# lucidrains/vector-quantize-pytorch

Measured on NVIDIA H100. Metric: vectors quantized/sec at dim=256, codebook=1024; indices bit-exact vs ref, higher is better.
Workload: dtype bf16

## Files before the change

### include/vqb200.h

```cpp
#ifndef VQB200_H
#define VQB200_H

#include <stddef.h>
#include <stdint.h>

#ifdef __cplusplus
extern "C" {
#endif

#define VQB_VERSION 100

#define VQB_DTYPE_F32 0
#define VQB_DTYPE_BF16 1

#define VQB_METRIC_EUCLID 0
#define VQB_METRIC_COSINE 1

#define VQB_OK 0
#define VQB_E_INVALID -1
#define VQB_E_UNSUPPORTED -2
#define VQB_E_ALIGN -3
#define VQB_E_NO_DEVICE -4
#define VQB_E_DRIVER -5
#define VQB_E_WORKSPACE -6

typedef struct vqb_flag_entry {
  int32_t row;
  int32_t count;
  int32_t cand0;
  int32_t cand1;
  int32_t cand2;
  int32_t pad[3];
} vqb_flag_entry;

typedef struct vqb_fused_outputs {
  const void* x_eff;
  const float* embed;
  void* q_out;
  int64_t* idx64_out;
  int64_t idx_stride;
  double* loss_sum;
  const void* x_raw;
  void* resid_out;
  void* qsum;
  float* stats_cnt;
  float* stats_sum;
  int dtype;
  void* planes_out;
} vqb_fused_outputs;

int vqb_version(void);
const char* vqb_strerror(int code);

int vqb_padded_codes(int K);

int vqb_codebook_prepare(const float* embed, int K, int D, int metric, void* planes, void* bext, float* bias,
                         float* cnorm2, float* cmax, void* stream);

int vqb_input_prepare(const void* x, int dtype, int64_t N, int D, int metric, void* x_eff, void* a_planes,
                      int n_planes, void* stream);

int vqb_assign(const void* a_planes, int n_a, int64_t N, int D, const void* b_planes, const void* bext,
               const float* cmax, int K, float margin_rel, int n_passes, int32_t* idx, vqb_flag_entry* flagged,
               int32_t* flag_count, float* dbg_best, const vqb_fused_outputs* fused , void* stream);

int vqb_assign_ex(const void* a_planes, int n_a, int64_t N, int D, const void* b_planes, const void* bext,
                  const float* cmax, int K, float margin_rel, int n_passes, int32_t* idx, vqb_flag_entry* flagged,
                  int32_t* flag_count, float* dbg_best, const vqb_fused_outputs* fused, int metric, const float* cnorm2,
                  void* stream);

int vqb_debug_set_profile_buffer(void* device_buffer);
int vqb_debug_active(void);
int vqb_debug_set_mode(int mode);
int vqb_debug_graph_stats(long long* out4);
int vqb_debug_assign_plan(int n_a, int D, int n_passes, int* out6);
int vqb_debug_stats_plan(int64_t N, int K, int sms, int* out3);

int vqb_fix_flagged(const void* x_eff, int dtype, int64_t N, int D, const float* embed, const float* cnorm2, int K,
                    int metric, vqb_flag_entry* flagged, const int32_t* flag_count, int32_t* idx,
                    const vqb_fused_outputs* fused , void* stream);

int vqb_gather(const void* x_eff, int dtype, int64_t N, int D, const float* embed, const int32_t* idx, void* q_out,
               int64_t* idx64_out, int64_t idx_stride, double* loss_sum, const void* x_raw, void* resid_out, void* qsum,
               void* stream);

int vqb_loss_finalize(const double* loss_sum, int64_t numel, int dtype, float weight, float* loss_out, void* stream);

int64_t vqb_stats_offset(int K);
int64_t vqb_stats_floats(int K, int D);
size_t vqb_ema_stats_workspace(int64_t N, int K);
int vqb_ema_stats(const void* x_eff, int dtype, int64_t N, int D, const int32_t* idx, int K, float* stats,
                  void* workspace, size_t workspace_bytes, void* stream);

int vqb_ema_apply(float* cluster_size, float* embed_avg, float* embed, const float* stats, int K, int D, double decay,
                  double eps, int metric, int do_lerp, int do_normalise, void* planes, void* bext, float* bias,
                  float* cnorm2, float* cmax, float* scratch, void* stream);

int vqb_ema_apply_weighted(float* cluster_size, float* embed_avg, float* embed, const float* stats, int K, int D,
                           double decay, double eps, int metric, int do_lerp, int do_normalise, const float* code_weight,
                           void* planes, void* bext, float* bias, float* cnorm2, float* cmax, float* scratch, void* stream);

int vqb_peer_barrier(void* const* peer_flags_host, int rank, int world, uint32_t* epoch_dev, void* stream);
int vqb_ema_apply_peers(float* cluster_size, float* embed_avg, float* embed, const void* const* peer_stats_host, int world,
                        int64_t slice_offset, int K, int D, double decay, double eps, int metric, int do_normalise,
                        const float* code_weight, void* planes, void* bext, float* bias, float* cnorm2, float* cmax,
                        float* scratch, void* stream);

typedef struct vqb_vq_forward_args {
  const void* x;
  int dtype, metric;
  int64_t N;
  int D, K;
  int already_normalised;
  float* cluster_size;
  float* embed_avg;
  float* embed;
  void* planes; void* bext; float* bias; float* cnorm2; float* cmax; float* scratch;
  void* q_out;
  int64_t* idx64_out; int64_t idx_stride;
  float* loss_out; float loss_weight;
  void* resid_out;
  void* qsum;
  int32_t* idx32;
  int update;
  int stats_mode;
  int stats_accumulate;
  int do_normalise;
  double decay, eps;
  float* stats;
  float margin_rel;
  void* workspace; size_t workspace_bytes;
  void* ev_search_begin; void* ev_search_end;
  const void* const* peer_stats; void* const* peer_flags; uint32_t* peer_epoch; int peer_rank, peer_world;
  int64_t peer_slice_offset;
  const void* a_planes_in; void* planes_out;
  const uint8_t* row_mask; const int64_t* n_live;
} vqb_vq_forward_args;
size_t vqb_vq_forward_workspace(int64_t N, int D, int K, int dtype, int metric, int update);
int vqb_vq_forward(const vqb_vq_forward_args* args, void* stream);

int vqb_decode(const float* embeds, int64_t embed_stride, int Q, int K, int D, const int64_t* idx, int64_t N,
               void* out, int dtype, void* stream);

int vqb_rvq_accumulate(const float* embeds, int64_t embed_stride, int Q, int K, int D, const int64_t* idx, int64_t N,
                       void* out, int dtype, void* stream);
int vqb_debug_gather_sum_plan(int nbooks, int K, int D, int esz, int64_t N, int sms, int* out3);

enum { VQB_RVQ_STAGE = 0, VQB_RVQ_EMA = 1, VQB_RVQ_ACCUMULATE = 2, VQB_RVQ_BARRIER = 3, VQB_RVQ_EMA_PEERS = 4,
       VQB_RVQ_SIMVQ_TAIL = 5 };
typedef struct vqb_rvq_op {
  int kind, lane;
  vqb_vq_forward_args stage;
  struct {
    float* cluster_size; float* embed_avg; float* embed; const float* stats; int K, D; double decay, eps;
    int metric, do_lerp, do_normalise; void* planes; void* bext; float* bias; float* cnorm2; float* cmax; float* scratch;
    int n_lerp; int64_t slice_stride;
  } ema;
  struct {
    const float* embeds; int64_t embed_stride; int Q, K, D; const int64_t* idx; int64_t N; void* out; int dtype;
  } acc;
  struct { void* const* flags; uint32_t* epoch; int rank, world; } bar;
  struct {
    float* cluster_size; float* embed_avg; float* embed; const void* const* peer_stats; int64_t slice_offset; int world, K, D;
    double decay, eps; int metric, do_normalise; void* planes; void* bext; float* bias; float* cnorm2; float* cmax; float* scratch;
    int n_lerp; int64_t slice_stride;
  } emap;
  struct {
    const float* r; const float* codes; const int32_t* idx; int64_t N; int D, rotation; float* r_next; float* qsum; int first;
    int64_t* idx64_out; int64_t idx_stride; double* loss_sum; float* loss_out; float input_weight, weight;
  } simvq;
} vqb_rvq_op;
int vqb_rvq_forward(const vqb_rvq_op* ops, int n_ops, void* stream);

int vqb_rsimvq_tail(const float* r, const float* codes, const int32_t* idx, int64_t N, int D, int rotation, float* r_next,
                    float* qsum, int first, int64_t* idx64_out, int64_t idx_stride, double* loss_sum, float* loss_out,
                    float input_weight, float weight, void* stream);
int vqb_rsimvq_backward(const float* x, const float* codes, int Q, int K, const int64_t* idx, int64_t N, int D, int n_active,
                        int rotation, const float* grad_q, const float* grad_loss, float* grad_x, void* stream);

int vqb_rotate(const void* src, const void* tgt, const void* grad_out, int64_t N, int D, int dtype, void* out, void* stream);

int vqb_diveq(const void* x, const void* q, const void* noise, const void* grad_out, int64_t N, int D, int dtype,
              float noise_scale, void* out, float* grad_q, void* stream);

int vqb_fsq_forward(const void* z, int in_dtype, int work_dtype, int64_t N, int G, int D, int Q, int n_active, int sym, int hard,
                    const float* consts, const float* scales, const float* clampv, void* out, void* idx, int idx64,
                    int64_t idx_s_row, int64_t idx_s_g, int64_t idx_s_q, void* stream);
int vqb_fsq_backward(const void* z, int in_dtype, int work_dtype, int64_t N, int G, int D, int Q, int n_active, int sym, int hard,
                     const float* consts, const float* scales, const float* clampv, const void* grad_out, void* grad_z,
                     void* stream);
int vqb_fsq_decode(const void* idx, int idx64, int64_t idx_s_row, int64_t idx_s_g, int64_t idx_s_q, int64_t N, int G, int D,
                   int Q, int work_dtype, int sym, const float* consts, const int32_t* levels_basis, const float* scales, void* out,
                   void* codes, void* stream);

int vqb_lfq_forward(const void* z, int dtype, int64_t N, int G, int D, int Q, int n_active, int residual, int training, int spherical,
                    const float* params, void* out, void* idx, int64_t idx_s_row, int64_t idx_s_g, int64_t idx_s_q, float* ent,
                    const uint8_t* rowmask, double* commit, int commit_blocks, void* stream);
int vqb_lfq_forward_blocks(int64_t N, int G);
int vqb_lfq_entropy(const float* x, int64_t N, int G, int D, int S, const int32_t* rows, int64_t R, int64_t rows_stride,
                    const float* m, float tau, int chunks, double* pse, float* colsum, void* stream);
int vqb_lfq_entropy_tiles(int D);
int vqb_lfq_entropy_backward(const float* x, int64_t N, int G, int D, int S, const int32_t* rows, int64_t R, int64_t rows_stride,
                             const float* m, float tau, const float* cp, const float* V, int ksplit, float* work, float* grad,
                             void* stream);
int vqb_lfq_backward(const void* z, int dtype, int64_t N, int G, int D, int Q, int n_active, int residual, int training, int spherical,
                     const float* params, const void* grad_out, const float* grad_ent, const float* cc, const uint8_t* rowmask,
                     void* grad_z, void* stream);
int vqb_lfq_decode(const void* idx, int idx64, int64_t idx_s_row, int64_t idx_s_g, int64_t idx_s_q, int64_t N, int G, int D, int Q,
                   const float* vals, float* out, float* codes, void* stream);

#ifdef __cplusplus
}
#endif
#endif
```

### vector_quantize_pytorch_b200/_C.py

```python
import ctypes
import os

from . import build as _build

_c = ctypes
_i32, _i64, _f32, _f64, _vp, _sz = _c.c_int, _c.c_int64, _c.c_float, _c.c_double, _c.c_void_p, _c.c_size_t

DTYPE_F32, DTYPE_BF16 = 0, 1
METRIC_EUCLID, METRIC_COSINE = 0, 1

class FusedOutputs(ctypes.Structure):
    _fields_ = [("x_eff", _vp), ("embed", _vp), ("q_out", _vp), ("idx64_out", _vp), ("idx_stride", _i64),
                ("loss_sum", _vp), ("x_raw", _vp), ("resid_out", _vp), ("qsum", _vp), ("stats_cnt", _vp), ("stats_sum", _vp),
                ("dtype", _i32), ("planes_out", _vp)]


class VQForwardArgs(ctypes.Structure):
    _fields_ = [("x", _vp), ("dtype", _i32), ("metric", _i32), ("N", _i64), ("D", _i32), ("K", _i32),
                ("already_normalised", _i32), ("cluster_size", _vp), ("embed_avg", _vp), ("embed", _vp),
                ("planes", _vp), ("bext", _vp), ("bias", _vp), ("cnorm2", _vp), ("cmax", _vp), ("scratch", _vp),
                ("q_out", _vp), ("idx64_out", _vp), ("idx_stride", _i64), ("loss_out", _vp), ("loss_weight", _f32),
                ("resid_out", _vp), ("qsum", _vp), ("idx32", _vp), ("update", _i32), ("stats_mode", _i32), ("stats_accumulate", _i32), ("do_normalise", _i32),
                ("decay", _f64), ("eps", _f64), ("stats", _vp), ("margin_rel", _f32), ("workspace", _vp),
                ("workspace_bytes", _sz), ("ev_search_begin", _vp), ("ev_search_end", _vp),
                ("peer_stats", _vp), ("peer_flags", _vp), ("peer_epoch", _vp), ("peer_rank", _i32), ("peer_world", _i32),
                ("peer_slice_offset", _i64), ("a_planes_in", _vp), ("planes_out", _vp), ("row_mask", _vp), ("n_live", _vp)]


class RvqEmaArgs(ctypes.Structure):
    _fields_ = [("cluster_size", _vp), ("embed_avg", _vp), ("embed", _vp), ("stats", _vp), ("K", _i32), ("D", _i32),
                ("decay", _f64), ("eps", _f64), ("metric", _i32), ("do_lerp", _i32), ("do_normalise", _i32),
                ("planes", _vp), ("bext", _vp), ("bias", _vp), ("cnorm2", _vp), ("cmax", _vp), ("scratch", _vp),
                ("n_lerp", _i32), ("slice_stride", _i64)]


class RvqAccArgs(ctypes.Structure):
    _fields_ = [("embeds", _vp), ("embed_stride", _i64), ("Q", _i32), ("K", _i32), ("D", _i32), ("idx", _vp), ("N", _i64),
                ("out", _vp), ("dtype", _i32)]


class RvqBarArgs(ctypes.Structure):
    _fields_ = [("flags", _vp), ("epoch", _vp), ("rank", _i32), ("world", _i32)]


class RvqEmaPeersArgs(ctypes.Structure):
    _fields_ = [("cluster_size", _vp), ("embed_avg", _vp), ("embed", _vp), ("peer_stats", _vp), ("slice_offset", _i64),
                ("world", _i32), ("K", _i32), ("D", _i32), ("decay", _f64), ("eps", _f64), ("metric", _i32),
                ("do_normalise", _i32), ("planes", _vp), ("bext", _vp), ("bias", _vp), ("cnorm2", _vp), ("cmax", _vp),
                ("scratch", _vp), ("n_lerp", _i32), ("slice_stride", _i64)]


class RvqSimvqArgs(ctypes.Structure):
    _fields_ = [("r", _vp), ("codes", _vp), ("idx", _vp), ("N", _i64), ("D", _i32), ("rotation", _i32), ("r_next", _vp),
                ("qsum", _vp), ("first", _i32), ("idx64_out", _vp), ("idx_stride", _i64), ("loss_sum", _vp), ("loss_out", _vp),
                ("input_weight", _f32), ("weight", _f32)]


class RvqOp(ctypes.Structure):
    _fields_ = [("kind", _i32), ("lane", _i32), ("stage", VQForwardArgs), ("ema", RvqEmaArgs), ("acc", RvqAccArgs),
                ("bar", RvqBarArgs), ("emap", RvqEmaPeersArgs), ("simvq", RvqSimvqArgs)]


RVQ_STAGE, RVQ_EMA, RVQ_ACCUMULATE, RVQ_BARRIER, RVQ_EMA_PEERS, RVQ_SIMVQ_TAIL = 0, 1, 2, 3, 4, 5

SIGNATURES = {
    "vqb_version": (_i32, []),
    "vqb_strerror": (_c.c_char_p, [_i32]),
    "vqb_padded_codes": (_i32, [_i32]),
    "vqb_codebook_prepare": (_i32, [_vp, _i32, _i32, _i32, _vp, _vp, _vp, _vp, _vp, _vp]),
    "vqb_input_prepare": (_i32, [_vp, _i32, _i64, _i32, _i32, _vp, _vp, _i32, _vp]),
    "vqb_assign": (_i32, [_vp, _i32, _i64, _i32, _vp, _vp, _vp, _i32, _f32, _i32, _vp, _vp, _vp, _vp, _vp, _vp]),
    "vqb_assign_ex": (_i32, [_vp, _i32, _i64, _i32, _vp, _vp, _vp, _i32, _f32, _i32, _vp, _vp, _vp, _vp, _vp, _i32, _vp, _vp]),
    "vqb_fix_flagged": (_i32, [_vp, _i32, _i64, _i32, _vp, _vp, _i32, _i32, _vp, _vp, _vp, _vp, _vp]),
    "vqb_gather": (_i32, [_vp, _i32, _i64, _i32, _vp, _vp, _vp, _vp, _i64, _vp, _vp, _vp, _vp, _vp]),
    "vqb_loss_finalize": (_i32, [_vp, _i64, _i32, _f32, _vp, _vp]),
    "vqb_stats_offset": (_i64, [_i32]),
    "vqb_stats_floats": (_i64, [_i32, _i32]),
    "vqb_ema_stats_workspace": (_sz, [_i64, _i32]),
    "vqb_ema_stats": (_i32, [_vp, _i32, _i64, _i32, _vp, _i32, _vp, _vp, _sz, _vp]),
    "vqb_ema_apply": (_i32, [_vp, _vp, _vp, _vp, _i32, _i32, _f64, _f64, _i32, _i32, _i32, _vp, _vp, _vp, _vp, _vp, _vp, _vp]),
    "vqb_rotate": (_i32, [_vp, _vp, _vp, _i64, _i32, _i32, _vp, _vp]),
    "vqb_diveq": (_i32, [_vp, _vp, _vp, _vp, _i64, _i32, _i32, _f32, _vp, _vp, _vp]),
    "vqb_peer_barrier": (_i32, [_vp, _i32, _i32, _vp, _vp]),
    "vqb_ema_apply_peers": (_i32, [_vp, _vp, _vp, _vp, _i32, _i64, _i32, _i32, _f64, _f64, _i32, _i32, _vp, _vp, _vp, _vp, _vp, _vp, _vp, _vp]),
    "vqb_ema_apply_weighted": (_i32, [_vp, _vp, _vp, _vp, _i32, _i32, _f64, _f64, _i32, _i32, _i32, _vp, _vp, _vp, _vp, _vp, _vp, _vp, _vp]),
    "vqb_vq_forward_workspace": (_sz, [_i64, _i32, _i32, _i32, _i32, _i32]),
    "vqb_vq_forward": (_i32, [_vp, _vp]),
    "vqb_debug_set_profile_buffer": (_i32, [_vp]),
    "vqb_debug_set_mode": (_i32, [_i32]),
    "vqb_debug_active": (_i32, []),
    "vqb_debug_graph_stats": (_i32, [_vp]),
    "vqb_debug_assign_plan": (_i32, [_i32, _i32, _i32, _vp]),
    "vqb_debug_stats_plan": (_i32, [_i64, _i32, _i32, _vp]),
    "vqb_decode": (_i32, [_vp, _i64, _i32, _i32, _i32, _vp, _i64, _vp, _i32, _vp]),
    "vqb_rvq_accumulate": (_i32, [_vp, _i64, _i32, _i32, _i32, _vp, _i64, _vp, _i32, _vp]),
    "vqb_debug_gather_sum_plan": (_i32, [_i32, _i32, _i32, _i32, _i64, _i32, _vp]),
    "vqb_rvq_forward": (_i32, [_vp, _i32, _vp]),
    "vqb_rsimvq_tail": (_i32, [_vp, _vp, _vp, _i64, _i32, _i32, _vp, _vp, _i32, _vp, _i64, _vp, _vp, _f32, _f32, _vp]),
    "vqb_rsimvq_backward": (_i32, [_vp, _vp, _i32, _i32, _vp, _i64, _i32, _i32, _i32, _vp, _vp, _vp, _vp]),
    "vqb_fsq_forward": (_i32, [_vp, _i32, _i32, _i64, _i32, _i32, _i32, _i32, _i32, _i32, _vp, _vp, _vp, _vp, _vp, _i32, _i64, _i64,
                               _i64, _vp]),
    "vqb_fsq_backward": (_i32, [_vp, _i32, _i32, _i64, _i32, _i32, _i32, _i32, _i32, _i32, _vp, _vp, _vp, _vp, _vp, _vp]),
    "vqb_fsq_decode": (_i32, [_vp, _i32, _i64, _i64, _i64, _i64, _i32, _i32, _i32, _i32, _i32, _vp, _vp, _vp, _vp, _vp, _vp]),
    "vqb_lfq_forward": (_i32, [_vp, _i32, _i64, _i32, _i32, _i32, _i32, _i32, _i32, _i32, _vp, _vp, _vp, _i64, _i64, _i64, _vp, _vp,
                               _vp, _i32, _vp]),
    "vqb_lfq_forward_blocks": (_i32, [_i64, _i32]),
    "vqb_lfq_entropy": (_i32, [_vp, _i64, _i32, _i32, _i32, _vp, _i64, _i64, _vp, _f32, _i32, _vp, _vp, _vp]),
    "vqb_lfq_entropy_tiles": (_i32, [_i32]),
    "vqb_lfq_entropy_backward": (_i32, [_vp, _i64, _i32, _i32, _i32, _vp, _i64, _i64, _vp, _f32, _vp, _vp, _i32, _vp, _vp, _vp]),
    "vqb_lfq_backward": (_i32, [_vp, _i32, _i64, _i32, _i32, _i32, _i32, _i32, _i32, _i32, _vp, _vp, _vp, _vp, _vp, _vp, _vp]),
    "vqb_lfq_decode": (_i32, [_vp, _i32, _i64, _i64, _i64, _i64, _i32, _i32, _i32, _vp, _vp, _vp, _vp]),
}


def _load():
    path = os.environ.get("VQB200_LIB")
    if not path:
        path = _build.LIB
        if _build.is_stale():
            if _build.find_nvcc() is not None:
                path = _build.build()
            elif not os.path.exists(path):
                raise ImportError("vqb200: libvqb200.so is missing and nvcc is not available to build it; "
                                  "run `python -m vector_quantize_pytorch_b200.build` where nvcc exists")
    lib = ctypes.CDLL(path)
    for name, (res, args) in SIGNATURES.items():
        fn = getattr(lib, name)
        fn.restype = res
        fn.argtypes = args
    return lib, path


lib, LIB_PATH = _load()


class VQBError(RuntimeError):
    pass


def check(rc, what):
    if rc != 0:
        raise VQBError(f"{what}: {lib.vqb_strerror(rc).decode()} (code {rc})")
```

### vector_quantize_pytorch_b200/csrc/code_operands.cuh

```cuda
#pragma once
#include "vqb_common.cuh"

namespace vqb {

constexpr int CODE_ROW_MAX_D = 8 * 128;

template <int NV>
__device__ __forceinline__ void load_code_row(const float* row, int D, int lane, float4 (&c)[NV]) {
#pragma unroll
  for (int j = 0; j < NV; ++j) {
    const int i = j * 128 + lane * 4;
    c[j] = i < D ? *reinterpret_cast<const float4*>(row + i) : make_float4(0.f, 0.f, 0.f, 0.f);
  }
}

template <int NV>
__device__ __forceinline__ void write_code_operands(const float4 (&c)[NV], int k, int Kpad, int D, int metric, uint16_t* planes,
                                                    uint16_t* bext, float* bias, float* cnorm2, float* cmax, int lane) {
  uint16_t* hi = planes + static_cast<int64_t>(k) * D;
  uint16_t* lo = planes + (static_cast<int64_t>(Kpad) + k) * D;
  double n2 = 0.0;
  float r2 = 0.f, l2 = 0.f;
#pragma unroll
  for (int j = 0; j < NV; ++j) {
    const int i = j * 128 + lane * 4;
    if (i >= D) continue;
    const float v[4] = {c[j].x, c[j].y, c[j].z, c[j].w};
    uint16_t h[4], l[4];
#pragma unroll
    for (int e = 0; e < 4; ++e) {
      h[e] = float_to_bf16_bits(v[e]);
      const float dl = v[e] - bf16_bits_to_float(h[e]);
      l[e] = float_to_bf16_bits(dl);
      const float d2 = dl - bf16_bits_to_float(l[e]);
      r2 = fmaf(d2, d2, r2);
      l2 = fmaf(bf16_bits_to_float(l[e]), bf16_bits_to_float(l[e]), l2);
      n2 += static_cast<double>(v[e]) * static_cast<double>(v[e]);
    }
    *reinterpret_cast<uint2*>(hi + i) = make_uint2(h[0] | (uint32_t(h[1]) << 16), h[2] | (uint32_t(h[3]) << 16));
    *reinterpret_cast<uint2*>(lo + i) = make_uint2(l[0] | (uint32_t(l[1]) << 16), l[2] | (uint32_t(l[3]) << 16));
  }
  n2 = warp_sum(n2);
  r2 = warp_sum(r2);
  l2 = warp_sum(l2);
  if (lane == 0) {
    const float n2f = static_cast<float>(n2);
    cnorm2[k] = n2f;
    const float b = (metric == VQB_METRIC_EUCLID) ? 0.5f * n2f : 0.f;
    bias[k] = b;
    const uint16_t b1 = float_to_bf16_bits(b);
    const float q1 = b - bf16_bits_to_float(b1);
    const uint16_t b2 = float_to_bf16_bits(q1);
    const uint16_t b3 = float_to_bf16_bits(q1 - bf16_bits_to_float(b2));
    uint16_t* row = bext + k * 16;
    row[0] = b1 ^ 0x8000; row[1] = b2 ^ 0x8000; row[2] = b3 ^ 0x8000;
#pragma unroll
    for (int j = 3; j < 16; ++j) row[j] = 0;
    atomicMax(reinterpret_cast<unsigned int*>(cmax + CMAX_NORM), __float_as_uint(sqrtf(n2f)));
    atomicMax(reinterpret_cast<unsigned int*>(cmax + CMAX_RES), __float_as_uint(__fsqrt_ru(r2) * 1.0001f));
    atomicMax(reinterpret_cast<unsigned int*>(cmax + CMAX_LO), __float_as_uint(__fsqrt_ru(l2) * 1.0001f));
  }
}

__device__ __forceinline__ void write_padding_operands(int k, int Kpad, int D, uint16_t* planes, uint16_t* bext, float* bias,
                                                       int lane) {
  uint16_t* hi = planes + static_cast<int64_t>(k) * D;
  uint16_t* lo = planes + (static_cast<int64_t>(Kpad) + k) * D;
  for (int i = lane; i < D; i += 32) { hi[i] = 0; lo[i] = 0; }
  if (lane == 0) bias[k] = INFINITY;
  if (lane < 16) bext[k * 16 + lane] = (lane == 0) ? float_to_bf16_bits(-3.0e38f) : 0;
}

}
```

### vector_quantize_pytorch_b200/csrc/ptx.cuh

```cuda
#pragma once
#include <cuda.h>
#include <cuda_runtime.h>
#include <stdint.h>

namespace vqb {

__device__ __forceinline__ uint32_t smem_u32(const void* p) {
  return static_cast<uint32_t>(__cvta_generic_to_shared(p));
}

__device__ __forceinline__ void mbar_init(uint32_t bar, uint32_t count) {
  asm volatile("mbarrier.init.shared::cta.b64 [%0], %1;" ::"r"(bar), "r"(count));
}
__device__ __forceinline__ void fence_barrier_init() {
  asm volatile("fence.mbarrier_init.release.cluster;" ::: "memory");
}
__device__ __forceinline__ void mbar_arrive(uint32_t bar) {
  asm volatile("mbarrier.arrive.shared::cta.b64 _, [%0];" ::"r"(bar) : "memory");
}
__device__ __forceinline__ void mbar_arrive_expect_tx(uint32_t bar, uint32_t bytes) {
  asm volatile("mbarrier.arrive.expect_tx.shared::cta.b64 _, [%0], %1;" ::"r"(bar), "r"(bytes) : "memory");
}
__device__ __forceinline__ bool mbar_try_wait(uint32_t bar, uint32_t parity) {
  uint32_t ok;
  asm volatile(
      "{\n"
      ".reg .pred p;\n"
      "mbarrier.try_wait.parity.shared::cta.b64 p, [%1], %2;\n"
      "selp.u32 %0, 1, 0, p;\n"
      "}\n"
      : "=r"(ok)
      : "r"(bar), "r"(parity)
      : "memory");
  return ok != 0;
}

#ifndef VQB_WAIT_TIMEOUT_CYCLES
#define VQB_WAIT_TIMEOUT_CYCLES (8000000000ll)
#endif
__device__ __forceinline__ void mbar_wait(uint32_t bar, uint32_t parity) {
  if (mbar_try_wait(bar, parity)) return;
  const long long t0 = clock64();
  while (!mbar_try_wait(bar, parity)) {
    if (clock64() - t0 > VQB_WAIT_TIMEOUT_CYCLES) __trap();
  }
}

__device__ __forceinline__ void tma_prefetch_desc(const CUtensorMap* m) {
  asm volatile("prefetch.tensormap [%0];" ::"l"(reinterpret_cast<uint64_t>(m)) : "memory");
}
__device__ __forceinline__ void tma_load_3d(uint32_t dst, const CUtensorMap* m, uint32_t bar, int c0, int c1, int c2) {
  asm volatile(
      "cp.async.bulk.tensor.3d.shared::cluster.global.tile.mbarrier::complete_tx::bytes [%0], [%1, {%3, %4, %5}], [%2];"
      ::"r"(dst), "l"(reinterpret_cast<uint64_t>(m)), "r"(bar), "r"(c0), "r"(c1), "r"(c2)
      : "memory");
}

__device__ __forceinline__ void tma_prefetch_l2_3d(const CUtensorMap* m, int c0, int c1, int c2) {
  asm volatile("cp.async.bulk.prefetch.tensor.3d.L2.global.tile [%0, {%1, %2, %3}];"
               ::"l"(reinterpret_cast<uint64_t>(m)), "r"(c0), "r"(c1), "r"(c2)
               : "memory");
}

__device__ __forceinline__ uint64_t wgmma_desc_sw128(uint32_t saddr) {
  uint64_t d = 0;
  d |= static_cast<uint64_t>((saddr >> 4) & 0x3FFF);
  d |= static_cast<uint64_t>(1) << 16;
  d |= static_cast<uint64_t>(1024 >> 4) << 32;
  d |= static_cast<uint64_t>(1) << 62;
  return d;
}

__device__ __forceinline__ uint64_t wgmma_desc_sw32(uint32_t saddr) {
  uint64_t d = 0;
  d |= static_cast<uint64_t>((saddr >> 4) & 0x3FFF);
  d |= static_cast<uint64_t>(1) << 16;
  d |= static_cast<uint64_t>(256 >> 4) << 32;
  d |= static_cast<uint64_t>(3) << 62;
  return d;
}

__device__ __forceinline__ void fence_proxy_async_shared() { asm volatile("fence.proxy.async.shared::cta;" ::: "memory"); }
__device__ __forceinline__ void wgmma_fence() { asm volatile("wgmma.fence.sync.aligned;" ::: "memory"); }
__device__ __forceinline__ void wgmma_commit() { asm volatile("wgmma.commit_group.sync.aligned;" ::: "memory"); }
template <int N>
__device__ __forceinline__ void wgmma_wait() { asm volatile("wgmma.wait_group.sync.aligned %0;" ::"n"(N) : "memory"); }

template <int R>
__device__ __forceinline__ void fence_regs(float (&d)[R]) {
#pragma unroll
  for (int i = 0; i < R; ++i) asm volatile("" : "+f"(d[i])::"memory");
}

__device__ __forceinline__ void wgmma_m64n128k16_bf16(float (&d)[64], uint64_t adesc, uint64_t bdesc) {
  asm volatile(
      "{\n"
      "wgmma.mma_async.sync.aligned.m64n128k16.f32.bf16.bf16 "
      "{%0, %1, %2, %3, %4, %5, %6, %7, %8, %9, %10, %11, %12, %13, %14, %15, "
      "%16, %17, %18, %19, %20, %21, %22, %23, %24, %25, %26, %27, %28, %29, %30, %31, "
      "%32, %33, %34, %35, %36, %37, %38, %39, %40, %41, %42, %43, %44, %45, %46, %47, "
      "%48, %49, %50, %51, %52, %53, %54, %55, %56, %57, %58, %59, %60, %61, %62, %63}, "
      "%64, %65, 1, 1, 1, 0, 0;\n"
      "}\n"
      : "+f"(d[0]), "+f"(d[1]), "+f"(d[2]), "+f"(d[3]), "+f"(d[4]), "+f"(d[5]), "+f"(d[6]), "+f"(d[7]),
        "+f"(d[8]), "+f"(d[9]), "+f"(d[10]), "+f"(d[11]), "+f"(d[12]), "+f"(d[13]), "+f"(d[14]), "+f"(d[15]),
        "+f"(d[16]), "+f"(d[17]), "+f"(d[18]), "+f"(d[19]), "+f"(d[20]), "+f"(d[21]), "+f"(d[22]), "+f"(d[23]),
        "+f"(d[24]), "+f"(d[25]), "+f"(d[26]), "+f"(d[27]), "+f"(d[28]), "+f"(d[29]), "+f"(d[30]), "+f"(d[31]),
        "+f"(d[32]), "+f"(d[33]), "+f"(d[34]), "+f"(d[35]), "+f"(d[36]), "+f"(d[37]), "+f"(d[38]), "+f"(d[39]),
        "+f"(d[40]), "+f"(d[41]), "+f"(d[42]), "+f"(d[43]), "+f"(d[44]), "+f"(d[45]), "+f"(d[46]), "+f"(d[47]),
        "+f"(d[48]), "+f"(d[49]), "+f"(d[50]), "+f"(d[51]), "+f"(d[52]), "+f"(d[53]), "+f"(d[54]), "+f"(d[55]),
        "+f"(d[56]), "+f"(d[57]), "+f"(d[58]), "+f"(d[59]), "+f"(d[60]), "+f"(d[61]), "+f"(d[62]), "+f"(d[63])
      : "l"(adesc), "l"(bdesc));
}

__device__ __forceinline__ void wgmma_m64n128k16_bf16_rs_set(float (&d)[64], uint32_t a01, uint64_t bdesc) {
  asm volatile(
      "{\n"
      ".reg .pred p;\n"
      "setp.ne.b32 p, %67, 0;\n"
      "wgmma.mma_async.sync.aligned.m64n128k16.f32.bf16.bf16 "
      "{%0, %1, %2, %3, %4, %5, %6, %7, %8, %9, %10, %11, %12, %13, %14, %15, "
      "%16, %17, %18, %19, %20, %21, %22, %23, %24, %25, %26, %27, %28, %29, %30, %31, "
      "%32, %33, %34, %35, %36, %37, %38, %39, %40, %41, %42, %43, %44, %45, %46, %47, "
      "%48, %49, %50, %51, %52, %53, %54, %55, %56, %57, %58, %59, %60, %61, %62, %63}, "
      "{%64, %64, %65, %65}, %66, p, 1, 1, 0;\n"
      "}\n"
      : "=f"(d[0]), "=f"(d[1]), "=f"(d[2]), "=f"(d[3]), "=f"(d[4]), "=f"(d[5]), "=f"(d[6]), "=f"(d[7]),
        "=f"(d[8]), "=f"(d[9]), "=f"(d[10]), "=f"(d[11]), "=f"(d[12]), "=f"(d[13]), "=f"(d[14]), "=f"(d[15]),
        "=f"(d[16]), "=f"(d[17]), "=f"(d[18]), "=f"(d[19]), "=f"(d[20]), "=f"(d[21]), "=f"(d[22]), "=f"(d[23]),
        "=f"(d[24]), "=f"(d[25]), "=f"(d[26]), "=f"(d[27]), "=f"(d[28]), "=f"(d[29]), "=f"(d[30]), "=f"(d[31]),
        "=f"(d[32]), "=f"(d[33]), "=f"(d[34]), "=f"(d[35]), "=f"(d[36]), "=f"(d[37]), "=f"(d[38]), "=f"(d[39]),
        "=f"(d[40]), "=f"(d[41]), "=f"(d[42]), "=f"(d[43]), "=f"(d[44]), "=f"(d[45]), "=f"(d[46]), "=f"(d[47]),
        "=f"(d[48]), "=f"(d[49]), "=f"(d[50]), "=f"(d[51]), "=f"(d[52]), "=f"(d[53]), "=f"(d[54]), "=f"(d[55]),
        "=f"(d[56]), "=f"(d[57]), "=f"(d[58]), "=f"(d[59]), "=f"(d[60]), "=f"(d[61]), "=f"(d[62]), "=f"(d[63])
      : "r"(a01), "r"(0u), "l"(bdesc), "n"(0));
}

__device__ __forceinline__ void wgmma_m64n256k16_bf16(float (&d)[128], uint64_t adesc, uint64_t bdesc) {
  asm volatile(
      "{\n"
      "wgmma.mma_async.sync.aligned.m64n256k16.f32.bf16.bf16 "
      "{%0, %1, %2, %3, %4, %5, %6, %7, %8, %9, %10, %11, %12, %13, %14, %15, "
      "%16, %17, %18, %19, %20, %21, %22, %23, %24, %25, %26, %27, %28, %29, %30, %31, "
      "%32, %33, %34, %35, %36, %37, %38, %39, %40, %41, %42, %43, %44, %45, %46, %47, "
      "%48, %49, %50, %51, %52, %53, %54, %55, %56, %57, %58, %59, %60, %61, %62, %63, "
      "%64, %65, %66, %67, %68, %69, %70, %71, %72, %73, %74, %75, %76, %77, %78, %79, "
      "%80, %81, %82, %83, %84, %85, %86, %87, %88, %89, %90, %91, %92, %93, %94, %95, "
      "%96, %97, %98, %99, %100, %101, %102, %103, %104, %105, %106, %107, %108, %109, %110, %111, "
      "%112, %113, %114, %115, %116, %117, %118, %119, %120, %121, %122, %123, %124, %125, %126, %127}, "
      "%128, %129, 1, 1, 1, 0, 0;\n"
      "}\n"
      :
        "+f"(d[0]), "+f"(d[1]), "+f"(d[2]), "+f"(d[3]), "+f"(d[4]), "+f"(d[5]), "+f"(d[6]), "+f"(d[7]),
        "+f"(d[8]), "+f"(d[9]), "+f"(d[10]), "+f"(d[11]), "+f"(d[12]), "+f"(d[13]), "+f"(d[14]), "+f"(d[15]),
        "+f"(d[16]), "+f"(d[17]), "+f"(d[18]), "+f"(d[19]), "+f"(d[20]), "+f"(d[21]), "+f"(d[22]), "+f"(d[23]),
        "+f"(d[24]), "+f"(d[25]), "+f"(d[26]), "+f"(d[27]), "+f"(d[28]), "+f"(d[29]), "+f"(d[30]), "+f"(d[31]),
        "+f"(d[32]), "+f"(d[33]), "+f"(d[34]), "+f"(d[35]), "+f"(d[36]), "+f"(d[37]), "+f"(d[38]), "+f"(d[39]),
        "+f"(d[40]), "+f"(d[41]), "+f"(d[42]), "+f"(d[43]), "+f"(d[44]), "+f"(d[45]), "+f"(d[46]), "+f"(d[47]),
        "+f"(d[48]), "+f"(d[49]), "+f"(d[50]), "+f"(d[51]), "+f"(d[52]), "+f"(d[53]), "+f"(d[54]), "+f"(d[55]),
        "+f"(d[56]), "+f"(d[57]), "+f"(d[58]), "+f"(d[59]), "+f"(d[60]), "+f"(d[61]), "+f"(d[62]), "+f"(d[63]),
        "+f"(d[64]), "+f"(d[65]), "+f"(d[66]), "+f"(d[67]), "+f"(d[68]), "+f"(d[69]), "+f"(d[70]), "+f"(d[71]),
        "+f"(d[72]), "+f"(d[73]), "+f"(d[74]), "+f"(d[75]), "+f"(d[76]), "+f"(d[77]), "+f"(d[78]), "+f"(d[79]),
        "+f"(d[80]), "+f"(d[81]), "+f"(d[82]), "+f"(d[83]), "+f"(d[84]), "+f"(d[85]), "+f"(d[86]), "+f"(d[87]),
        "+f"(d[88]), "+f"(d[89]), "+f"(d[90]), "+f"(d[91]), "+f"(d[92]), "+f"(d[93]), "+f"(d[94]), "+f"(d[95]),
        "+f"(d[96]), "+f"(d[97]), "+f"(d[98]), "+f"(d[99]), "+f"(d[100]), "+f"(d[101]), "+f"(d[102]), "+f"(d[103]),
        "+f"(d[104]), "+f"(d[105]), "+f"(d[106]), "+f"(d[107]), "+f"(d[108]), "+f"(d[109]), "+f"(d[110]), "+f"(d[111]),
        "+f"(d[112]), "+f"(d[113]), "+f"(d[114]), "+f"(d[115]), "+f"(d[116]), "+f"(d[117]), "+f"(d[118]), "+f"(d[119]),
        "+f"(d[120]), "+f"(d[121]), "+f"(d[122]), "+f"(d[123]), "+f"(d[124]), "+f"(d[125]), "+f"(d[126]), "+f"(d[127])
      : "l"(adesc), "l"(bdesc));
}

__device__ __forceinline__ void wgmma_m64n256k16_bf16_ss_set(float (&d)[128], uint64_t adesc, uint64_t bdesc) {
  asm volatile(
      "{\n"
      ".reg .pred p;\n"
      "setp.ne.b32 p, %130, 0;\n"
      "wgmma.mma_async.sync.aligned.m64n256k16.f32.bf16.bf16 "
      "{%0, %1, %2, %3, %4, %5, %6, %7, %8, %9, %10, %11, %12, %13, %14, %15, "
      "%16, %17, %18, %19, %20, %21, %22, %23, %24, %25, %26, %27, %28, %29, %30, %31, "
      "%32, %33, %34, %35, %36, %37, %38, %39, %40, %41, %42, %43, %44, %45, %46, %47, "
      "%48, %49, %50, %51, %52, %53, %54, %55, %56, %57, %58, %59, %60, %61, %62, %63, "
      "%64, %65, %66, %67, %68, %69, %70, %71, %72, %73, %74, %75, %76, %77, %78, %79, "
      "%80, %81, %82, %83, %84, %85, %86, %87, %88, %89, %90, %91, %92, %93, %94, %95, "
      "%96, %97, %98, %99, %100, %101, %102, %103, %104, %105, %106, %107, %108, %109, %110, %111, "
      "%112, %113, %114, %115, %116, %117, %118, %119, %120, %121, %122, %123, %124, %125, %126, %127}, "
      "%128, %129, p, 1, 1, 0, 0;\n"
      "}\n"
      :
        "=f"(d[0]), "=f"(d[1]), "=f"(d[2]), "=f"(d[3]), "=f"(d[4]), "=f"(d[5]), "=f"(d[6]), "=f"(d[7]),
        "=f"(d[8]), "=f"(d[9]), "=f"(d[10]), "=f"(d[11]), "=f"(d[12]), "=f"(d[13]), "=f"(d[14]), "=f"(d[15]),
        "=f"(d[16]), "=f"(d[17]), "=f"(d[18]), "=f"(d[19]), "=f"(d[20]), "=f"(d[21]), "=f"(d[22]), "=f"(d[23]),
        "=f"(d[24]), "=f"(d[25]), "=f"(d[26]), "=f"(d[27]), "=f"(d[28]), "=f"(d[29]), "=f"(d[30]), "=f"(d[31]),
        "=f"(d[32]), "=f"(d[33]), "=f"(d[34]), "=f"(d[35]), "=f"(d[36]), "=f"(d[37]), "=f"(d[38]), "=f"(d[39]),
        "=f"(d[40]), "=f"(d[41]), "=f"(d[42]), "=f"(d[43]), "=f"(d[44]), "=f"(d[45]), "=f"(d[46]), "=f"(d[47]),
        "=f"(d[48]), "=f"(d[49]), "=f"(d[50]), "=f"(d[51]), "=f"(d[52]), "=f"(d[53]), "=f"(d[54]), "=f"(d[55]),
        "=f"(d[56]), "=f"(d[57]), "=f"(d[58]), "=f"(d[59]), "=f"(d[60]), "=f"(d[61]), "=f"(d[62]), "=f"(d[63]),
        "=f"(d[64]), "=f"(d[65]), "=f"(d[66]), "=f"(d[67]), "=f"(d[68]), "=f"(d[69]), "=f"(d[70]), "=f"(d[71]),
        "=f"(d[72]), "=f"(d[73]), "=f"(d[74]), "=f"(d[75]), "=f"(d[76]), "=f"(d[77]), "=f"(d[78]), "=f"(d[79]),
        "=f"(d[80]), "=f"(d[81]), "=f"(d[82]), "=f"(d[83]), "=f"(d[84]), "=f"(d[85]), "=f"(d[86]), "=f"(d[87]),
        "=f"(d[88]), "=f"(d[89]), "=f"(d[90]), "=f"(d[91]), "=f"(d[92]), "=f"(d[93]), "=f"(d[94]), "=f"(d[95]),
        "=f"(d[96]), "=f"(d[97]), "=f"(d[98]), "=f"(d[99]), "=f"(d[100]), "=f"(d[101]), "=f"(d[102]), "=f"(d[103]),
        "=f"(d[104]), "=f"(d[105]), "=f"(d[106]), "=f"(d[107]), "=f"(d[108]), "=f"(d[109]), "=f"(d[110]), "=f"(d[111]),
        "=f"(d[112]), "=f"(d[113]), "=f"(d[114]), "=f"(d[115]), "=f"(d[116]), "=f"(d[117]), "=f"(d[118]), "=f"(d[119]),
        "=f"(d[120]), "=f"(d[121]), "=f"(d[122]), "=f"(d[123]), "=f"(d[124]), "=f"(d[125]), "=f"(d[126]), "=f"(d[127])
      : "l"(adesc), "l"(bdesc), "n"(0));
}

__device__ __forceinline__ void wgmma_m64n256k16_bf16_rs_set(float (&d)[128], uint32_t a01, uint64_t bdesc) {
  asm volatile(
      "{\n"
      ".reg .pred p;\n"
      "setp.ne.b32 p, %131, 0;\n"
      "wgmma.mma_async.sync.aligned.m64n256k16.f32.bf16.bf16 "
      "{%0, %1, %2, %3, %4, %5, %6, %7, %8, %9, %10, %11, %12, %13, %14, %15, "
      "%16, %17, %18, %19, %20, %21, %22, %23, %24, %25, %26, %27, %28, %29, %30, %31, "
      "%32, %33, %34, %35, %36, %37, %38, %39, %40, %41, %42, %43, %44, %45, %46, %47, "
      "%48, %49, %50, %51, %52, %53, %54, %55, %56, %57, %58, %59, %60, %61, %62, %63, "
      "%64, %65, %66, %67, %68, %69, %70, %71, %72, %73, %74, %75, %76, %77, %78, %79, "
      "%80, %81, %82, %83, %84, %85, %86, %87, %88, %89, %90, %91, %92, %93, %94, %95, "
      "%96, %97, %98, %99, %100, %101, %102, %103, %104, %105, %106, %107, %108, %109, %110, %111, "
      "%112, %113, %114, %115, %116, %117, %118, %119, %120, %121, %122, %123, %124, %125, %126, %127}, "
      "{%128, %128, %129, %129}, %130, p, 1, 1, 0;\n"
      "}\n"
      :
        "=f"(d[0]), "=f"(d[1]), "=f"(d[2]), "=f"(d[3]), "=f"(d[4]), "=f"(d[5]), "=f"(d[6]), "=f"(d[7]),
        "=f"(d[8]), "=f"(d[9]), "=f"(d[10]), "=f"(d[11]), "=f"(d[12]), "=f"(d[13]), "=f"(d[14]), "=f"(d[15]),
        "=f"(d[16]), "=f"(d[17]), "=f"(d[18]), "=f"(d[19]), "=f"(d[20]), "=f"(d[21]), "=f"(d[22]), "=f"(d[23]),
        "=f"(d[24]), "=f"(d[25]), "=f"(d[26]), "=f"(d[27]), "=f"(d[28]), "=f"(d[29]), "=f"(d[30]), "=f"(d[31]),
        "=f"(d[32]), "=f"(d[33]), "=f"(d[34]), "=f"(d[35]), "=f"(d[36]), "=f"(d[37]), "=f"(d[38]), "=f"(d[39]),
        "=f"(d[40]), "=f"(d[41]), "=f"(d[42]), "=f"(d[43]), "=f"(d[44]), "=f"(d[45]), "=f"(d[46]), "=f"(d[47]),
        "=f"(d[48]), "=f"(d[49]), "=f"(d[50]), "=f"(d[51]), "=f"(d[52]), "=f"(d[53]), "=f"(d[54]), "=f"(d[55]),
        "=f"(d[56]), "=f"(d[57]), "=f"(d[58]), "=f"(d[59]), "=f"(d[60]), "=f"(d[61]), "=f"(d[62]), "=f"(d[63]),
        "=f"(d[64]), "=f"(d[65]), "=f"(d[66]), "=f"(d[67]), "=f"(d[68]), "=f"(d[69]), "=f"(d[70]), "=f"(d[71]),
        "=f"(d[72]), "=f"(d[73]), "=f"(d[74]), "=f"(d[75]), "=f"(d[76]), "=f"(d[77]), "=f"(d[78]), "=f"(d[79]),
        "=f"(d[80]), "=f"(d[81]), "=f"(d[82]), "=f"(d[83]), "=f"(d[84]), "=f"(d[85]), "=f"(d[86]), "=f"(d[87]),
        "=f"(d[88]), "=f"(d[89]), "=f"(d[90]), "=f"(d[91]), "=f"(d[92]), "=f"(d[93]), "=f"(d[94]), "=f"(d[95]),
        "=f"(d[96]), "=f"(d[97]), "=f"(d[98]), "=f"(d[99]), "=f"(d[100]), "=f"(d[101]), "=f"(d[102]), "=f"(d[103]),
        "=f"(d[104]), "=f"(d[105]), "=f"(d[106]), "=f"(d[107]), "=f"(d[108]), "=f"(d[109]), "=f"(d[110]), "=f"(d[111]),
        "=f"(d[112]), "=f"(d[113]), "=f"(d[114]), "=f"(d[115]), "=f"(d[116]), "=f"(d[117]), "=f"(d[118]), "=f"(d[119]),
        "=f"(d[120]), "=f"(d[121]), "=f"(d[122]), "=f"(d[123]), "=f"(d[124]), "=f"(d[125]), "=f"(d[126]), "=f"(d[127])
      : "r"(a01), "r"(0u), "l"(bdesc), "n"(0));
}

}
```

### vector_quantize_pytorch_b200/csrc/vq_assign.cu

```cuda
#include <type_traits>
#include "ptx.cuh"
#include "vqb_common.cuh"
#include "gather_row.cuh"
#include "epilogue.cuh"

#ifdef VQB_PROFILE
#define PROF_CLOCK() clock64()
#else
#define PROF_CLOCK() 0ll
#endif

namespace vqb {

constexpr int BM = 128;
constexpr int WM = 64;
constexpr int BN_STAGE = 128;
constexpr int BK = 64;
constexpr int A_SUB_BYTES = BM * BK * 2;
constexpr int B_SUB_BYTES = BN_STAGE * BK * 2;
constexpr int MAX_A_SUB = 8;
constexpr int MAX_STAGES = 8;
constexpr int NUM_CONSUMER_WARPS = 8;
constexpr int NUM_STORE_WARPS = 3;
constexpr int NUM_THREADS = 128 + NUM_CONSUMER_WARPS * 32;
constexpr int SMEM_CTRL_BYTES = 14336;
constexpr int SMEM_LIMIT = 232448;
constexpr int SEED_BYTES = BN_STAGE * 32;

struct AssignParams {
  int64_t N;
  int D, K, Kpad;
  int n_a, n_passes;
  int KB;
  int n_stages;
  int n_seed;
  int stream_a;
  const uint16_t* a_global;
  const uint16_t* bext;
  int num_row_tiles, num_code_steps;
  float margin_rel;
  const float* cmax;
  int32_t* idx;
  int32_t* idx_prov;
  int32_t* hist;
  int hist_shift;
  vqb_flag_entry* flagged;
  int32_t* flag_count;
  float* dbg_best;
  const uint8_t* row_mask;
  long long* prof;
  FusedOut fo;
  int copy_mode;
  int resid_mode;
  int metric;
  const uint16_t* b_hi;
  const float* cnorm2;
  uint32_t tagmask, mul1, mulm1;
};

struct Ctrl {
  uint64_t a_full[MAX_A_SUB], a_empty[MAX_A_SUB];
  uint64_t b_full[MAX_STAGES], b_empty[MAX_STAGES];
  uint64_t g_full[2], g_empty[2];
  int gidx[2][BM];
  MergeSlot merge[BM][3];
  float x2[BM];
};
static_assert(sizeof(Ctrl) <= SMEM_CTRL_BYTES, "control block too large");

template <int GB>
__device__ __forceinline__ float tail_rows(const FusedOut& fo, const int64_t (&rows)[GB], const int (&ks)[GB], int D, int lane) {
  if (fo.dtype == VQB_DTYPE_BF16) return gather_rows<VQB_DTYPE_BF16, GB>(fo, rows, ks, D, lane);
  return gather_rows<VQB_DTYPE_F32, GB>(fo, rows, ks, D, lane);
}

__device__ __forceinline__ float sq_diff16(const uint4& xa, const uint4& ca, bool bf) {
  const uint32_t xw[4] = {xa.x, xa.y, xa.z, xa.w}, cw[4] = {ca.x, ca.y, ca.z, ca.w};
  float s = 0.f;
#pragma unroll
  for (int e = 0; e < 4; ++e) {
    if (bf) {
      const float d0 = __uint_as_float(xw[e] << 16) - __uint_as_float(cw[e] << 16);
      const float d1 = __uint_as_float(xw[e] & 0xFFFF0000u) - __uint_as_float(cw[e] & 0xFFFF0000u);
      s += bf16_round(d0 * d0);
      s += bf16_round(d1 * d1);
    } else {
      const float d = __uint_as_float(xw[e]) - __uint_as_float(cw[e]);
      s += d * d;
    }
  }
  return s;
}

template <int WN>
struct StepLocals {
  float loss_ = 0.f;
  __device__ __forceinline__ float& loss() { return loss_; }
};
template <>
struct StepLocals<256> {
  static __device__ __forceinline__ float& loss() {
    __shared__ float s[NUM_CONSUMER_WARPS * 32];
    return s[threadIdx.x - 128];
  }
  static __device__ __forceinline__ uint32_t* bias_ones() {
    __shared__ __align__(256) uint32_t o[WM * 16 / 2];
    return o;
  }
  __device__ __forceinline__ StepLocals() { loss() = 0.f; }
};
constexpr int WIDE_STATIC_SMEM = NUM_CONSUMER_WARPS * 32 * 4 + WM * 16 * 2;

template <int TAIL, int WN>
__global__ void __launch_bounds__(NUM_THREADS, 1)
vq_assign_kernel(const __grid_constant__ CUtensorMap tmA, const __grid_constant__ CUtensorMap tmB,
                 const __grid_constant__ CUtensorMap tmS, const AssignParams p) {
  static_assert(WN == 128 || WN == 256, "code step width");
  constexpr int SPAN = WN / BN_STAGE;
  constexpr uint32_t STEP_SEED_BYTES = SPAN * SEED_BYTES;
  extern __shared__ __align__(1024) uint8_t smem[];
  Ctrl* ctrl = reinterpret_cast<Ctrl*>(smem);
  const uint32_t smem_base = smem_u32(smem);
  const uint32_t a_base = (smem_base + SMEM_CTRL_BYTES + 1023u) & ~1023u;
  const bool stream_a = WN == 128 && p.stream_a;
  const int n_sub = stream_a ? 0 : p.n_a * p.KB;
  const uint32_t b_base = a_base + n_sub * A_SUB_BYTES;
  const uint32_t a_stage_bytes = stream_a ? A_SUB_BYTES : 0;
  const uint32_t stage_stride = a_stage_bytes + SPAN * B_SUB_BYTES;
  const int n_ring = p.n_stages / SPAN;
  const uint32_t seed_base = b_base + n_ring * stage_stride;

  const int warp = threadIdx.x >> 5;
  const int lane = threadIdx.x & 31;

  if (threadIdx.x == 0) {
    tma_prefetch_desc(&tmA);
    tma_prefetch_desc(&tmB);
    tma_prefetch_desc(&tmS);
    for (int s = 0; s < n_sub; ++s) {
      mbar_init(smem_u32(&ctrl->a_full[s]), 1);
      mbar_init(smem_u32(&ctrl->a_empty[s]), NUM_CONSUMER_WARPS);
    }
    for (int s = 0; s < n_ring; ++s) {
      mbar_init(smem_u32(&ctrl->b_full[s]), 1);
      mbar_init(smem_u32(&ctrl->b_empty[s]), NUM_CONSUMER_WARPS);
    }
    for (int s = 0; s < 2; ++s) {
      mbar_init(smem_u32(&ctrl->g_full[s]), NUM_CONSUMER_WARPS);
      mbar_init(smem_u32(&ctrl->g_empty[s]), NUM_STORE_WARPS);
    }
    fence_barrier_init();
  }
  if constexpr (WN == 256) {
    for (int i = threadIdx.x; i < WM * 16 / 2; i += NUM_THREADS) StepLocals<256>::bias_ones()[i] = 0x3F803F80u;
    fence_proxy_async_shared();
  }
  __syncthreads();

  if (warp == 0) {
    if (lane == 0) {
      long long w_empty = 0, w_aempty = 0;
      const long long pstart = PROF_CLOCK();
      int stage = 0, gstep = 0;
      uint32_t ph = 0;
      for (int t = 0, tile = static_cast<int>(blockIdx.x); tile < p.num_row_tiles; ++t, tile += static_cast<int>(gridDim.x)) {
        const int row0 = tile * BM;
        if (!stream_a && tile + static_cast<int>(gridDim.x) < p.num_row_tiles) {
          for (int ap = 0; ap < p.n_a; ++ap)
            for (int kb = 0; kb < p.KB; ++kb) tma_prefetch_l2_3d(&tmA, kb * BK, row0 + static_cast<int>(gridDim.x) * BM, ap);
        }
        for (int ct = 0; ct < p.num_code_steps; ++ct, ++gstep) {
          for (int kb = 0; kb < p.KB; ++kb) {
            for (int ps = 0; ps < p.n_passes; ++ps) {
              const int bplane = (ps == 1) ? 1 : 0;
              const int aplane = (ps == 2) ? 1 : 0;
              if (!stream_a && ct == 0 && (ps == 0 || ps == 2)) {
                const int sub = aplane * p.KB + kb;
                { const long long c0 = PROF_CLOCK(); mbar_wait(smem_u32(&ctrl->a_empty[sub]), (t & 1) ^ 1); w_aempty += PROF_CLOCK() - c0; }
                mbar_arrive_expect_tx(smem_u32(&ctrl->a_full[sub]), A_SUB_BYTES);
                tma_load_3d(a_base + sub * A_SUB_BYTES, &tmA, smem_u32(&ctrl->a_full[sub]), kb * BK, row0, aplane);
              }
              { const long long c0 = PROF_CLOCK(); mbar_wait(smem_u32(&ctrl->b_empty[stage]), ph ^ 1); w_empty += PROF_CLOCK() - c0; }
              const bool seeds = kb == 0 && ps == 0;
              mbar_arrive_expect_tx(smem_u32(&ctrl->b_full[stage]), stage_stride + (seeds ? STEP_SEED_BYTES : 0));
              if (seeds)
                tma_load_3d(seed_base + (gstep % p.n_seed) * STEP_SEED_BYTES, &tmS, smem_u32(&ctrl->b_full[stage]), 0, ct * WN, 0);
              if (stream_a)
                tma_load_3d(b_base + stage * stage_stride, &tmA, smem_u32(&ctrl->b_full[stage]), kb * BK, row0, aplane);
              tma_load_3d(b_base + stage * stage_stride + a_stage_bytes, &tmB, smem_u32(&ctrl->b_full[stage]), kb * BK,
                          ct * WN, bplane);
              if (++stage == n_ring) { stage = 0; ph ^= 1; }
            }
          }
        }
      }
      if (p.prof) {
        p.prof[blockIdx.x * 16 + 0] = w_empty;
        p.prof[blockIdx.x * 16 + 1] = PROF_CLOCK() - pstart;
        p.prof[blockIdx.x * 16 + 6] = w_aempty;
      }
    }
  } else if (warp <= NUM_STORE_WARPS) {
    const int sw = warp - 1;
    float lsum = 0.f;
    for (int t = 0, tile = static_cast<int>(blockIdx.x); p.fo.enabled && tile < p.num_row_tiles; ++t, tile += static_cast<int>(gridDim.x)) {
      mbar_wait(smem_u32(&ctrl->g_full[t & 1]), (t >> 1) & 1);
      const int* gi = ctrl->gidx[t & 1];
      if (TAIL >= 1) {
        constexpr int CB = 4;
        const bool bf = p.fo.dtype == VQB_DTYPE_BF16;
        const int row_bytes = p.D * (bf ? 2 : 4);
        const uint8_t* src = bf ? reinterpret_cast<const uint8_t*>(p.b_hi) : reinterpret_cast<const uint8_t*>(p.fo.embed);
        const uint8_t* xin = static_cast<const uint8_t*>(p.fo.x_eff);
        uint8_t* dst = static_cast<uint8_t*>(TAIL == 2 ? p.fo.resid_out : p.fo.q_out);
        for (int r0 = sw * CB; r0 < BM; r0 += NUM_STORE_WARPS * CB) {
          int ks[CB];
          bool ex[CB];
#pragma unroll
          for (int b = 0; b < CB; ++b) {
            const int g = gi[r0 + b];
            ex[b] = g < -1;
            ks[b] = ex[b] ? -2 - g : g;
          }
          const int64_t row_base = static_cast<int64_t>(tile) * BM + r0;
          if (p.fo.idx64_out && lane < CB && ks[lane & (CB - 1)] >= 0) {
            int kk = 0;
#pragma unroll
            for (int b = 0; b < CB; ++b) kk = (lane == b) ? ks[b] : kk;
            p.fo.idx64_out[(row_base + lane) * p.fo.idx_stride] = kk;
          }
          if (dst || (ex[0] | ex[1] | ex[2] | ex[3])) {
            for (int off = lane * 16; off < row_bytes; off += 512) {
              uint4 v[CB];
#pragma unroll
              for (int b = 0; b < CB; ++b)
                if (ks[b] >= 0) v[b] = __ldg(reinterpret_cast<const uint4*>(src + static_cast<int64_t>(ks[b]) * row_bytes + off));
              if (TAIL == 1) {
#pragma unroll
                for (int b = 0; b < CB; ++b)
                  if (ex[b]) lsum += sq_diff16(*reinterpret_cast<const uint4*>(xin + (row_base + b) * row_bytes + off), v[b], bf);
              }
              if (TAIL == 2) {
                uint4 x[CB];
#pragma unroll
                for (int b = 0; b < CB; ++b)
                  if (ks[b] >= 0) x[b] = *reinterpret_cast<const uint4*>(xin + (row_base + b) * row_bytes + off);
#pragma unroll
                for (int b = 0; b < CB; ++b) {
                  if (ks[b] < 0) continue;
                  if (ex[b]) lsum += sq_diff16(x[b], v[b], bf);
                  const uint32_t xw[4] = {x[b].x, x[b].y, x[b].z, x[b].w}, cw[4] = {v[b].x, v[b].y, v[b].z, v[b].w};
                  uint32_t rw[4];
                  if (bf) {
#pragma unroll
                    for (int e = 0; e < 4; ++e) {
                      const float d0 = __uint_as_float(xw[e] << 16) - __uint_as_float(cw[e] << 16);
                      const float d1 = __uint_as_float(xw[e] & 0xFFFF0000u) - __uint_as_float(cw[e] & 0xFFFF0000u);
                      asm("cvt.rn.bf16x2.f32 %0, %1, %2;" : "=r"(rw[e]) : "f"(d1), "f"(d0));
                    }
                  } else {
#pragma unroll
                    for (int e = 0; e < 4; ++e) rw[e] = __float_as_uint(__uint_as_float(xw[e]) - __uint_as_float(cw[e]));
                    if (p.fo.planes_out) {
                      const float rf[4] = {__uint_as_float(rw[0]), __uint_as_float(rw[1]), __uint_as_float(rw[2]), __uint_as_float(rw[3])};
                      store_planes4(p.fo.planes_out, p.fo.planes_stride, ((row_base + b) * row_bytes + off) >> 2, rf);
                    }
                  }
                  v[b] = make_uint4(rw[0], rw[1], rw[2], rw[3]);
                }
              }
#pragma unroll
              for (int b = 0; b < CB; ++b)
                if (dst && ks[b] >= 0) *reinterpret_cast<uint4*>(dst + (row_base + b) * row_bytes + off) = v[b];
            }
          }
        }
      } else {
        constexpr int GB = 2;
        for (int r0 = sw * GB; r0 < BM; r0 += NUM_STORE_WARPS * GB) {
          int64_t rows[GB];
          int ks[GB];
          bool any = false;
#pragma unroll
          for (int b = 0; b < GB; ++b) {
            ks[b] = gi[r0 + b];
            rows[b] = ks[b] >= 0 ? static_cast<int64_t>(tile) * BM + r0 + b : -1;
            any |= ks[b] >= 0;
          }
          if (!any) continue;
          lsum += tail_rows<GB>(p.fo, rows, ks, p.D, lane);
        }
      }
      __syncwarp();
      if (lane == 0) mbar_arrive(smem_u32(&ctrl->g_empty[t & 1]));
    }
    if (p.fo.enabled && p.fo.loss_sum) {
      const double w = warp_sum(static_cast<double>(lsum));
      if (lane == 0) atomicAdd(p.fo.loss_sum, w);
    }
  } else {
    const int wg = (warp >> 2) - 1;
    const int q = lane & 3;
    const int rit0 = wg * WM + (warp & 3) * 16 + (lane >> 2);
    const int n_items = p.KB * p.n_passes;
    const uint32_t a_row_off = wg * WM * 128;
    const uint32_t bias_a = q == 0 ? 0x3F803F80u : (q == 1 ? 0x00003F80u : 0u);
    long long w_full = 0, w_afull = 0, w_gap = 0, gap0 = -1;
    const long long cstart = PROF_CLOCK();
    float acc[WN / 2];
    int stage = 0, gstep = 0;
    uint32_t ph = 0;
    StepLocals<WN> locals;
    auto release = [&](int st, int sub) {
      if (lane == 0) {
        mbar_arrive(smem_u32(&ctrl->b_empty[st]));
        if (sub >= 0) mbar_arrive(smem_u32(&ctrl->a_empty[sub]));
      }
    };
    auto row_norms = [&](int tile, float (&xlo)[2]) {
#pragma unroll
      for (int h = 0; h < 2; ++h) {
        const int64_t row = static_cast<int64_t>(tile) * BM + rit0 + 8 * h;
        float a = 0.f, alo = 0.f;
        if (row < p.N) {
          const uint16_t* hp = p.a_global + row * p.D;
          for (int c = q * 8; c < p.D; c += 32) {
            const uint4 u = __ldg(reinterpret_cast<const uint4*>(hp + c));
            uint4 l = make_uint4(0u, 0u, 0u, 0u);
            if (p.n_a == 2) l = __ldg(reinterpret_cast<const uint4*>(hp + p.N * p.D + c));
            const uint32_t w[4] = {u.x, u.y, u.z, u.w};
            const uint32_t wl[4] = {l.x, l.y, l.z, l.w};
#pragma unroll
            for (int e = 0; e < 4; ++e) {
              const float h0 = __uint_as_float(w[e] << 16), h1 = __uint_as_float(w[e] & 0xFFFF0000u);
              const float l0 = __uint_as_float(wl[e] << 16), l1 = __uint_as_float(wl[e] & 0xFFFF0000u);
              a = fmaf(h0 + l0, h0 + l0, a);
              a = fmaf(h1 + l1, h1 + l1, a);
              alo = fmaf(l0, l0, alo);
              alo = fmaf(l1, l1, alo);
            }
          }
        }
        a += __shfl_xor_sync(0xffffffffu, a, 1);
        a += __shfl_xor_sync(0xffffffffu, a, 2);
        alo += __shfl_xor_sync(0xffffffffu, alo, 1);
        alo += __shfl_xor_sync(0xffffffffu, alo, 2);
        if (q == 0) ctrl->x2[rit0 + 8 * h] = a;
        xlo[h] = alo;
      }
    };
    auto init_band = [&](auto (&sc)[2], float (&xlo)[2]) {
      const bool euclid = p.metric != VQB_METRIC_COSINE;
      const float cmax = __ldg(p.cmax + CMAX_NORM);
      const float cres = __ldg(p.cmax + CMAX_RES);
      const float caux = p.n_a == 2 ? 0x1.02p-8f * cmax + __ldg(p.cmax + CMAX_LO) : 0.f;
      __syncwarp();
#pragma unroll
      for (int h = 0; h < 2; ++h) {
        const float x2 = ctrl->x2[rit0 + 8 * h];
        const float xn = sqrtf(x2);
        const float xc = xn * cmax;
        xlo[h] = p.n_a == 2 ? sqrtf(xlo[h]) * 1.0001f : 0.f;
        sc[h].init(2.f * (xn * cres + xlo[h] * caux + p.margin_rel * xc + (euclid ? 0x1p-21f * cmax * cmax : 0.f)) +
                   0x1p-18f * (xc + (euclid ? 0.5f * cmax * cmax : 0.f)) +
                   (euclid ? 0x1p-22f * (x2 + cmax * cmax) + 1e-8f : 1e-30f));
      }
    };
    for (int t = 0, tile = static_cast<int>(blockIdx.x); tile < p.num_row_tiles; ++t, tile += static_cast<int>(gridDim.x)) {
      typename std::conditional<WN == 128, ScanReg, ScanState<16>>::type sc[2];
      ScanQueue<16> sq[2];

      float xlo[2] = {0.f, 0.f};
      for (int ct = 0; ct < p.num_code_steps; ++ct) {
        const bool last_ct = ct == p.num_code_steps - 1;
        if (WN == 256 && ct == 0) {
          row_norms(tile, xlo);
          init_band(sc, xlo);
        }
        if (gap0 >= 0) w_gap += PROF_CLOCK() - gap0;
        { const long long c0 = PROF_CLOCK(); mbar_wait(smem_u32(&ctrl->b_full[stage]), ph); w_full += PROF_CLOCK() - c0; }
        wgmma_fence();
        const uint64_t sd = wgmma_desc_sw32(seed_base + (gstep % p.n_seed) * STEP_SEED_BYTES);
        if constexpr (WN == 128) wgmma_m64n128k16_bf16_rs_set(acc, bias_a, sd);
        else wgmma_m64n256k16_bf16_ss_set(acc, wgmma_desc_sw32(smem_u32(StepLocals<256>::bias_ones())), sd);
        int kb = 0, ps = 0;
        int pend_stage = -1, pend_sub = -1;
        for (int i = 0; i < n_items; ++i) {
          const int aplane = (ps == 2) ? 1 : 0;
          const int sub = aplane * p.KB + kb;
          if (ct == 0 && !stream_a) { const long long c0 = PROF_CLOCK(); mbar_wait(smem_u32(&ctrl->a_full[sub]), t & 1); w_afull += PROF_CLOCK() - c0; }
          if (i > 0) { const long long c0 = PROF_CLOCK(); mbar_wait(smem_u32(&ctrl->b_full[stage]), ph); w_full += PROF_CLOCK() - c0; }
          const uint32_t st_addr = b_base + stage * stage_stride;
          const uint32_t a_addr = (stream_a ? st_addr : a_base + sub * A_SUB_BYTES) + a_row_off;
          const uint64_t ad = wgmma_desc_sw128(a_addr);
          const uint64_t bd = wgmma_desc_sw128(st_addr + a_stage_bytes);
          fence_regs(acc);
          wgmma_fence();
#pragma unroll
          for (int k = 0; k < 8; k += 2) {
            if constexpr (WN == 128) wgmma_m64n128k16_bf16(acc, ad + k, bd + k);
            else wgmma_m64n256k16_bf16(acc, ad + k, bd + k);
          }
          wgmma_commit();
          if (i == n_items - 1) gap0 = PROF_CLOCK();
          wgmma_wait<1>();
          fence_regs(acc);
          if (pend_stage >= 0) release(pend_stage, pend_sub);
          const bool last_use = last_ct && !stream_a && (aplane == 1 ? ps == 2 : ps == 1);
          pend_stage = stage;
          pend_sub = last_use ? sub : -1;
          if (++stage == n_ring) { stage = 0; ph ^= 1; }
          if (++ps == p.n_passes) { ps = 0; ++kb; }
        }
        if (WN == 128 && ct == 0) row_norms(tile, xlo);
        wgmma_wait<0>();
        fence_regs(acc);
        release(pend_stage, pend_sub);
        ++gstep;
        if ((ct + 1) * WN > p.Kpad) {
#pragma unroll
          for (int j = 0; j < WN / 8; ++j)
#pragma unroll
            for (int b = 0; b < 2; ++b)
              if (ct * WN + 8 * j + 2 * q + b >= p.Kpad) { acc[4 * j + b] = -3.0e38f; acc[4 * j + 2 + b] = -3.0e38f; }
        }

        if (WN == 128 && ct == 0) {
          init_band(sc, xlo);
        } else if (ct > 0) {
#pragma unroll
          for (int h = 0; h < 2; ++h) {
            float m = sc[h].t1;
            m = fmaxf(m, __shfl_xor_sync(0xffffffffu, m, 1));
            m = fmaxf(m, __shfl_xor_sync(0xffffffffu, m, 2));
            sc[h].raise(m);
          }
        }
#pragma unroll
        for (int g = 0; g < WN / 64; ++g) {
#pragma unroll
          for (int h = 0; h < 2; ++h) {
            uint32_t r[16];
#pragma unroll
            for (int e = 0; e < 16; ++e) r[e] = __float_as_uint(acc[4 * (8 * g + (e >> 1)) + 2 * h + (e & 1)]);
            if constexpr (WN == 128) sc[h].template scan16<true, false>(sq[h], r, ct * WN + 64 * g + 2 * q, p.mul1);
            else sc[h].template scan16<true>(sq[h], r, ct * WN + 64 * g + 2 * q);
          }
        }
      }

      if (p.fo.enabled) mbar_wait(smem_u32(&ctrl->g_empty[t & 1]), ((t >> 1) & 1) ^ 1);
#pragma unroll
      for (int h = 0; h < 2; ++h) {
        const int rit = rit0 + 8 * h;
        RowState st;
        sc[h].finish(sq[h], st, p.tagmask, p.mul1, p.mulm1);
        MergeSlot* slots = ctrl->merge[rit];
        if (q != 0) publish(&slots[q - 1], st);
        __syncwarp();
        if (q == 0) {
          const RowResult rr = merge_slices(st, slots, 3, 1);
          const int n = rr.n, i0 = rr.i0, i1 = rr.i1;
          const float best = rr.best;
          const int64_t row = static_cast<int64_t>(tile) * BM + rit;
          const bool live = row < p.N && (p.row_mask == nullptr || __ldg(p.row_mask + row) != 0);
          bool exact_loss = false;
          if (TAIL >= 1 && p.fo.loss_sum && live && n < 2) {
            float d2 = ctrl->x2[rit] - 2.f * best;
            if (p.metric == VQB_METRIC_COSINE) d2 += __ldg(p.cnorm2 + i0);
            exact_loss = !(d2 >= 0x1p14f * st.W);
            if (!exact_loss) locals.loss() += d2;
          }
          if (p.fo.enabled) ctrl->gidx[t & 1][rit] = (live && n < 2) ? (exact_loss ? -2 - i0 : i0) : -1;
          if (row < p.N && !live) {
            p.idx[row] = -1;
            if (p.idx_prov) p.idx_prov[row] = -1;
          } else if (row < p.N) {
            p.idx[row] = i0;
            if (p.idx_prov) p.idx_prov[row] = (n < 2) ? i0 : -1;
            if (p.hist && n < 2) atomicAdd(p.hist + static_cast<size_t>(tile >> p.hist_shift) * p.K + i0, 1);
            if (p.dbg_best) p.dbg_best[row] = best;
            if (n >= 2) {
              const bool many = n > 3;
              const int s = many ? static_cast<int>(p.N) - 1 - atomicAdd(p.flag_count + 1, 1) : atomicAdd(p.flag_count, 1);
              vqb_flag_entry e;
              e.row = static_cast<int32_t>(row);
              e.cand0 = many ? 0 : i0;
              e.cand1 = many ? 0 : i1;
              e.cand2 = rr.i2;
              e.count = n;
              e.pad[0] = e.pad[1] = e.pad[2] = 0;
              p.flagged[s] = e;
            }
          }
        }
        __syncwarp();
      }
      if (p.fo.enabled && lane == 0) mbar_arrive(smem_u32(&ctrl->g_full[t & 1]));
    }
    if (TAIL >= 1 && p.fo.loss_sum) {
      const double w = warp_sum(static_cast<double>(locals.loss()));
      if (lane == 0) atomicAdd(p.fo.loss_sum, w);
    }
    if (p.prof && threadIdx.x == 128) {
      p.prof[blockIdx.x * 16 + 2] = w_full;
      p.prof[blockIdx.x * 16 + 3] = PROF_CLOCK() - cstart;
      p.prof[blockIdx.x * 16 + 4] = w_gap;
      p.prof[blockIdx.x * 16 + 5] = w_afull;
    }
  }
}

typedef CUresult (*PFN_encodeTiled)(CUtensorMap*, CUtensorMapDataType, cuuint32_t, void*, const cuuint64_t*,
                                    const cuuint64_t*, const cuuint32_t*, const cuuint32_t*, CUtensorMapInterleave,
                                    CUtensorMapSwizzle, CUtensorMapL2promotion, CUtensorMapFloatOOBfill);

static PFN_encodeTiled get_encode_fn() {
  static PFN_encodeTiled fn = nullptr;
  static bool tried = false;
  if (!tried) {
    tried = true;
    void* f = nullptr;
    cudaDriverEntryPointQueryResult qres;
    if (cudaGetDriverEntryPoint("cuTensorMapEncodeTiled", &f, cudaEnableDefault, &qres) == cudaSuccess &&
        qres == cudaDriverEntryPointSuccess)
      fn = reinterpret_cast<PFN_encodeTiled>(f);
  }
  return fn;
}

static int make_map(CUtensorMap* m, const void* base, int cols, int64_t rows, int planes, int box_cols, int box_rows,
                    CUtensorMapSwizzle swz) {
  PFN_encodeTiled enc = get_encode_fn();
  if (!enc) return VQB_E_DRIVER;
  cuuint64_t dims[3] = {static_cast<cuuint64_t>(cols), static_cast<cuuint64_t>(rows), static_cast<cuuint64_t>(planes)};
  cuuint64_t strides[2] = {static_cast<cuuint64_t>(cols) * 2, static_cast<cuuint64_t>(cols) * 2 * static_cast<cuuint64_t>(rows)};
  cuuint32_t box[3] = {static_cast<cuuint32_t>(box_cols), static_cast<cuuint32_t>(box_rows), 1};
  cuuint32_t estr[3] = {1, 1, 1};
  CUresult r = enc(m, CU_TENSOR_MAP_DATA_TYPE_BFLOAT16, 3, const_cast<void*>(base), dims, strides, box, estr,
                   CU_TENSOR_MAP_INTERLEAVE_NONE, swz, CU_TENSOR_MAP_L2_PROMOTION_L2_256B, CU_TENSOR_MAP_FLOAT_OOB_FILL_NONE);
  return r == CUDA_SUCCESS ? VQB_OK : VQB_E_DRIVER;
}

struct AssignPlan {
  int stream_a, n_stages, n_seed, n_items, KB, smem_bytes;
};

static int assign_plan(int n_a, int D, int n_passes, AssignPlan* pl) {
  if (D <= 0 || (n_a != 1 && n_a != 2)) return VQB_E_INVALID;
  if (n_passes == 0) n_passes = n_a + 1;
  if (n_passes != n_a + 1) return VQB_E_UNSUPPORTED;
  if (D % 8 != 0) return VQB_E_UNSUPPORTED;
  const int KB = (D + BK - 1) / BK;
  const int stream_a = n_a * KB > MAX_A_SUB ? 1 : 0;
  const int a_bytes = stream_a ? 0 : n_a * KB * A_SUB_BYTES;
  const int stage_bytes = B_SUB_BYTES + (stream_a ? A_SUB_BYTES : 0);
  const int fixed = SMEM_CTRL_BYTES + 1024  + a_bytes;
  const int n_items = KB * n_passes;
  int stages = MAX_STAGES;
  auto seed_slots = [&](int st) { return (st + n_items - 1) / n_items; };
  while (stages >= 2 && fixed + stages * stage_bytes + seed_slots(stages) * SEED_BYTES > SMEM_LIMIT) --stages;
  if (stages < 2) return VQB_E_UNSUPPORTED;
  pl->stream_a = stream_a;
  pl->n_stages = stages;
  pl->n_seed = seed_slots(stages);
  pl->n_items = n_items;
  pl->KB = KB;
  pl->smem_bytes = fixed + stages * stage_bytes + pl->n_seed * SEED_BYTES;
  return VQB_OK;
}

static bool wide_step(const AssignPlan& pl, int Kpad, int* n_seed, int* smem_bytes) {
  if (pl.stream_a || pl.n_stages % 2 != 0 || Kpad <= BN_STAGE) return false;
  const int ring = pl.n_stages / 2;
  const int seeds = (ring + pl.n_items - 1) / pl.n_items;
  const int bytes = pl.smem_bytes - pl.n_seed * SEED_BYTES + seeds * 2 * SEED_BYTES;
  if (bytes + WIDE_STATIC_SMEM > SMEM_LIMIT) return false;
  *n_seed = seeds;
  *smem_bytes = bytes;
  return true;
}

}

using namespace vqb;

extern "C" int vqb_debug_assign_plan(int n_a, int D, int n_passes, int* out6) {
  if (!out6) return VQB_E_INVALID;
  AssignPlan pl;
  const int rc = assign_plan(n_a, D, n_passes, &pl);
  if (rc) return rc;
  out6[0] = pl.stream_a; out6[1] = pl.n_stages; out6[2] = pl.n_seed;
  out6[3] = pl.n_items; out6[4] = pl.KB; out6[5] = pl.smem_bytes;
  return VQB_OK;
}

extern "C" int vqb_padded_codes(int K) {
  if (K <= 0) return 0;
  const int BN = code_tile(K);
  return (K + BN - 1) / BN * BN;
}

static long long* g_prof = nullptr;
static int g_dbg_mode = 0;
extern "C" int vqb_debug_set_mode(int mode) { g_dbg_mode = mode; return VQB_OK; }
extern "C" int vqb_debug_active(void) { return (g_prof != nullptr) || (g_dbg_mode != 0); }
extern "C" int vqb_debug_set_profile_buffer(void* buf) { g_prof = static_cast<long long*>(buf); return VQB_OK; }

extern "C" int vqb_assign(const void* a_planes, int n_a, int64_t N, int D, const void* b_planes, const void* bext,
                          const float* cmax, int K, float margin_rel, int n_passes, int32_t* idx,
                          vqb_flag_entry* flagged, int32_t* flag_count, float* dbg_best,
                          const vqb_fused_outputs* fused, void* stream) {
  return vqb_assign_ex(a_planes, n_a, N, D, b_planes, bext, cmax, K, margin_rel, n_passes, idx, flagged, flag_count,
                       dbg_best, fused, VQB_METRIC_EUCLID, nullptr, stream);
}

extern "C" int vqb_assign_ex(const void* a_planes, int n_a, int64_t N, int D, const void* b_planes, const void* bext,
                             const float* cmax, int K, float margin_rel, int n_passes, int32_t* idx,
                             vqb_flag_entry* flagged, int32_t* flag_count, float* dbg_best,
                             const vqb_fused_outputs* fused, int metric, const float* cnorm2, void* stream) {
  return vqb::assign_launch(a_planes, n_a, N, D, b_planes, bext, cmax, K, margin_rel, n_passes, idx, nullptr, nullptr, 0,
                            flagged, flag_count, dbg_best, fused, metric, cnorm2, stream);
}

int vqb::assign_launch(const void* a_planes, int n_a, int64_t N, int D, const void* b_planes, const void* bext,
                       const float* cmax, int K, float margin_rel, int n_passes, int32_t* idx, int32_t* idx_prov,
                       int32_t* hist, int hist_shift, vqb_flag_entry* flagged, int32_t* flag_count, float* dbg_best,
                       const vqb_fused_outputs* fused, int metric, const float* cnorm2, void* stream, const uint8_t* row_mask) {
  if (!a_planes || !b_planes || !bext || !cmax || !idx || !flagged || !flag_count) return VQB_E_INVALID;
  if (N <= 0 || K <= 0) return VQB_E_INVALID;
  AssignPlan plan;
  int rc = assign_plan(n_a, D, n_passes, &plan);
  if (rc) return rc;
  if (n_passes == 0) n_passes = n_a + 1;
  if (N > (static_cast<int64_t>(1) << 31) - BM) return VQB_E_UNSUPPORTED;
  if ((reinterpret_cast<uintptr_t>(a_planes) | reinterpret_cast<uintptr_t>(b_planes) | reinterpret_cast<uintptr_t>(bext)) & 15)
    return VQB_E_ALIGN;
  AssignParams p;
  rc = make_fused(&p.fo, fused, D, N);
  if (rc) return rc;
  rc = check_device();
  if (rc) return rc;

  p.N = N; p.D = D; p.K = K;
  p.Kpad = vqb_padded_codes(K);
  p.n_a = n_a; p.n_passes = n_passes; p.KB = plan.KB;
  p.num_row_tiles = static_cast<int>((N + BM - 1) / BM);
  int smem_bytes = plan.smem_bytes;
  p.n_seed = plan.n_seed;
  const bool wide = wide_step(plan, p.Kpad, &p.n_seed, &smem_bytes);
  const int WN = wide ? 256 : 128;
  p.num_code_steps = (p.Kpad + WN - 1) / WN;
  p.margin_rel = margin_rel;
  p.cmax = cmax; p.idx = idx; p.idx_prov = idx_prov; p.hist = hist; p.hist_shift = hist_shift; p.flagged = flagged; p.flag_count = flag_count; p.dbg_best = dbg_best;
  p.row_mask = row_mask;
  p.prof = g_prof;
  p.tagmask = 0xFFFFFFF0u; p.mul1 = 1u; p.mulm1 = 0xFFFFFFFFu;
  p.metric = metric;
  p.cnorm2 = cnorm2;
  p.b_hi = static_cast<const uint16_t*>(b_planes);
  p.bext = static_cast<const uint16_t*>(bext);
  p.copy_mode = p.fo.enabled && !p.fo.resid_out && !(metric == VQB_METRIC_COSINE && p.fo.loss_sum && !cnorm2);
  p.resid_mode = p.fo.enabled && p.fo.resid_out && !p.fo.q_out &&
                 (!p.fo.x_raw || p.fo.x_raw == p.fo.x_eff) && !(metric == VQB_METRIC_COSINE && p.fo.loss_sum && !cnorm2);
  p.stream_a = plan.stream_a;
  p.a_global = static_cast<const uint16_t*>(a_planes);
  p.n_stages = plan.n_stages;

  CUtensorMap tmA, tmB, tmS;
  rc = make_map(&tmA, a_planes, D, N, n_a, BK, BM, CU_TENSOR_MAP_SWIZZLE_128B);
  if (rc) return rc;
  rc = make_map(&tmB, b_planes, D, p.Kpad, 2, BK, WN, CU_TENSOR_MAP_SWIZZLE_128B);
  if (rc) return rc;
  rc = make_map(&tmS, bext, 16, p.Kpad, 1, 16, WN, CU_TENSOR_MAP_SWIZZLE_32B);
  if (rc) return rc;

  static bool attr_set = false;
  if (!attr_set) {
    void (*const kernels[6])(CUtensorMap, CUtensorMap, CUtensorMap, AssignParams) = {
        vq_assign_kernel<0, 128>, vq_assign_kernel<1, 128>, vq_assign_kernel<2, 128>,
        vq_assign_kernel<0, 256>, vq_assign_kernel<1, 256>, vq_assign_kernel<2, 256>};
    for (int i = 0; i < 6; ++i) {
      const int dyn = i < 3 ? SMEM_LIMIT : SMEM_LIMIT - WIDE_STATIC_SMEM;
      const cudaError_t e = cudaFuncSetAttribute(kernels[i], cudaFuncAttributeMaxDynamicSharedMemorySize, dyn);
      if (e != cudaSuccess) return static_cast<int>(e);
    }
    attr_set = true;
  }
  const int grid = p.num_row_tiles < num_sms() ? p.num_row_tiles : num_sms();
  cudaStream_t s = static_cast<cudaStream_t>(stream);
  if (wide) {
    if (p.copy_mode) vq_assign_kernel<1, 256><<<grid, NUM_THREADS, smem_bytes, s>>>(tmA, tmB, tmS, p);
    else if (p.resid_mode) vq_assign_kernel<2, 256><<<grid, NUM_THREADS, smem_bytes, s>>>(tmA, tmB, tmS, p);
    else vq_assign_kernel<0, 256><<<grid, NUM_THREADS, smem_bytes, s>>>(tmA, tmB, tmS, p);
  } else {
    if (p.copy_mode) vq_assign_kernel<1, 128><<<grid, NUM_THREADS, smem_bytes, s>>>(tmA, tmB, tmS, p);
    else if (p.resid_mode) vq_assign_kernel<2, 128><<<grid, NUM_THREADS, smem_bytes, s>>>(tmA, tmB, tmS, p);
    else vq_assign_kernel<0, 128><<<grid, NUM_THREADS, smem_bytes, s>>>(tmA, tmB, tmS, p);
  }
  return static_cast<int>(cudaGetLastError());
}
```

### vector_quantize_pytorch_b200/csrc/vq_ema.cu

```cuda
#include "vqb_common.cuh"
#include "code_operands.cuh"

namespace vqb {

constexpr int SEG_CHUNK = 512;
constexpr int SEG_THREADS = 256;

struct StatsWs {
  int32_t* counts;
  int32_t* offsets;
  int32_t* cursor;
  int32_t* nwork;
  int32_t* perm;
  int4* work;
  int32_t* ticket;
  int32_t* cta_counts;
};

static inline size_t align_up(size_t v, size_t a) { return (v + a - 1) / a * a; }
static inline int64_t max_work_items(int64_t N, int K) { return K + N / SEG_CHUNK + 1; }

constexpr int SORT_THREADS = 512;
constexpr int SORT_MAX_K = 16384;
constexpr int64_t SORT_MAX_CELLS = 1 << 22;
// ... 35 lines not shown
    ws->perm = reinterpret_cast<int32_t*>(b + o_perm);
    ws->work = reinterpret_cast<int4*>(b + o_work);
    ws->ticket = reinterpret_cast<int32_t*>(b + o_cta);
    ws->cta_counts = reinterpret_cast<int32_t*>(b + o_cta + 256);
  }
  return off;
}

__global__ void hist_kernel(const int32_t* __restrict__ idx, int64_t N, int K, int32_t* counts) {
  extern __shared__ int32_t sh[];
  const bool use_sh = K <= 8192;
  if (use_sh) {
    for (int i = threadIdx.x; i < K; i += blockDim.x) sh[i] = 0;
    __syncthreads();
  }
  for (int64_t r = static_cast<int64_t>(blockIdx.x) * blockDim.x + threadIdx.x; r < N;
       r += static_cast<int64_t>(gridDim.x) * blockDim.x) {
    const int k = idx[r];
    if (k < 0) continue;
    if (use_sh) atomicAdd(&sh[k], 1); else atomicAdd(&counts[k], 1);
  }
  if (use_sh) {
    __syncthreads();
    for (int i = threadIdx.x; i < K; i += blockDim.x)
      if (sh[i]) atomicAdd(&counts[i], sh[i]);
  }
}

__global__ void __launch_bounds__(SORT_THREADS)
hist_cta_kernel(const int32_t* __restrict__ idx, int64_t N, int K, int64_t rows_per_cta, int32_t* __restrict__ cta_counts) {
  extern __shared__ int32_t sh[];
  for (int i = threadIdx.x; i < K; i += SORT_THREADS) sh[i] = 0;
  __syncthreads();
  const int64_t b = blockIdx.x * rows_per_cta;
  const int64_t e = min(N, b + rows_per_cta);
  for (int64_t r = b + threadIdx.x; r < e; r += SORT_THREADS) {
    const int k = idx[r];
    if (k >= 0) atomicAdd(&sh[k], 1);
  }
  __syncthreads();
  int32_t* out = cta_counts + static_cast<size_t>(blockIdx.x) * K;
  for (int i = threadIdx.x; i < K; i += SORT_THREADS) out[i] = sh[i];
}

__device__ void scan_codes_block(const int32_t* counts, int K, int32_t* offsets, int32_t* cursor, int4* work, int32_t* nwork,
                                 float* stats) {
  __shared__ int32_t s_c[32], s_w[32];
  __shared__ int32_t carry_cnt, carry_wk, tot_cnt, tot_wk;
  const int nt = blockDim.x, lane = threadIdx.x & 31, warp = threadIdx.x >> 5, nwarps = nt >> 5;
  if (threadIdx.x == 0) { carry_cnt = 0; carry_wk = 0; }
  __syncthreads();
  for (int base = 0; base < K; base += nt) {
    const int k = base + threadIdx.x;
    const int c = k < K ? __ldcg(counts + k) : 0;
    const int w = (c + SEG_CHUNK - 1) / SEG_CHUNK;
    int ic = c, iw = w;
#pragma unroll
    for (int o = 1; o < 32; o <<= 1) {
      const int a = __shfl_up_sync(0xffffffffu, ic, o), b = __shfl_up_sync(0xffffffffu, iw, o);
      if (lane >= o) { ic += a; iw += b; }
    }
    if (lane == 31) { s_c[warp] = ic; s_w[warp] = iw; }
    __syncthreads();
    if (warp == 0) {
      int a = lane < nwarps ? s_c[lane] : 0, b = lane < nwarps ? s_w[lane] : 0;
      const int a0 = a, b0 = b;
#pragma unroll
      for (int o = 1; o < 32; o <<= 1) {
        const int x = __shfl_up_sync(0xffffffffu, a, o), y = __shfl_up_sync(0xffffffffu, b, o);
        if (lane >= o) { a += x; b += y; }
      }
      s_c[lane] = a - a0;
      s_w[lane] = b - b0;
      if (lane == 31) { tot_cnt = a; tot_wk = b; }
    }
    __syncthreads();
    const int wc = s_c[warp], ww = s_w[warp];
    const int ex_cnt = carry_cnt + wc + ic - c;
    const int ex_wk = carry_wk + ww + iw - w;
    if (k < K) {
      offsets[k] = ex_cnt;
      if (cursor) cursor[k] = ex_cnt;
      if (c) atomicAdd(stats + k, static_cast<float>(c));
      for (int j = 0; j < w; ++j) {
        const int b = ex_cnt + j * SEG_CHUNK;
        const int e = min(ex_cnt + c, b + SEG_CHUNK);
        work[ex_wk + j] = make_int4(k, b, e, 0);
      }
    }
    __syncthreads();
    if (threadIdx.x == 0) { carry_cnt += tot_cnt; carry_wk += tot_wk; }
    __syncthreads();
  }
  if (threadIdx.x == 0) *nwork = carry_wk;
}

constexpr int CS_CODES = 32, CS_PARTS = 32, CS_PER = 8;
__global__ void __launch_bounds__(CS_CODES * CS_PARTS)
colscan_kernel(int32_t* __restrict__ cta_counts, int G, int K, int32_t* __restrict__ counts, int32_t* ticket,
               int32_t* offsets, int4* work, int32_t* nwork, float* stats) {
  __shared__ int32_t part[CS_PARTS][CS_CODES + 1];
  __shared__ int s_last;
  const int lane = threadIdx.x & 31, w = threadIdx.x >> 5;
  const int k = blockIdx.x * CS_CODES + lane;
  const int per = (G + CS_PARTS - 1) / CS_PARTS;
  const int g0 = min(G, w * per), g1 = min(G, g0 + per);
  int v[CS_PER];
  int sum = 0;
#pragma unroll
  for (int j = 0; j < CS_PER; ++j) {
    v[j] = (k < K && g0 + j < g1) ? __ldcg(cta_counts + static_cast<size_t>(g0 + j) * K + k) : 0;
    sum += v[j];
  }
  part[w][lane] = sum;
  __syncthreads();
  int run = 0, total = 0;
#pragma unroll 8
  for (int q = 0; q < CS_PARTS; ++q) { const int x = part[q][lane]; run += (q < w) ? x : 0; total += x; }
  if (k < K) {
#pragma unroll
    for (int j = 0; j < CS_PER; ++j) {
      if (g0 + j < g1) cta_counts[static_cast<size_t>(g0 + j) * K + k] = run;
      run += v[j];
    }
    if (w == 0) counts[k] = total;
  }
  __threadfence();
  __syncthreads();
  if (threadIdx.x == 0) s_last = atomicAdd(ticket, 1) == static_cast<int>(gridDim.x) - 1;
  __syncthreads();
  if (!s_last) return;
  __threadfence();
  if (threadIdx.x == 0) *ticket = 0;
  scan_codes_block(counts, K, offsets, nullptr, work, nwork, stats);
}

__global__ void __launch_bounds__(SORT_THREADS)
scatter_cta_kernel(const int32_t* __restrict__ idx, int64_t N, int K, int64_t rows_per_cta,
                   const int32_t* __restrict__ cta_counts, const int32_t* __restrict__ offsets, int32_t* __restrict__ perm) {
  extern __shared__ int32_t sh[];
  const int32_t* base = cta_counts + static_cast<size_t>(blockIdx.x) * K;
  for (int i = threadIdx.x; i < K; i += SORT_THREADS) sh[i] = offsets[i] + base[i];
  __syncthreads();
  const int64_t b = blockIdx.x * rows_per_cta;
  const int64_t e = min(N, b + rows_per_cta);
  for (int64_t r = b + threadIdx.x; r < e; r += SORT_THREADS) {
    const int k = idx[r];
    if (k < 0) continue;
    const int pos = atomicAdd(&sh[k], 1);
    perm[pos] = static_cast<int32_t>(r);
  }
}

__global__ void scan_kernel(const int32_t* __restrict__ counts, int K, int32_t* offsets, int32_t* cursor, int4* work,
                            int32_t* nwork, float* stats) {
  scan_codes_block(counts, K, offsets, cursor, work, nwork, stats);
}

__global__ void scatter_kernel(const int32_t* __restrict__ idx, int64_t N, int32_t* cursor, int32_t* perm) {
  for (int64_t r = static_cast<int64_t>(blockIdx.x) * blockDim.x + threadIdx.x; r < N;
       r += static_cast<int64_t>(gridDim.x) * blockDim.x) {
    const int k = idx[r];
    if (k < 0) continue;
    const int pos = atomicAdd(&cursor[k], 1);
    perm[pos] = static_cast<int32_t>(r);
  }
}

template <int DT>
__global__ void __launch_bounds__(SEG_THREADS)
segsum_kernel(const void* __restrict__ x, int D, const int32_t* __restrict__ perm, const int4* __restrict__ work,
              const int32_t* __restrict__ nwork, float* embed_sum) {
  if (static_cast<int>(blockIdx.x) >= *nwork) return;
  constexpr int VEC = (DT == VQB_DTYPE_BF16) ? 8 : 4;
  constexpr int UNROLL = 8;
  extern __shared__ __align__(16) uint8_t seg_smem[];
  int32_t* s_perm = reinterpret_cast<int32_t*>(seg_smem);
  float* red = reinterpret_cast<float*>(seg_smem + SEG_CHUNK * sizeof(int32_t));
  const int4 wk = work[blockIdx.x];
  const int nrows = wk.z - wk.y;
  for (int i = threadIdx.x; i < nrows; i += SEG_THREADS) s_perm[i] = perm[wk.y + i];
  __syncthreads();
  const int TX = D / VEC;
  const int NY = SEG_THREADS / TX;
  const int tx = threadIdx.x % TX, ty = threadIdx.x / TX;
  float acc[VEC];
#pragma unroll
  for (int e = 0; e < VEC; ++e) acc[e] = 0.f;
  if (ty < NY) {
    const uint8_t* xb = reinterpret_cast<const uint8_t*>(x) + static_cast<size_t>(tx) * 16;
    const size_t row_bytes = static_cast<size_t>(D) * (DT == VQB_DTYPE_BF16 ? 2 : 4);
    auto accumulate = [&](const uint4& u) {
      const uint32_t w[4] = {u.x, u.y, u.z, u.w};
      if (DT == VQB_DTYPE_BF16) {
#pragma unroll
        for (int e = 0; e < 4; ++e) { acc[(2 * e) % VEC] += __uint_as_float(w[e] << 16); acc[(2 * e + 1) % VEC] += __uint_as_float(w[e] & 0xFFFF0000u); }
      } else {
#pragma unroll
        for (int e = 0; e < 4; ++e) acc[e % VEC] += __uint_as_float(w[e]);
      }
    };
    int r = ty;
    for (; r + (UNROLL - 1) * NY < nrows; r += UNROLL * NY) {
      uint4 u[UNROLL];
#pragma unroll
      for (int q = 0; q < UNROLL; ++q) u[q] = __ldg(reinterpret_cast<const uint4*>(xb + static_cast<size_t>(s_perm[r + q * NY]) * row_bytes));
#pragma unroll
      for (int q = 0; q < UNROLL; ++q) accumulate(u[q]);
    }
    for (; r < nrows; r += NY) accumulate(__ldg(reinterpret_cast<const uint4*>(xb + static_cast<size_t>(s_perm[r]) * row_bytes)));
    float* dst = red + ty * D + tx * VEC;
#pragma unroll
    for (int e = 0; e < VEC; ++e) dst[e] = acc[e];
  }
  __syncthreads();
  for (int i = threadIdx.x; i < D; i += blockDim.x) {
    float s = 0.f;
    for (int y = 0; y < NY; ++y) s += red[y * D + i];
    float* out = embed_sum + static_cast<int64_t>(wk.x) * D + i;
    atomicAdd(out, s);
  }
}

template <int DT>
__global__ void stats_add_flagged_kernel(const void* __restrict__ x, int64_t N, int D, const vqb_flag_entry* __restrict__ flagged,
                                         const int32_t* __restrict__ flag_count, const int32_t* __restrict__ idx,
                                         float* stats, int64_t soff) {
  using E = Elem<DT>;
  const int lane = threadIdx.x & 31;
  const int warps = (gridDim.x * blockDim.x) >> 5;
  int64_t cnt = flag_count[0], cnt_back = flag_count[1];
  if (cnt > N) cnt = N;
  if (cnt_back > N - cnt) cnt_back = N - cnt;
  for (int64_t j = (blockIdx.x * blockDim.x + threadIdx.x) >> 5; j < cnt + cnt_back; j += warps) {
    const int64_t e = j < cnt ? j : N - 1 - (j - cnt);
    const int row = flagged[e].row;
    const int k = idx[row];
    if (lane == 0) atomicAdd(stats + k, 1.f);
    float* dst = stats + soff + static_cast<int64_t>(k) * D;
    for (int i = lane * 4; i < D; i += 128) {
      const int64_t o = static_cast<int64_t>(row) * D + i;
      asm volatile("red.global.add.v4.f32 [%0], {%1, %2, %3, %4};" ::"l"(dst + i), "f"(E::load(x, o)), "f"(E::load(x, o + 1)),
                   "f"(E::load(x, o + 2)), "f"(E::load(x, o + 3)) : "memory");
    }
  }
}

__device__ __forceinline__ float lerp_f32(float a, float b, float w) {
  return (fabsf(w) < 0.5f) ? a + w * (b - a) : b - (b - a) * (1.f - w);
}

struct LocalStats {
  const float* p;
  __device__ __forceinline__ float load(int64_t i) const { return p[i]; }
  __device__ __forceinline__ float4 load4(int64_t i) const { return *reinterpret_cast<const float4*>(p + i); }
};
struct PeerStats {
  EmaStats s;
  __device__ __forceinline__ float load(int64_t i) const {
    float v[MAX_PEERS];
#pragma unroll
    for (int r = 0; r < MAX_PEERS; ++r)
      if (r < s.world) v[r] = s.p[r][i];
    float n = 0.f;
#pragma unroll
    for (int r = 0; r < MAX_PEERS; ++r)
      if (r < s.world) n += v[r];
    return n;
  }
  __device__ __forceinline__ float4 load4(int64_t i) const {
    float4 v[MAX_PEERS];
#pragma unroll
    for (int r = 0; r < MAX_PEERS; ++r)
      if (r < s.world) v[r] = *reinterpret_cast<const float4*>(s.p[r] + i);
    float4 n = make_float4(0.f, 0.f, 0.f, 0.f);
#pragma unroll
    for (int r = 0; r < MAX_PEERS; ++r)
      if (r < s.world) { n.x += v[r].x; n.y += v[r].y; n.z += v[r].z; n.w += v[r].w; }
    return n;
  }
};

template <class Src>
__global__ void ema_sizes_kernel(float* cluster_size, const Src src, int K, float w, const float* __restrict__ code_weight,
                                 int n_lerp, int64_t slice_stride, float* scratch, float* cmax) {
  __shared__ double part[32];
  double s = 0.0;
  for (int k = threadIdx.x; k < K; k += blockDim.x) {
    float c = cluster_size[k];
    if (n_lerp) {
      const float wk = code_weight ? __fmul_rn(w, code_weight[k]) : w;
      for (int j = 0; j < n_lerp; ++j) c = lerp_f32(c, src.load(j * slice_stride + k), wk);
      cluster_size[k] = c;
    }
    s += c;
  }
  s = warp_sum(s);
  if ((threadIdx.x & 31) == 0) part[threadIdx.x >> 5] = s;
  __syncthreads();
  if (threadIdx.x == 0) {
    double t = 0.0;
    for (int i = 0; i < (blockDim.x >> 5); ++i) t += part[i];
    scratch[0] = static_cast<float>(t);
    if (cmax) { cmax[CMAX_NORM] = 0.f; cmax[CMAX_RES] = 0.f; cmax[CMAX_LO] = 0.f; }
  }
}

template <int NV, class Src>
__global__ void ema_rows_kernel(const float* __restrict__ cluster_size, float* embed_avg, float* embed, const Src src,
                                int64_t soff, int K, int Kpad, int D, float w, const float* __restrict__ code_weight, float eps,
                                float keps, int metric, int n_lerp, int64_t slice_stride, int do_normalise,
                                const float* __restrict__ scratch, uint16_t* planes, uint16_t* bext, float* bias, float* cnorm2,
                                float* cmax) {
  const int lane = threadIdx.x & 31;
  const int k = blockIdx.x * (blockDim.x >> 5) + (threadIdx.x >> 5);
  if (k >= Kpad) return;
  if (k >= K) {
    if (do_normalise) write_padding_operands(k, Kpad, D, planes, bext, bias, lane);
    return;
  }
  float* avg = embed_avg + static_cast<int64_t>(k) * D;
  float* emb = embed + static_cast<int64_t>(k) * D;
  float4 a[NV];
  load_code_row<NV>(avg, D, lane, a);
  if (code_weight) w = __fmul_rn(w, code_weight[k]);
  const int64_t roff = soff + static_cast<int64_t>(k) * D;
  for (int q = 0; q < n_lerp; ++q) {
    float4 b[NV];
#pragma unroll
    for (int j = 0; j < NV; ++j) {
      const int i = j * 128 + lane * 4;
      if (i < D) b[j] = src.load4(q * slice_stride + roff + i);
    }
#pragma unroll
    for (int j = 0; j < NV; ++j) {
      const int i = j * 128 + lane * 4;
      if (i >= D) continue;
      a[j].x = lerp_f32(a[j].x, b[j].x, w); a[j].y = lerp_f32(a[j].y, b[j].y, w);
      a[j].z = lerp_f32(a[j].z, b[j].z, w); a[j].w = lerp_f32(a[j].w, b[j].w, w);
    }
  }
  if (n_lerp) {
#pragma unroll
    for (int j = 0; j < NV; ++j) {
      const int i = j * 128 + lane * 4;
      if (i < D) *reinterpret_cast<float4*>(avg + i) = a[j];
    }
  }
  if (!do_normalise) return;
  const float total = scratch[0];
  const float denom = __fmul_rn(__fdiv_rn(__fadd_rn(cluster_size[k], eps), __fadd_rn(total, keps)), total);
  double n2 = 0.0;
#pragma unroll
  for (int j = 0; j < NV; ++j) {
    const int i = j * 128 + lane * 4;
    if (i >= D) continue;
    a[j] = make_float4(__fdiv_rn(a[j].x, denom), __fdiv_rn(a[j].y, denom), __fdiv_rn(a[j].z, denom), __fdiv_rn(a[j].w, denom));
    if (metric == VQB_METRIC_COSINE)
      n2 += static_cast<double>(a[j].x) * a[j].x + static_cast<double>(a[j].y) * a[j].y + static_cast<double>(a[j].z) * a[j].z +
            static_cast<double>(a[j].w) * a[j].w;
  }
  if (metric == VQB_METRIC_COSINE) {
    const float nrm = fmaxf(static_cast<float>(sqrt(warp_sum(n2))), 1e-6f);
#pragma unroll
    for (int j = 0; j < NV; ++j)
      a[j] = make_float4(__fdiv_rn(a[j].x, nrm), __fdiv_rn(a[j].y, nrm), __fdiv_rn(a[j].z, nrm), __fdiv_rn(a[j].w, nrm));
  }
#pragma unroll
  for (int j = 0; j < NV; ++j) {
    const int i = j * 128 + lane * 4;
    if (i < D) *reinterpret_cast<float4*>(emb + i) = a[j];
  }
  write_code_operands<NV>(a, k, Kpad, D, metric, planes, bext, bias, cnorm2, cmax, lane);
}

template <class Src>
static void ema_launch(int part, const Src& src, float* cluster_size, float* embed_avg, float* embed, int K, int D, float w,
                       const float* code_weight, float eps, float keps, int metric, int n_lerp, int64_t slice_stride,
                       int do_normalise, uint16_t* planes, uint16_t* bext, float* bias, float* cnorm2, float* cmax,
                       float* scratch, cudaStream_t s) {
  if (part & 1)
    ema_sizes_kernel<Src><<<1, 1024, 0, s>>>(cluster_size, src, K, w, code_weight, n_lerp, slice_stride, scratch,
                                             do_normalise ? cmax : nullptr);
  if (part & 2) {
    const int Kpad = vqb_padded_codes(K);
    const int wpb = 8;
    const int64_t soff = vqb_stats_offset(K);
    auto rows = D <= 4 * 128 ? ema_rows_kernel<4, Src> : ema_rows_kernel<8, Src>;
    rows<<<(Kpad + wpb - 1) / wpb, wpb * 32, 0, s>>>(cluster_size, embed_avg, embed, src, soff, K, Kpad, D, w, code_weight, eps, keps,
                                                    metric, n_lerp, slice_stride, do_normalise, scratch, planes, bext, bias, cnorm2,
                                                    cmax);
  }
}

}

using namespace vqb;

extern "C" int64_t vqb_stats_offset(int K) { return K <= 0 ? 0 : (static_cast<int64_t>(K) + 3) / 4 * 4; }
extern "C" int64_t vqb_stats_floats(int K, int D) { return (K <= 0 || D <= 0) ? 0 : vqb_stats_offset(K) + static_cast<int64_t>(K) * D; }

int vqb::stats_add_flagged(const void* x_eff, int dtype, int64_t N, int D, const vqb_flag_entry* flagged,
                           const int32_t* flag_count, const int32_t* idx, int K, float* stats, void* stream) {
  if (!x_eff || !flagged || !flag_count || !idx || !stats) return VQB_E_INVALID;
  cudaStream_t s = static_cast<cudaStream_t>(stream);
  const int g = num_sms() * 8;
  const int64_t soff = vqb_stats_offset(K);
  if (dtype == VQB_DTYPE_F32) stats_add_flagged_kernel<VQB_DTYPE_F32><<<g, 256, 0, s>>>(x_eff, N, D, flagged, flag_count, idx, stats, soff);
  else stats_add_flagged_kernel<VQB_DTYPE_BF16><<<g, 256, 0, s>>>(x_eff, N, D, flagged, flag_count, idx, stats, soff);
  return static_cast<int>(cudaGetLastError());
}

extern "C" size_t vqb_ema_stats_workspace(int64_t N, int K) {
  if (N <= 0 || K <= 0) return 0;
  return carve(nullptr, nullptr, N, K);
}

extern "C" int vqb_debug_stats_plan(int64_t N, int K, int sms, int* out3) {
  if (!out3 || N <= 0 || K <= 0 || sms <= 0) return VQB_E_INVALID;
  if (N >= (static_cast<int64_t>(1) << 31)) return VQB_E_UNSUPPORTED;
  int shift = 31;
  out3[0] = sort_ctas(N, K, sms, &shift);
  out3[1] = shift;
  out3[2] = static_cast<int>(sort_ctas_bound(N, K));
  return VQB_OK;
}

static int stats_check(const void* x_eff, int dtype, int64_t N, int D, int K, const float* stats, const void* workspace,
                       size_t workspace_bytes, StatsWs* ws) {
  if (!stats || !workspace || N <= 0 || D <= 0 || K <= 0) return VQB_E_INVALID;
  if (dtype != VQB_DTYPE_F32 && dtype != VQB_DTYPE_BF16) return VQB_E_INVALID;
  if (D % 8 != 0 || D > 4 * SEG_THREADS) return VQB_E_UNSUPPORTED;
  if (N >= (static_cast<int64_t>(1) << 31)) return VQB_E_UNSUPPORTED;
  if ((reinterpret_cast<uintptr_t>(x_eff) | reinterpret_cast<uintptr_t>(workspace) | reinterpret_cast<uintptr_t>(stats)) & 15)
    return VQB_E_ALIGN;
  if (carve(ws, const_cast<void*>(workspace), N, K) > workspace_bytes) return VQB_E_WORKSPACE;
  return VQB_OK;
}

int vqb::stats_begin(float* stats, int dtype, int64_t N, int D, int K, void* workspace, size_t workspace_bytes, int prehist,
                     size_t zero_before, int32_t** hist, int* hist_shift, void* stats_stream, void* stream) {
  StatsWs ws;
  int rc = stats_check(stats, dtype, N, D, K, stats, workspace, workspace_bytes, &ws);
  if (rc) return rc;
  cudaStream_t s = static_cast<cudaStream_t>(stream);
  cudaError_t e = cudaMemsetAsync(stats, 0, sizeof(float) * static_cast<size_t>(vqb_stats_floats(K, D)),
                                  static_cast<cudaStream_t>(stats_stream ? stats_stream : stream));
  if (e != cudaSuccess) return static_cast<int>(e);
  int shift = 31;
  const int G = sort_ctas(N, K, num_sms(), &shift);
  e = cudaMemsetAsync(reinterpret_cast<uint8_t*>(ws.ticket) - zero_before, 0,
                      zero_before + 256 + ((G > 0 && prehist) ? sizeof(int32_t) * static_cast<size_t>(G) * K : 0), s);
  if (e != cudaSuccess) return static_cast<int>(e);
  if (G == 0) {
    e = cudaMemsetAsync(ws.counts, 0, sizeof(int32_t) * K, s);
    if (e != cudaSuccess) return static_cast<int>(e);
  }
  if (hist) *hist = G > 0 ? ws.cta_counts : ws.counts;
  if (hist_shift) *hist_shift = shift;
  return VQB_OK;
}

int vqb::stats_scan(const int32_t* idx, int dtype, int64_t N, int D, int K, float* stats, void* workspace,
                    size_t workspace_bytes, int prehist, void* stream) {
  StatsWs ws;
  int rc = stats_check(stats, dtype, N, D, K, stats, workspace, workspace_bytes, &ws);
  if (rc) return rc;
  if (!idx) return VQB_E_INVALID;
  cudaStream_t s = static_cast<cudaStream_t>(stream);
  int shift = 31;
  const int G = sort_ctas(N, K, num_sms(), &shift);
  if (G > 0) {
    static bool attr_set = false;
    if (!attr_set) {
      cudaFuncSetAttribute(hist_cta_kernel, cudaFuncAttributeMaxDynamicSharedMemorySize, SORT_MAX_K * 4);
      cudaFuncSetAttribute(scatter_cta_kernel, cudaFuncAttributeMaxDynamicSharedMemorySize, SORT_MAX_K * 4);
      attr_set = true;
    }
    const int64_t rows_per_cta = static_cast<int64_t>(128) << shift;
    if (!prehist) hist_cta_kernel<<<G, SORT_THREADS, static_cast<size_t>(K) * sizeof(int32_t), s>>>(idx, N, K, rows_per_cta, ws.cta_counts);
    colscan_kernel<<<(K + CS_CODES - 1) / CS_CODES, CS_CODES * CS_PARTS, 0, s>>>(ws.cta_counts, G, K, ws.counts, ws.ticket,
                                                                              ws.offsets, ws.work, ws.nwork, stats);
  } else {
    if (!prehist) {
      int g = static_cast<int>((N + 1023) / 1024);
      const int cap = num_sms() * 4;
      if (g > cap) g = cap;
      hist_kernel<<<g, 256, K <= 8192 ? K * sizeof(int32_t) : 0, s>>>(idx, N, K, ws.counts);
    }
    scan_kernel<<<1, 1024, 0, s>>>(ws.counts, K, ws.offsets, ws.cursor, ws.work, ws.nwork, stats);
  }
  return static_cast<int>(cudaGetLastError());
}

int vqb::stats_sum(const void* x_eff, int dtype, int64_t N, int D, const int32_t* idx, int K, float* stats, void* workspace,
                   size_t workspace_bytes, void* stream) {
  StatsWs ws;
  int rc = stats_check(x_eff, dtype, N, D, K, stats, workspace, workspace_bytes, &ws);
  if (rc) return rc;
  if (!x_eff || !idx) return VQB_E_INVALID;
  cudaStream_t s = static_cast<cudaStream_t>(stream);
  int shift = 31;
  const int G = sort_ctas(N, K, num_sms(), &shift);
  if (G > 0) {
    scatter_cta_kernel<<<G, SORT_THREADS, static_cast<size_t>(K) * sizeof(int32_t), s>>>(idx, N, K, static_cast<int64_t>(128) << shift,
                                                                                        ws.cta_counts, ws.offsets, ws.perm);
  } else {
    int g = static_cast<int>((N + 1023) / 1024);
    const int cap = num_sms() * 4;
    if (g > cap) g = cap;
    scatter_kernel<<<g, 256, 0, s>>>(idx, N, ws.cursor, ws.perm);
  }
  const int64_t soff = vqb_stats_offset(K);
  const int items = static_cast<int>(max_work_items(N, K));
  const int TX = D / (dtype == VQB_DTYPE_BF16 ? 8 : 4);
  const size_t red_bytes = SEG_CHUNK * sizeof(int32_t) + static_cast<size_t>(SEG_THREADS / TX) * D * sizeof(float);
  if (dtype == VQB_DTYPE_F32)
    segsum_kernel<VQB_DTYPE_F32><<<items, SEG_THREADS, red_bytes, s>>>(x_eff, D, ws.perm, ws.work, ws.nwork, stats + soff);
  else
    segsum_kernel<VQB_DTYPE_BF16><<<items, SEG_THREADS, red_bytes, s>>>(x_eff, D, ws.perm, ws.work, ws.nwork, stats + soff);
  return static_cast<int>(cudaGetLastError());
}

extern "C" int vqb_ema_stats(const void* x_eff, int dtype, int64_t N, int D, const int32_t* idx, int K, float* stats,
                             void* workspace, size_t workspace_bytes, void* stream) {
  if (!x_eff || !idx) return VQB_E_INVALID;
  int rc = stats_begin(stats, dtype, N, D, K, workspace, workspace_bytes, 0, 0, nullptr, nullptr, nullptr, stream);
  if (rc) return rc;
  rc = stats_scan(idx, dtype, N, D, K, stats, workspace, workspace_bytes, 0, stream);
  if (rc) return rc;
  return stats_sum(x_eff, dtype, N, D, idx, K, stats, workspace, workspace_bytes, stream);
}

extern "C" int vqb_ema_apply(float* cluster_size, float* embed_avg, float* embed, const float* stats, int K, int D,
                             double decay, double eps, int metric, int do_lerp, int do_normalise, void* planes,
                             void* bext, float* bias, float* cnorm2, float* cmax, float* scratch, void* stream) {
  return vqb_ema_apply_weighted(cluster_size, embed_avg, embed, stats, K, D, decay, eps, metric, do_lerp, do_normalise,
                                nullptr, planes, bext, bias, cnorm2, cmax, scratch, stream);
}

extern "C" int vqb_ema_apply_weighted(float* cluster_size, float* embed_avg, float* embed, const float* stats, int K, int D,
                                      double decay, double eps, int metric, int do_lerp, int do_normalise,
                                      const float* code_weight, void* planes, void* bext, float* bias, float* cnorm2,
                                      float* cmax, float* scratch, void* stream) {
  return ema_apply_part(3, local_stats(stats), cluster_size, embed_avg, embed, K, D, decay, eps, metric, do_lerp ? 1 : 0,
                        do_normalise, code_weight, planes, bext, bias, cnorm2, cmax, scratch, stream);
}

extern "C" int vqb_ema_apply_peers(float* cluster_size, float* embed_avg, float* embed, const void* const* peer_stats_host,
                                   int world, int64_t slice_offset, int K, int D, double decay, double eps, int metric,
                                   int do_normalise, const float* code_weight, void* planes, void* bext, float* bias,
                                   float* cnorm2, float* cmax, float* scratch, void* stream) {
  EmaStats src;
  const int rc = peer_stats(&src, peer_stats_host, world, slice_offset);
  if (rc) return rc;
  return ema_apply_part(3, src, cluster_size, embed_avg, embed, K, D, decay, eps, metric, 1, do_normalise, code_weight, planes,
                        bext, bias, cnorm2, cmax, scratch, stream);
}

int vqb::ema_apply_part(int part, const EmaStats& src, float* cluster_size, float* embed_avg, float* embed, int K, int D,
                        double decay, double eps, int metric, int n_lerp, int do_normalise, const float* code_weight,
                        void* planes, void* bext, float* bias, float* cnorm2, float* cmax, float* scratch, void* stream,
                        int64_t slice_stride) {
  if (!cluster_size || !embed_avg || !embed || !scratch || K <= 0 || D <= 0 || n_lerp < 0) return VQB_E_INVALID;
  if (n_lerp && (!src.p[0] || (slice_stride & 3))) return VQB_E_INVALID;
  if (!n_lerp && src.world) return VQB_E_INVALID;
  if (do_normalise && (!planes || !bext || !bias || !cnorm2 || !cmax)) return VQB_E_INVALID;
  if (D % 8 != 0 || D > CODE_ROW_MAX_D) return VQB_E_UNSUPPORTED;
  if ((reinterpret_cast<uintptr_t>(embed_avg) | reinterpret_cast<uintptr_t>(embed) | reinterpret_cast<uintptr_t>(planes)) & 15)
    return VQB_E_ALIGN;
  const int64_t soff = vqb_stats_offset(K);
  for (int r = 0; n_lerp && r < (src.world ? src.world : 1); ++r)
    if ((reinterpret_cast<uintptr_t>(src.p[r]) | reinterpret_cast<uintptr_t>(src.p[r] + soff)) & 15) return VQB_E_ALIGN;
  const float w = static_cast<float>(1.0 - decay);
  const float epsf = static_cast<float>(eps);
  const float keps = static_cast<float>(static_cast<double>(K) * eps);
  uint16_t* pl = static_cast<uint16_t*>(planes);
  uint16_t* be = static_cast<uint16_t*>(bext);
  cudaStream_t s = static_cast<cudaStream_t>(stream);
  if (src.world)
    ema_launch(part, PeerStats{src}, cluster_size, embed_avg, embed, K, D, w, code_weight, epsf, keps, metric, n_lerp, slice_stride,
               do_normalise, pl, be, bias, cnorm2, cmax, scratch, s);
  else
    ema_launch(part, LocalStats{src.p[0]}, cluster_size, embed_avg, embed, K, D, w, code_weight, epsf, keps, metric, n_lerp,
               slice_stride, do_normalise, pl, be, bias, cnorm2, cmax, scratch, s);
  return static_cast<int>(cudaGetLastError());
}
```

### vector_quantize_pytorch_b200/csrc/vq_forward.cu

```cuda
#include "vqb_common.cuh"
#include <stdio.h>
#include <stdlib.h>
#include <string.h>
#include <mutex>

using namespace vqb;

static_assert(sizeof(vqb_vq_forward_args) == 328, "vqb_vq_forward_args layout changed");
static_assert(sizeof(vqb_fused_outputs) == 104, "vqb_fused_outputs layout changed");
static_assert(sizeof(vqb_rvq_op) == 808, "vqb_rvq_op layout changed");

extern "C" int vqb_debug_active(void);

namespace {
inline size_t up256(size_t v) { return (v + 255) / 256 * 256; }

struct FwdWs {
  size_t x_eff, a_planes, flagged, counters, stats_ws, idx_prov, total;
};

FwdWs carve_fwd(int64_t N, int D, int K, int dtype, int metric, int update) {
  FwdWs w;
  size_t off = 0;
  const size_t esz = dtype == VQB_DTYPE_BF16 ? 2 : 4;
// ... 202 lines not shown
    cudaGraphDestroy(graph);
    if (++g_graph_failures > 4) g_graph_disabled = true;
    return fn(ctx, stream);
  };
  Variant* use = nullptr;
  if (pend || !donor) {
    use = pend ? pend : spare;
    if (!use) return fail();
    cudaGraphExec_t exec = nullptr;
    if (cudaGraphInstantiate(&exec, graph, 0) != cudaSuccess || !exec) return fail();
    if (use == &se->var[se->n_var]) ++se->n_var;
    use->exec = exec;
    ++g_n_instantiate;
  } else {
    if (spare) {
      if (spare == &se->var[se->n_var]) ++se->n_var;
      memcpy(spare->pkey, pk, kKeyBytes);
      spare->exec = nullptr;
      spare->last_use = g_tick;
    }
    cudaGraphExecUpdateResultInfo info;
    if (cudaGraphExecUpdate(donor->exec, graph, &info) != cudaSuccess) {
      cudaGetLastError();
      cudaGraphExecDestroy(donor->exec);
      donor->exec = nullptr;
      if (cudaGraphInstantiate(&donor->exec, graph, 0) != cudaSuccess || !donor->exec) {
        donor->exec = nullptr;
        memset(donor->pkey, 0xFF, kKeyBytes);
        return fail();
      }
    }
    use = donor;
    ++g_n_update;
  }
  cudaGraphDestroy(graph);
  memcpy(use->pkey, pk, kKeyBytes);
  use->last_use = g_tick;
  return static_cast<int>(cudaGraphLaunch(use->exec, s));
}

bool graphs_usable(cudaStream_t s) {
  cudaStreamCaptureStatus cap = cudaStreamCaptureStatusNone;
  return graph_mode() && !g_graph_disabled && !vqb_debug_active() && cudaStreamIsCapturing(s, &cap) == cudaSuccess &&
         cap == cudaStreamCaptureStatusNone;
}

int enqueue_one(const void* ctx, void* stream) { return vq_forward_enqueue(static_cast<const vqb_vq_forward_args*>(ctx), stream); }

struct RvqCtx { const vqb_rvq_op* ops; int n; };

struct LaneStreams {
  cudaStream_t stream[kLanes] = {nullptr, nullptr, nullptr, nullptr};
  cudaEvent_t begin = nullptr, done[kLanes] = {nullptr, nullptr, nullptr, nullptr};
  bool ok = false;
};
LaneStreams* lane_streams() {
  static LaneStreams ls;
  static bool tried = false;
  if (!tried) {
    tried = true;
    ls.ok = cudaEventCreateWithFlags(&ls.begin, cudaEventDisableTiming) == cudaSuccess;
    for (int l = 1; l < kLanes && ls.ok; ++l)
      ls.ok = cudaStreamCreateWithFlags(&ls.stream[l], cudaStreamNonBlocking) == cudaSuccess &&
              cudaEventCreateWithFlags(&ls.done[l], cudaEventDisableTiming) == cudaSuccess;
    if (!ls.ok) cudaGetLastError();
  }
  return ls.ok ? &ls : nullptr;
}

int rvq_enqueue(const void* ctx, void* stream) {
  const RvqCtx* c = static_cast<const RvqCtx*>(ctx);
  cudaStream_t s = static_cast<cudaStream_t>(stream);
  bool used[kLanes] = {false, false, false, false};
  for (int i = 0; i < c->n; ++i) {
    if (c->ops[i].lane < 0 || c->ops[i].lane >= kLanes) return VQB_E_INVALID;
    used[c->ops[i].lane] = true;
  }
  LaneStreams* ls = (used[1] || used[2] || used[3]) ? lane_streams() : nullptr;
  cudaStream_t lane_s[kLanes] = {s, s, s, s};
  if (ls) {
    if (cudaEventRecord(ls->begin, s) != cudaSuccess) return static_cast<int>(cudaGetLastError());
    for (int l = 1; l < kLanes; ++l)
      if (used[l]) {
        if (cudaStreamWaitEvent(ls->stream[l], ls->begin, 0) != cudaSuccess) return static_cast<int>(cudaGetLastError());
        lane_s[l] = ls->stream[l];
      }
  }
  int rc = VQB_OK;
  for (int i = 0; i < c->n && rc == VQB_OK; ++i) {
    const vqb_rvq_op& op = c->ops[i];
    cudaStream_t os = lane_s[op.lane];
    if (op.kind == VQB_RVQ_STAGE) {
      rc = vq_forward_enqueue(&op.stage, os, ls ? op.lane : 0);
    } else if (op.kind == VQB_RVQ_EMA) {
      rc = ema_apply_part(3, local_stats(op.ema.stats), op.ema.cluster_size, op.ema.embed_avg, op.ema.embed, op.ema.K, op.ema.D,
                          op.ema.decay, op.ema.eps, op.ema.metric, op.ema.do_lerp ? (op.ema.n_lerp > 1 ? op.ema.n_lerp : 1) : 0,
                          op.ema.do_normalise, nullptr, op.ema.planes, op.ema.bext, op.ema.bias, op.ema.cnorm2, op.ema.cmax,
                          op.ema.scratch, os, op.ema.slice_stride);
    } else if (op.kind == VQB_RVQ_ACCUMULATE) {
      rc = vqb_rvq_accumulate(op.acc.embeds, op.acc.embed_stride, op.acc.Q, op.acc.K, op.acc.D, op.acc.idx, op.acc.N,
                              op.acc.out, op.acc.dtype, os);
    } else if (op.kind == VQB_RVQ_BARRIER) {
      rc = vqb_peer_barrier(op.bar.flags, op.bar.rank, op.bar.world, op.bar.epoch, os);
    } else if (op.kind == VQB_RVQ_EMA_PEERS) {
      EmaStats src;
      rc = peer_stats(&src, op.emap.peer_stats, op.emap.world, op.emap.slice_offset);
      if (rc == VQB_OK)
        rc = ema_apply_part(3, src, op.emap.cluster_size, op.emap.embed_avg, op.emap.embed, op.emap.K, op.emap.D, op.emap.decay,
                            op.emap.eps, op.emap.metric, op.emap.n_lerp > 1 ? op.emap.n_lerp : 1, op.emap.do_normalise, nullptr,
                            op.emap.planes, op.emap.bext, op.emap.bias, op.emap.cnorm2, op.emap.cmax, op.emap.scratch, os,
                            op.emap.slice_stride);
    } else if (op.kind == VQB_RVQ_SIMVQ_TAIL) {
      const auto& t = op.simvq;
      rc = vqb_rsimvq_tail(t.r, t.codes, t.idx, t.N, t.D, t.rotation, t.r_next, t.qsum, t.first, t.idx64_out, t.idx_stride,
                           t.loss_sum, t.loss_out, t.input_weight, t.weight, os);
    } else {
      rc = VQB_E_INVALID;
    }
  }
  if (ls) {
    for (int l = 1; l < kLanes; ++l)
      if (used[l]) {
        if (cudaEventRecord(ls->done[l], ls->stream[l]) != cudaSuccess || cudaStreamWaitEvent(s, ls->done[l], 0) != cudaSuccess)
          if (rc == VQB_OK) rc = static_cast<int>(cudaGetLastError());
      }
  }
  return rc;
}

uint64_t hash_words(const uint64_t* w, int n, uint64_t seed) {
  uint64_t h = seed ^ 0x9E3779B97F4A7C15ull;
  for (int i = 0; i < n; ++i) {
    h ^= w[i] + 0x9E3779B97F4A7C15ull + (h << 6) + (h >> 2);
    h *= 0xFF51AFD7ED558CCDull;
    h ^= h >> 33;
  }
  return h;
}
}

extern "C" int vqb_vq_forward(const vqb_vq_forward_args* a, void* stream) {
  if (!a) return VQB_E_INVALID;
  if (a->update && a->stats_accumulate) return VQB_E_UNSUPPORTED;
  if (a->qsum) return VQB_E_UNSUPPORTED;
  std::lock_guard<std::mutex> lock(g_cache_mutex);
  if (a->ev_search_begin || a->ev_search_end || !graphs_usable(static_cast<cudaStream_t>(stream)))
    return vq_forward_enqueue(a, stream);
  uint64_t sk[kKeyWords], pk[kKeyWords];
  make_keys(a, stream, sk, pk);
  return run_cached(sk, pk, enqueue_one, a, stream);
}

extern "C" int vqb_rvq_forward(const vqb_rvq_op* ops, int n_ops, void* stream) {
  if (!ops || n_ops <= 0 || n_ops > kKeyWords - 2) return VQB_E_INVALID;
  std::lock_guard<std::mutex> lock(g_cache_mutex);
  RvqCtx ctx{ops, n_ops};
  bool events = false;
  for (int i = 0; i < n_ops; ++i) {
    if (ops[i].kind != VQB_RVQ_STAGE) continue;
    if (ops[i].stage.update && ops[i].stage.stats_accumulate) return VQB_E_UNSUPPORTED;
    if (ops[i].stage.qsum) return VQB_E_UNSUPPORTED;
    events |= ops[i].stage.ev_search_begin || ops[i].stage.ev_search_end;
  }
  if (events || !graphs_usable(static_cast<cudaStream_t>(stream))) return rvq_enqueue(&ctx, stream);
  uint64_t sk[kKeyWords], pk[kKeyWords];
  memset(sk, 0, sizeof(sk));
  memset(pk, 0, sizeof(pk));
  for (int i = 0; i < n_ops; ++i) {
    const vqb_rvq_op& op = ops[i];
    uint64_t s1[kKeyWords], p1[kKeyWords];
    memset(s1, 0, sizeof(s1));
    memset(p1, 0, sizeof(p1));
    if (op.kind == VQB_RVQ_STAGE) {
      make_keys(&op.stage, nullptr, s1, p1);
    } else if (op.kind == VQB_RVQ_EMA) {
      const void* ptrs[] = {op.ema.cluster_size, op.ema.embed_avg, op.ema.embed, op.ema.stats, op.ema.planes, op.ema.bext,
                            op.ema.bias, op.ema.cnorm2, op.ema.cmax, op.ema.scratch};
      for (int j = 0; j < 10; ++j) p1[j] = reinterpret_cast<uint64_t>(ptrs[j]);
      s1[0] = op.ema.K; s1[1] = op.ema.D; s1[2] = op.ema.metric; s1[3] = op.ema.do_lerp; s1[4] = op.ema.do_normalise;
      memcpy(&s1[5], &op.ema.decay, 8); memcpy(&s1[6], &op.ema.eps, 8);
      s1[7] = static_cast<uint64_t>(op.ema.n_lerp); s1[8] = static_cast<uint64_t>(op.ema.slice_stride);
    } else if (op.kind == VQB_RVQ_BARRIER) {
      if (!op.bar.flags || op.bar.world < 1 || op.bar.world > 16) return VQB_E_INVALID;
      for (int r = 0; r < op.bar.world; ++r) p1[r] = reinterpret_cast<uint64_t>(op.bar.flags[r]);
      p1[16] = reinterpret_cast<uint64_t>(op.bar.epoch);
      s1[0] = op.bar.rank; s1[1] = op.bar.world;
    } else if (op.kind == VQB_RVQ_EMA_PEERS) {
      if (!op.emap.peer_stats || op.emap.world < 1 || op.emap.world > 16) return VQB_E_INVALID;
      const void* ptrs[] = {op.emap.cluster_size, op.emap.embed_avg, op.emap.embed, op.emap.planes, op.emap.bext,
                            op.emap.bias, op.emap.cnorm2, op.emap.cmax, op.emap.scratch};
      for (int j = 0; j < 9; ++j) p1[j] = reinterpret_cast<uint64_t>(ptrs[j]);
      for (int r = 0; r < op.emap.world; ++r) p1[16 + r] = reinterpret_cast<uint64_t>(op.emap.peer_stats[r]);
      s1[0] = op.emap.K; s1[1] = op.emap.D; s1[2] = op.emap.metric; s1[3] = op.emap.do_normalise; s1[4] = op.emap.world;
      s1[5] = static_cast<uint64_t>(op.emap.slice_offset);
      memcpy(&s1[6], &op.emap.decay, 8); memcpy(&s1[7], &op.emap.eps, 8);
      s1[8] = static_cast<uint64_t>(op.emap.n_lerp); s1[9] = static_cast<uint64_t>(op.emap.slice_stride);
    } else if (op.kind == VQB_RVQ_ACCUMULATE) {
      p1[0] = reinterpret_cast<uint64_t>(op.acc.embeds); p1[1] = reinterpret_cast<uint64_t>(op.acc.idx);
      p1[2] = reinterpret_cast<uint64_t>(op.acc.out);
      s1[0] = op.acc.embed_stride; s1[1] = op.acc.Q; s1[2] = op.acc.K; s1[3] = op.acc.D; s1[4] = op.acc.N; s1[5] = op.acc.dtype;
    } else if (op.kind == VQB_RVQ_SIMVQ_TAIL) {
      const auto& t = op.simvq;
      const void* ptrs[] = {t.r, t.codes, t.idx, t.r_next, t.qsum, t.idx64_out, t.loss_sum, t.loss_out};
      for (int j = 0; j < 8; ++j) p1[j] = reinterpret_cast<uint64_t>(ptrs[j]);
      s1[0] = static_cast<uint64_t>(t.N); s1[1] = t.D; s1[2] = t.rotation; s1[3] = t.first; s1[4] = static_cast<uint64_t>(t.idx_stride);
      s1[5] = t.loss_out != nullptr;
      uint32_t wb[2];
      memcpy(&wb[0], &t.input_weight, 4); memcpy(&wb[1], &t.weight, 4);
      s1[6] = wb[0]; s1[7] = wb[1];
    } else {
      return VQB_E_INVALID;
    }
    sk[i] = hash_words(s1, kKeyWords, (static_cast<uint64_t>(op.kind) << 8) | static_cast<uint64_t>(op.lane));
    pk[i] = hash_words(p1, kKeyWords, 1);
  }
  sk[kKeyWords - 2] = static_cast<uint64_t>(n_ops) | (1ull << 40);
  sk[kKeyWords - 1] = reinterpret_cast<uint64_t>(stream);
  return run_cached(sk, pk, rvq_enqueue, &ctx, stream);
}

extern "C" int vqb_debug_graph_stats(long long* out4) {
  if (!out4) return VQB_E_INVALID;
  out4[0] = g_n_replay; out4[1] = g_n_update; out4[2] = g_n_instantiate; out4[3] = g_n_direct;
  return VQB_OK;
}

static int vq_forward_enqueue(const vqb_vq_forward_args* a, void* stream, int lane) {
  if (!a || !a->x || !a->embed || !a->planes || !a->bext || !a->cnorm2 || !a->cmax || !a->idx32 || !a->workspace)
    return VQB_E_INVALID;
  if (a->N <= 0 || a->D <= 0 || a->K <= 0) return VQB_E_INVALID;
  if (a->dtype != VQB_DTYPE_F32 && a->dtype != VQB_DTYPE_BF16) return VQB_E_INVALID;
  if (a->update && (!a->stats)) return VQB_E_INVALID;
  if (a->update >= 2 && (!a->cluster_size || !a->embed_avg || !a->bias || !a->scratch)) return VQB_E_INVALID;
  if (a->update == 3 && (!a->peer_stats || !a->peer_flags || !a->peer_epoch || a->peer_world < 1 || a->peer_world > 16))
    return VQB_E_INVALID;
  if (a->update < 0 || a->update > 3) return VQB_E_INVALID;
  const FwdWs w = carve_fwd(a->N, a->D, a->K, a->dtype, a->metric, a->update);
  if (w.total > a->workspace_bytes) return VQB_E_WORKSPACE;
  if (reinterpret_cast<uintptr_t>(a->workspace) & 255) return VQB_E_ALIGN;
  uint8_t* ws = static_cast<uint8_t*>(a->workspace);
  cudaStream_t s = static_cast<cudaStream_t>(stream);
  const bool cosine = a->metric == VQB_METRIC_COSINE;
  const bool l2 = cosine && !a->already_normalised;

  const void* x_eff = a->x;
  const void* a_planes = a->x;
  int n_a = 1;
  int rc = VQB_OK;
  if (a->dtype == VQB_DTYPE_BF16) {
    if (l2) {
      rc = vqb_input_prepare(a->x, a->dtype, a->N, a->D, 1, ws + w.x_eff, nullptr, 0, stream);
      if (rc) return rc;
      x_eff = ws + w.x_eff;
      a_planes = x_eff;
    }
  } else if (a->a_planes_in && !l2) {
    if (reinterpret_cast<uintptr_t>(a->a_planes_in) & 15) return VQB_E_ALIGN;
    a_planes = a->a_planes_in;
    n_a = 2;
  } else {
    rc = vqb_input_prepare(a->x, a->dtype, a->N, a->D, l2 ? 1 : 0, l2 ? ws + w.x_eff : nullptr, ws + w.a_planes, 2, stream);
    if (rc) return rc;
    if (l2) x_eff = ws + w.x_eff;
    a_planes = ws + w.a_planes;
    n_a = 2;
  }
  int32_t* flag_count = reinterpret_cast<int32_t*>(ws + w.counters);
  double* loss_sum = reinterpret_cast<double*>(ws + w.counters + 8);
  cudaError_t e = cudaSuccess;
  bool counters_zeroed = false;

  vqb_fused_outputs f = {};
  f.x_eff = x_eff; f.embed = a->embed; f.q_out = a->q_out; f.idx64_out = a->idx64_out; f.idx_stride = a->idx_stride;
  f.loss_sum = a->loss_out ? loss_sum : nullptr;
  f.x_raw = (x_eff != a->x) ? a->x : nullptr;
  f.resid_out = a->resid_out; f.dtype = a->dtype;
  f.planes_out = (a->dtype == VQB_DTYPE_F32 && a->resid_out && !l2) ? a->planes_out : nullptr;
  if (a->planes_out && (a->dtype != VQB_DTYPE_F32 || !a->resid_out || l2)) return VQB_E_UNSUPPORTED;
  const bool want_tail = a->q_out || a->idx64_out || a->loss_out;
  if (a->row_mask && (a->resid_out || a->planes_out)) return VQB_E_UNSUPPORTED;
  if (a->n_live && !a->row_mask) return VQB_E_INVALID;
  vqb_flag_entry* flagged = reinterpret_cast<vqb_flag_entry*>(ws + w.flagged);
  SideStream* side = a->update ? side_stream(lane) : nullptr;
  int32_t* idx_prov = side ? reinterpret_cast<int32_t*>(ws + w.idx_prov) : nullptr;
  const size_t stats_ws_bytes = a->update ? vqb_ema_stats_workspace(a->N, a->K) : 0;
  int32_t* hist = nullptr;
  int hist_shift = 0;
  if (side) {
    if (cudaEventRecord(side->fork0, s) != cudaSuccess || cudaStreamWaitEvent(side->stream, side->fork0, 0) != cudaSuccess)
      return static_cast<int>(cudaGetLastError());
    static_assert(sizeof(vqb_flag_entry) == 32, "flag entry layout");
    rc = stats_begin(a->stats, a->dtype, a->N, a->D, a->K, ws + w.stats_ws, stats_ws_bytes, 1, w.stats_ws - w.counters, &hist,
                     &hist_shift, side->stream, stream);
    if (rc) return rc;
    counters_zeroed = true;
  }
  if (!counters_zeroed) {
    e = cudaMemsetAsync(ws + w.counters, 0, 16, s);
    if (e != cudaSuccess) return static_cast<int>(e);
  }
  if (a->ev_search_begin) cudaEventRecord(static_cast<cudaEvent_t>(a->ev_search_begin), s);
  rc = assign_launch(a_planes, n_a, a->N, a->D, a->planes, a->bext, a->cmax, a->K, a->margin_rel, 0, a->idx32, idx_prov,
                     hist, hist_shift, flagged, flag_count, nullptr, want_tail ? &f : nullptr, a->metric, a->cnorm2, stream,
                     a->row_mask);
  if (rc) return rc;
  if (a->ev_search_end) cudaEventRecord(static_cast<cudaEvent_t>(a->ev_search_end), s);
  if (side) {
    if (cudaEventRecord(side->fork, s) != cudaSuccess || cudaStreamWaitEvent(side->stream, side->fork, 0) != cudaSuccess)
      return static_cast<int>(cudaGetLastError());
    rc = stats_scan(idx_prov, a->dtype, a->N, a->D, a->K, a->stats, ws + w.stats_ws, stats_ws_bytes, 1, side->stream);
    const cudaError_t ce = cudaEventRecord(side->counts, side->stream);
    if (!rc) rc = stats_sum(x_eff, a->dtype, a->N, a->D, idx_prov, a->K, a->stats, ws + w.stats_ws, stats_ws_bytes, side->stream);
    const cudaError_t je = cudaEventRecord(side->join, side->stream);
    if (rc) return rc;
    if (ce != cudaSuccess || je != cudaSuccess) return static_cast<int>(cudaGetLastError());
  }
  rc = vqb_fix_flagged(x_eff, a->dtype, a->N, a->D, a->embed, a->cnorm2, a->K, a->metric, flagged, flag_count, a->idx32,
                       want_tail ? &f : nullptr, stream);
  if (rc) return rc;
  if (a->loss_out) {
    rc = loss_finalize_launch(loss_sum, a->N * a->D, a->row_mask ? a->n_live : nullptr, a->D, a->dtype, a->loss_weight, a->loss_out,
                              stream);
    if (rc) return rc;
  }
  EmaStats src = local_stats(a->stats);
  if (a->update == 3) {
    rc = peer_stats(&src, a->peer_stats, a->peer_world, a->peer_slice_offset);
    if (rc) return rc;
  }
  auto ema = [&](int part) {
    return ema_apply_part(part, src, a->cluster_size, a->embed_avg, a->embed, a->K, a->D, a->decay, a->eps, a->metric, 1,
                          a->do_normalise, nullptr, a->planes, a->bext, a->bias, a->cnorm2, a->cmax, a->scratch, stream);
  };
  if (side) {
    if (cudaStreamWaitEvent(s, side->counts, 0) != cudaSuccess) return static_cast<int>(cudaGetLastError());
    rc = stats_add_flagged(x_eff, a->dtype, a->N, a->D, flagged, flag_count, a->idx32, a->K, a->stats, stream);
    if (rc) return rc;
    if (a->update >= 2) {
      if (a->update == 3) {
        rc = vqb_peer_barrier(a->peer_flags, a->peer_rank, a->peer_world, a->peer_epoch, stream);
        if (rc) return rc;
      }
      rc = ema(1);
      if (rc) return rc;
    }
    if (cudaStreamWaitEvent(s, side->join, 0) != cudaSuccess) return static_cast<int>(cudaGetLastError());
  } else if (a->update) {
    rc = vqb_ema_stats(x_eff, a->dtype, a->N, a->D, a->idx32, a->K, a->stats, ws + w.stats_ws, stats_ws_bytes, stream);
    if (rc) return rc;
  }
  if (a->update < 2) return VQB_OK;
  if (a->update == 3) {
    rc = vqb_peer_barrier(a->peer_flags, a->peer_rank, a->peer_world, a->peer_epoch, stream);
    if (rc) return rc;
  }
  return ema(side ? 2 : 3);
}
```

### vector_quantize_pytorch_b200/csrc/vqb_common.cuh

```cuda
#pragma once
#include <cuda_runtime.h>
#include <cuda_bf16.h>
#include <stdint.h>
#include <stdio.h>
#include <math.h>

#include "../../include/vqb200.h"

namespace vqb {

enum CmaxSlot { CMAX_NORM = 0 , CMAX_RES = 1 , CMAX_LO = 2 , CMAX_SLOTS = 3 };

__host__ __device__ inline int code_tile(int K) { return K >= 256 ? 256 : ((K + 15) / 16) * 16; }

inline int device_props(int* sms, int* major) {
  static int cached_dev = -1, c_sms = 0, c_major = 0;
  int dev = 0;
  if (cudaGetDevice(&dev) != cudaSuccess) return VQB_E_NO_DEVICE;
  if (dev != cached_dev) {
    if (cudaDeviceGetAttribute(&c_sms, cudaDevAttrMultiProcessorCount, dev) != cudaSuccess) return VQB_E_NO_DEVICE;
    if (cudaDeviceGetAttribute(&c_major, cudaDevAttrComputeCapabilityMajor, dev) != cudaSuccess) return VQB_E_NO_DEVICE;
    cached_dev = dev;
  }
  *sms = c_sms;
  *major = c_major;
  return VQB_OK;
}
inline int check_device() {
  int sms, major;
  int rc = device_props(&sms, &major);
  if (rc) return rc;
  return major == 9 ? VQB_OK : VQB_E_NO_DEVICE;
}
inline int num_sms() {
  int sms = 1, major;
  device_props(&sms, &major);
  return sms;
}

__device__ __forceinline__ float bf16_bits_to_float(uint16_t b) { return __uint_as_float(static_cast<uint32_t>(b) << 16); }
__device__ __forceinline__ uint16_t float_to_bf16_bits(float f) {
  return __bfloat16_as_ushort(__float2bfloat16_rn(f));
}
__device__ __forceinline__ float bf16_round(float f) { return bf16_bits_to_float(float_to_bf16_bits(f)); }

template <int DT> struct Elem;
template <> struct Elem<VQB_DTYPE_F32> {
  using T = float;
  static __device__ __forceinline__ float load(const void* p, int64_t i) { return reinterpret_cast<const float*>(p)[i]; }
  static __device__ __forceinline__ void store(void* p, int64_t i, float v) { reinterpret_cast<float*>(p)[i] = v; }
  static __device__ __forceinline__ float round(float v) { return v; }
};
template <> struct Elem<VQB_DTYPE_BF16> {
  using T = uint16_t;
  static __device__ __forceinline__ float load(const void* p, int64_t i) { return bf16_bits_to_float(reinterpret_cast<const uint16_t*>(p)[i]); }
  static __device__ __forceinline__ void store(void* p, int64_t i, float v) { reinterpret_cast<uint16_t*>(p)[i] = float_to_bf16_bits(v); }
  static __device__ __forceinline__ float round(float v) { return bf16_round(v); }
};

__device__ __forceinline__ double warp_sum(double v) {
#pragma unroll
  for (int o = 16; o > 0; o >>= 1) v += __shfl_xor_sync(0xffffffffu, v, o);
  return v;
}
__device__ __forceinline__ float warp_sum(float v) {
#pragma unroll
  for (int o = 16; o > 0; o >>= 1) v += __shfl_xor_sync(0xffffffffu, v, o);
  return v;
}


int assign_launch(const void* a_planes, int n_a, int64_t N, int D, const void* b_planes, const void* bext,
                  const float* cmax, int K, float margin_rel, int n_passes, int32_t* idx, int32_t* idx_prov,
                  int32_t* hist, int hist_shift, vqb_flag_entry* flagged, int32_t* flag_count, float* dbg_best,
                  const vqb_fused_outputs* fused, int metric, const float* cnorm2, void* stream,
                  const uint8_t* row_mask = nullptr );
int loss_finalize_launch(const double* loss_sum, int64_t numel, const int64_t* n_live, int D, int dtype, float weight,
                         float* loss_out, void* stream);
int stats_add_flagged(const void* x_eff, int dtype, int64_t N, int D, const vqb_flag_entry* flagged,
                      const int32_t* flag_count, const int32_t* idx, int K, float* stats, void* stream);
int stats_begin(float* stats, int dtype, int64_t N, int D, int K, void* workspace, size_t workspace_bytes, int prehist,
                size_t zero_before, int32_t** hist, int* hist_shift, void* stats_stream, void* stream);
int stats_scan(const int32_t* idx, int dtype, int64_t N, int D, int K, float* stats, void* workspace, size_t workspace_bytes,
               int prehist, void* stream);
int stats_sum(const void* x_eff, int dtype, int64_t N, int D, const int32_t* idx, int K, float* stats, void* workspace,
              size_t workspace_bytes, void* stream);
constexpr int MAX_PEERS = 16;
struct EmaStats {
  const float* p[MAX_PEERS];
  int world;
};
inline EmaStats local_stats(const float* stats) {
  EmaStats s = {};
  s.p[0] = stats;
  return s;
}
int peer_stats(EmaStats* src, const void* const* peer_stats_host, int world, int64_t slice_offset);
int ema_apply_part(int part, const EmaStats& src, float* cluster_size, float* embed_avg, float* embed, int K, int D,
                   double decay, double eps, int metric, int n_lerp, int do_normalise, const float* code_weight,
                   void* planes, void* bext, float* bias, float* cnorm2, float* cmax, float* scratch, void* stream,
                   int64_t slice_stride = 0);


}
```

### vector_quantize_pytorch_b200/ops.py

```python
from __future__ import annotations

import ctypes
from dataclasses import dataclass

import torch

from . import _C
from ._C import lib, check

DEFAULT_MARGIN = 2.0 ** -18

_DT = {torch.float32: _C.DTYPE_F32, torch.bfloat16: _C.DTYPE_BF16}

PROFILE_EVENTS = None
LAUNCHES = 0


def _count(n):
    global LAUNCHES
    LAUNCHES += n


def _dtype_code(t: torch.Tensor) -> int:
    try:
        return _DT[t.dtype]
    except KeyError:
        raise TypeError(f"vqb200 supports float32 and bfloat16 inputs, got {t.dtype}") from None


def _require_cuda(*ts):
    for t in ts:
        if t is not None and not t.is_cuda:
            raise RuntimeError("vqb200 has no CPU path: tensors must live on a CUDA (H100, sm_90) device")


def _p(t):
    return None if t is None else t.data_ptr()


def _stream():
    return torch.cuda.current_stream().cuda_stream


def padded_codes(K: int) -> int:
    return lib.vqb_padded_codes(K)


@dataclass
class CodebookOperands:
    planes: torch.Tensor
    bext: torch.Tensor
    bias: torch.Tensor
    cnorm2: torch.Tensor
    cmax: torch.Tensor
    scratch: torch.Tensor
    K: int
    D: int
    cosine: bool

    @staticmethod
    def allocate(K: int, D: int, cosine: bool, device) -> "CodebookOperands":
        Kpad = padded_codes(K)
        return CodebookOperands(
            planes=torch.empty((2, Kpad, D), dtype=torch.float16, device=device),
            bext=torch.empty((Kpad, 16), dtype=torch.bfloat16, device=device),
            bias=torch.empty((Kpad,), dtype=torch.float32, device=device),
            cnorm2=torch.empty((K,), dtype=torch.float32, device=device),
            cmax=torch.zeros((3,), dtype=torch.float32, device=device),
            scratch=torch.zeros((2,), dtype=torch.float32, device=device),
            K=K, D=D, cosine=cosine)


def prepare_codebook(embed: torch.Tensor, cosine: bool, out: CodebookOperands | None = None) -> CodebookOperands:
    _require_cuda(embed)
    assert embed.dtype == torch.float32 and embed.dim() == 2 and embed.is_contiguous()
    K, D = embed.shape
    ops = out if out is not None else CodebookOperands.allocate(K, D, cosine, embed.device)
    with torch.cuda.device(embed.device):
        check(lib.vqb_codebook_prepare(_p(embed), K, D, int(cosine), _p(ops.planes), _p(ops.bext), _p(ops.bias), _p(ops.cnorm2),
                                       _p(ops.cmax), _stream()), "vqb_codebook_prepare")
    _count(1)
    return ops


@dataclass
class SearchResult:
    idx: torch.Tensor
    x_eff: torch.Tensor
    flag_count: torch.Tensor
    flagged: torch.Tensor
    best: torch.Tensor | None = None
    rescan_count: torch.Tensor | None = None


def search(x: torch.Tensor, ops: CodebookOperands, embed: torch.Tensor, *, margin: float | None = None, n_passes: int = 0,
           debug_best: bool = False, fix: bool = True, normalise: bool = True, fused: dict | None = None) -> SearchResult:
    _require_cuda(x, embed)
    assert x.dim() == 2 and x.is_contiguous()
    N, D = x.shape
    assert D == ops.D
    dt = _dtype_code(x)
    cosine = ops.cosine
    l2 = cosine and normalise
    dev = x.device
    margin = DEFAULT_MARGIN if margin is None else margin
    with torch.cuda.device(dev):
        st = _stream()
        if x.dtype == torch.bfloat16:
            if l2:
                x_eff = torch.empty_like(x)
                check(lib.vqb_input_prepare(_p(x), dt, N, D, 1, _p(x_eff), None, 0, st), "vqb_input_prepare")
                _count(1)
            else:
                x_eff = x
            a_planes, n_a = x_eff, 1
        else:
            a_planes = torch.empty((2, N, D), dtype=torch.bfloat16, device=dev)
            x_eff = torch.empty_like(x) if l2 else x
            check(lib.vqb_input_prepare(_p(x), dt, N, D, int(l2), _p(x_eff) if l2 else None, _p(a_planes), 2, st),
                  "vqb_input_prepare")
            _count(1)
            n_a = 2
        idx = torch.empty((N,), dtype=torch.int32, device=dev)
        flagged = torch.empty((N, 8), dtype=torch.int32, device=dev)
        count = torch.zeros((2,), dtype=torch.int32, device=dev)
        best = torch.empty((N,), dtype=torch.float32, device=dev) if debug_best else None
        fo = None
        if fused is not None:
            fo = _C.FusedOutputs(x_eff=_p(x_eff), embed=_p(embed), q_out=_p(fused.get("q_out")),
                                 idx64_out=_p(fused.get("idx64_out")), idx_stride=int(fused.get("idx_stride", 1)),
                                 loss_sum=_p(fused.get("loss_sum")), x_raw=_p(x) if x_eff is not x else None,
                                 resid_out=_p(fused.get("resid_out")), stats_cnt=None, stats_sum=None, dtype=dt,
                                 planes_out=_p(fused.get("planes_out")),
                                 qsum=_p(fused.get("qsum")))
        fo_ref = ctypes.byref(fo) if fo is not None else None
        prof = PROFILE_EVENTS
        if prof is not None:
            ev0, ev1 = torch.cuda.Event(enable_timing=True), torch.cuda.Event(enable_timing=True)
            ev0.record()
        check(lib.vqb_assign_ex(_p(a_planes), n_a, N, D, _p(ops.planes), _p(ops.bext), _p(ops.cmax), ops.K, float(margin),
                                int(n_passes), _p(idx), _p(flagged), _p(count), _p(best), fo_ref, int(cosine),
                                _p(ops.cnorm2), st), "vqb_assign")
        if prof is not None:
            ev1.record()
            prof.append((ev0, ev1))
        _count(1 + 3 * int(fix))
        if fix:
            check(lib.vqb_fix_flagged(_p(x_eff), dt, N, D, _p(embed), _p(ops.cnorm2), ops.K, int(cosine), _p(flagged),
                                      _p(count), _p(idx), fo_ref, st), "vqb_fix_flagged")
    return SearchResult(idx, x_eff, count[:1], flagged, best, count[1:])


class Scratch:

    def __init__(self):
        self.idx = None
        self.ws = None

    def __deepcopy__(self, memo):
        return Scratch()

    def __reduce__(self):
        return (Scratch, ())

    @staticmethod
    def _fit(buf, nbytes, device):
        if buf is None or buf.numel() < nbytes or buf.device != device:
            buf = torch.empty((max(nbytes, 256),), dtype=torch.uint8, device=device)
        return buf

    def take(self, idx_bytes: int, ws_bytes: int, device) -> tuple[torch.Tensor, torch.Tensor]:
        self.idx = self._fit(self.idx, idx_bytes, device)
        self.ws = self._fit(self.ws, ws_bytes, device)
        return self.idx, self.ws


def vq_forward_args(x: torch.Tensor, ops: CodebookOperands, state: tuple, *, update: int, do_normalise: bool, decay: float,
                    eps: float, q_out=None, idx64_out=None, idx_stride: int = 1, loss_out=None, loss_weight: float = 1.0,
                    resid_out=None, stats=None, margin: float | None = None, already_normalised: bool = False,
                    scratch: Scratch | None = None, peer=None, peer_ptrs=None, peer_slice_offset: int = 0,
                    a_planes_in=None, planes_out=None, row_mask=None, n_live=None):
    if row_mask is not None:
        assert row_mask.dtype == torch.uint8 and row_mask.is_contiguous() and row_mask.numel() == x.shape[0] and row_mask.is_cuda
        assert n_live is None or (n_live.dtype == torch.int64 and n_live.numel() == 1 and n_live.is_cuda)
    _require_cuda(x, state[2])
    assert x.dim() == 2 and x.is_contiguous()
    N, D = x.shape
    K = ops.K
    dt = _dtype_code(x)
    dev = x.device
    cs, ea, emb = state
    nbytes = lib.vqb_vq_forward_workspace(N, D, K, dt, int(ops.cosine), int(update))
    idx_buf, ws = (scratch or Scratch()).take(4 * N, nbytes, dev)
    idx32 = idx_buf[:4 * N].view(torch.int32)
    if update and stats is None:
        stats = torch.empty((stats_floats(K, D),), dtype=torch.float32, device=dev)
    a = _C.VQForwardArgs(
        x=_p(x), dtype=dt, metric=int(ops.cosine), N=N, D=D, K=K, already_normalised=int(already_normalised),
        cluster_size=_p(cs), embed_avg=_p(ea), embed=_p(emb), planes=_p(ops.planes), bext=_p(ops.bext), bias=_p(ops.bias),
        cnorm2=_p(ops.cnorm2), cmax=_p(ops.cmax), scratch=_p(ops.scratch), q_out=_p(q_out), idx64_out=_p(idx64_out),
        idx_stride=int(idx_stride), loss_out=_p(loss_out), loss_weight=float(loss_weight), resid_out=_p(resid_out),
        idx32=_p(idx32), update=int(update), stats_mode=1, do_normalise=int(do_normalise), decay=float(decay),
        eps=float(eps), stats=_p(stats), margin_rel=float(DEFAULT_MARGIN if margin is None else margin),
        workspace=_p(ws), workspace_bytes=nbytes, ev_search_begin=None, ev_search_end=None,
        a_planes_in=_p(a_planes_in), planes_out=_p(planes_out), row_mask=_p(row_mask), n_live=_p(n_live))
    if update == 3:
        a.peer_stats = ctypes.cast(peer_ptrs, ctypes.c_void_p)
        a.peer_flags = ctypes.cast(peer.flag_ptrs, ctypes.c_void_p)
        a.peer_epoch = peer.epoch.data_ptr()
        a.peer_rank, a.peer_world, a.peer_slice_offset = peer.rank, peer.world, int(peer_slice_offset)
    n_launch = (4 + (1 if dt == _C.DTYPE_F32 or ops.cosine else 0) + (1 if loss_out is not None else 0) + (5 if update else 0)
                + (2 if update == 2 else 0) + (3 if update == 3 else 0))
    return a, idx32, stats, n_launch


def vq_forward(x: torch.Tensor, ops: CodebookOperands, state: tuple, **kw) -> tuple[torch.Tensor, torch.Tensor | None]:
    a, idx32, stats, n_launch = vq_forward_args(x, ops, state, **kw)
    with torch.cuda.device(x.device):
        prof = PROFILE_EVENTS
        if prof is not None:
            ev0, ev1 = torch.cuda.Event(enable_timing=True), torch.cuda.Event(enable_timing=True)
            ev0.record(); ev1.record()
            a.ev_search_begin, a.ev_search_end = ev0.cuda_event, ev1.cuda_event
            prof.append((ev0, ev1))
        check(lib.vqb_vq_forward(ctypes.byref(a), _stream()), "vqb_vq_forward")
    _count(n_launch)
    return idx32, stats


class RvqProgram:
    MAX_OPS = 62

    def __init__(self, device):
        self.device = device
        self.ops = []
        self.keep = []
        self.scratch = {}
        self.scratch_bufs = []
        self.launches = 0

    def stage(self, lane, x, cb_ops, state, **kw):
        scratch = self.scratch.setdefault(lane, Scratch())
        a, idx32, stats, n = vq_forward_args(x, cb_ops, state, scratch=scratch, **kw)
        op = _C.RvqOp(kind=_C.RVQ_STAGE, lane=lane)
        op.stage = a
        self.ops.append(op)
        self.keep.append((x, cb_ops, state, kw, idx32, stats))
        self.scratch_bufs += [scratch.idx, scratch.ws]
        self.launches += n
        return idx32, stats

    def ema(self, lane, cluster_size, embed_avg, embed, stats, cb_ops, *, decay, eps, do_lerp, do_normalise, n_lerp=1, slice_stride=0):
        K, D = embed.shape
        op = _C.RvqOp(kind=_C.RVQ_EMA, lane=lane)
        op.ema = _C.RvqEmaArgs(cluster_size=_p(cluster_size), embed_avg=_p(embed_avg), embed=_p(embed), stats=_p(stats), K=K, D=D,
                               decay=float(decay), eps=float(eps), metric=int(cb_ops.cosine), do_lerp=int(do_lerp),
                               do_normalise=int(do_normalise), planes=_p(cb_ops.planes), bext=_p(cb_ops.bext), bias=_p(cb_ops.bias),
                               cnorm2=_p(cb_ops.cnorm2), cmax=_p(cb_ops.cmax), scratch=_p(cb_ops.scratch),
                               n_lerp=int(n_lerp), slice_stride=int(slice_stride))
        self.ops.append(op)
        self.keep.append((cluster_size, embed_avg, embed, stats, cb_ops))
        self.launches += 2

    def barrier(self, lane, peer):
        op = _C.RvqOp(kind=_C.RVQ_BARRIER, lane=lane)
        op.bar = _C.RvqBarArgs(flags=ctypes.cast(peer.flag_ptrs, ctypes.c_void_p), epoch=peer.epoch.data_ptr(), rank=peer.rank,
                               world=peer.world)
        self.ops.append(op)
        self.keep.append(peer)
        self.launches += 1

    def ema_peers(self, lane, cluster_size, embed_avg, embed, peer, peer_ptrs, slice_offset, cb_ops, *, decay, eps, do_normalise,
                  n_lerp=1, slice_stride=0):
        K, D = embed.shape
        op = _C.RvqOp(kind=_C.RVQ_EMA_PEERS, lane=lane)
        op.emap = _C.RvqEmaPeersArgs(cluster_size=_p(cluster_size), embed_avg=_p(embed_avg), embed=_p(embed),
                                     peer_stats=ctypes.cast(peer_ptrs, ctypes.c_void_p), slice_offset=int(slice_offset),
                                     world=peer.world, K=K, D=D, decay=float(decay), eps=float(eps), metric=int(cb_ops.cosine),
                                     do_normalise=int(do_normalise), planes=_p(cb_ops.planes), bext=_p(cb_ops.bext),
                                     bias=_p(cb_ops.bias), cnorm2=_p(cb_ops.cnorm2), cmax=_p(cb_ops.cmax), scratch=_p(cb_ops.scratch),
                                     n_lerp=int(n_lerp), slice_stride=int(slice_stride))
        self.ops.append(op)
        self.keep.append((cluster_size, embed_avg, embed, peer, peer_ptrs, cb_ops))
        self.launches += 2

    def accumulate(self, lane, embeds, indices, out):
        N, Q = indices.shape
        if embeds.dim() == 2:
            K, D = embeds.shape
            stride = 0
        else:
            _, K, D = embeds.shape
            stride = K * D
        op = _C.RvqOp(kind=_C.RVQ_ACCUMULATE, lane=lane)
        op.acc = _C.RvqAccArgs(embeds=_p(embeds), embed_stride=stride, Q=Q, K=K, D=D, idx=_p(indices), N=N, out=_p(out),
                               dtype=_DT[out.dtype])
        self.ops.append(op)
        self.keep.append((embeds, indices, out))
        self.launches += 1

    def simvq_tail(self, lane, r, codes, idx32, *, rotation, r_next, qsum, first, idx64_out, idx_stride, loss_sum, loss_out,
                   input_weight, weight):
        N, D = r.shape
        op = _C.RvqOp(kind=_C.RVQ_SIMVQ_TAIL, lane=lane)
        op.simvq = _C.RvqSimvqArgs(r=_p(r), codes=_p(codes), idx=_p(idx32), N=N, D=D, rotation=int(rotation), r_next=_p(r_next),
                                   qsum=_p(qsum), first=int(first), idx64_out=_p(idx64_out), idx_stride=int(idx_stride),
                                   loss_sum=_p(loss_sum), loss_out=_p(loss_out), input_weight=float(input_weight),
                                   weight=float(weight))
        self.ops.append(op)
        self.keep.append((r, codes, idx32, r_next, qsum, idx64_out, loss_sum, loss_out))
        self.launches += 3 if loss_out is not None else 1

    def freeze(self):
        n = len(self.ops)
        assert 0 < n <= self.MAX_OPS
        self.arr = (_C.RvqOp * n)(*self.ops)
        self.n = n
        self.ops = None
        self.keep = None
        return self

    def run(self):
        if getattr(self, "arr", None) is None:
            self.freeze()
        with torch.cuda.device(self.device):
            check(lib.vqb_rvq_forward(ctypes.cast(self.arr, ctypes.c_void_p), self.n, _stream()), "vqb_rvq_forward")
        _count(self.launches)


def gather(x_eff: torch.Tensor, embed: torch.Tensor, idx: torch.Tensor, *, q_out: torch.Tensor | None = None,
           idx64_out: torch.Tensor | None = None, idx_stride: int = 1, loss_sum: torch.Tensor | None = None,
           x_raw: torch.Tensor | None = None, resid_out: torch.Tensor | None = None) -> None:
    _require_cuda(x_eff, embed, idx)
    N, D = x_eff.shape
    with torch.cuda.device(x_eff.device):
        check(lib.vqb_gather(_p(x_eff), _dtype_code(x_eff), N, D, _p(embed), _p(idx), _p(q_out), _p(idx64_out),
                             int(idx_stride), _p(loss_sum), _p(x_raw), _p(resid_out), None, _stream()), "vqb_gather")
    _count(1)


def loss_finalize(loss_sum: torch.Tensor, numel: int, dtype: torch.dtype, weight: float, out: torch.Tensor) -> None:
    with torch.cuda.device(loss_sum.device):
        check(lib.vqb_loss_finalize(_p(loss_sum), int(numel), _DT[dtype], float(weight), _p(out), _stream()),
              "vqb_loss_finalize")
    _count(1)


def stats_floats(K: int, D: int) -> int:
    return lib.vqb_stats_floats(K, D)


def stats_offset(K: int) -> int:
    return lib.vqb_stats_offset(K)


def ema_stats(x_eff: torch.Tensor, idx: torch.Tensor, K: int, out: torch.Tensor | None = None) -> torch.Tensor:
    _require_cuda(x_eff, idx)
    N, D = x_eff.shape
    dev = x_eff.device
    stats = out if out is not None else torch.empty((stats_floats(K, D),), dtype=torch.float32, device=dev)
    ws_bytes = lib.vqb_ema_stats_workspace(N, K)
    ws = torch.empty((ws_bytes,), dtype=torch.uint8, device=dev)
    with torch.cuda.device(dev):
        check(lib.vqb_ema_stats(_p(x_eff), _dtype_code(x_eff), N, D, _p(idx), K, _p(stats), _p(ws), ws_bytes, _stream()),
              "vqb_ema_stats")
    _count(4)
    return stats


def ema_apply(cluster_size: torch.Tensor, embed_avg: torch.Tensor, embed: torch.Tensor, stats: torch.Tensor | None,
              ops: CodebookOperands, *, decay: float, eps: float, do_lerp: bool, do_normalise: bool,
# ... 263 lines not shown
```

Baseline: 397.0 million.

## Add single-pass fp16 codebook plane to replace multi-pass bf16 split search

```diff
diff --git a/include/vqb200.h b/include/vqb200.h
--- a/include/vqb200.h
+++ b/include/vqb200.h
@@ -74,6 +74,10 @@
 int vqb_debug_set_mode(int mode);
 int vqb_debug_graph_stats(long long* out4);
 int vqb_debug_assign_plan(int n_a, int D, int n_passes, int* out6);
+int vqb_debug_assign_plan_f16(int D, int* out6);
+int vqb_debug_assign_f16(const void* x, int64_t N, int D, const void* b_planes, const void* bext, const float* cmax, int K,
+                         float margin_rel, int32_t* idx, vqb_flag_entry* flagged, int32_t* flag_count, float* dbg_best,
+                         int metric, void* stream);
 int vqb_debug_stats_plan(int64_t N, int K, int sms, int* out3);
 
 int vqb_fix_flagged(const void* x_eff, int dtype, int64_t N, int D, const float* embed, const float* cnorm2, int K,
diff --git a/vector_quantize_pytorch_b200/_C.py b/vector_quantize_pytorch_b200/_C.py
--- a/vector_quantize_pytorch_b200/_C.py
+++ b/vector_quantize_pytorch_b200/_C.py
@@ -91,6 +91,8 @@
     "vqb_debug_active": (_i32, []),
     "vqb_debug_graph_stats": (_i32, [_vp]),
     "vqb_debug_assign_plan": (_i32, [_i32, _i32, _i32, _vp]),
+    "vqb_debug_assign_plan_f16": (_i32, [_i32, _vp]),
+    "vqb_debug_assign_f16": (_i32, [_vp, _i64, _i32, _vp, _vp, _vp, _i32, _f32, _vp, _vp, _vp, _vp, _i32, _vp]),
     "vqb_debug_stats_plan": (_i32, [_i64, _i32, _i32, _vp]),
     "vqb_decode": (_i32, [_vp, _i64, _i32, _i32, _i32, _vp, _i64, _vp, _i32, _vp]),
     "vqb_rvq_accumulate": (_i32, [_vp, _i64, _i32, _i32, _i32, _vp, _i64, _vp, _i32, _vp]),
diff --git a/vector_quantize_pytorch_b200/csrc/code_operands.cuh b/vector_quantize_pytorch_b200/csrc/code_operands.cuh
--- a/vector_quantize_pytorch_b200/csrc/code_operands.cuh
+++ b/vector_quantize_pytorch_b200/csrc/code_operands.cuh
@@ -19,14 +19,24 @@
                                                     uint16_t* bext, float* bias, float* cnorm2, float* cmax, int lane) {
   uint16_t* hi = planes + static_cast<int64_t>(k) * D;
   uint16_t* lo = planes + (static_cast<int64_t>(Kpad) + k) * D;
+  uint16_t* h16 = planes + (2 * static_cast<int64_t>(Kpad) + k) * D;
   double n2 = 0.0;
-  float r2 = 0.f, l2 = 0.f;
+  float r2 = 0.f, l2 = 0.f, f2 = 0.f;
 #pragma unroll
   for (int j = 0; j < NV; ++j) {
     const int i = j * 128 + lane * 4;
     if (i >= D) continue;
     const float v[4] = {c[j].x, c[j].y, c[j].z, c[j].w};
     uint16_t h[4], l[4];
+    uint32_t w16[2];
+#pragma unroll
+    for (int e = 0; e < 2; ++e) {
+      asm("cvt.rn.satfinite.f16x2.f32 %0, %1, %2;" : "=r"(w16[e]) : "f"(v[2 * e + 1]), "f"(v[2 * e]));
+      const float d0 = v[2 * e] - __half2float(__ushort_as_half(static_cast<uint16_t>(w16[e] & 0xFFFFu)));
+      const float d1 = v[2 * e + 1] - __half2float(__ushort_as_half(static_cast<uint16_t>(w16[e] >> 16)));
+      f2 = fmaf(d0, d0, f2);
+      f2 = fmaf(d1, d1, f2);
+    }
 #pragma unroll
     for (int e = 0; e < 4; ++e) {
       h[e] = float_to_bf16_bits(v[e]);
@@ -39,10 +49,12 @@
     }
     *reinterpret_cast<uint2*>(hi + i) = make_uint2(h[0] | (uint32_t(h[1]) << 16), h[2] | (uint32_t(h[3]) << 16));
     *reinterpret_cast<uint2*>(lo + i) = make_uint2(l[0] | (uint32_t(l[1]) << 16), l[2] | (uint32_t(l[3]) << 16));
+    *reinterpret_cast<uint2*>(h16 + i) = make_uint2(w16[0], w16[1]);
   }
   n2 = warp_sum(n2);
   r2 = warp_sum(r2);
   l2 = warp_sum(l2);
+  f2 = warp_sum(f2);
   if (lane == 0) {
     const float n2f = static_cast<float>(n2);
     cnorm2[k] = n2f;
@@ -59,6 +71,7 @@
     atomicMax(reinterpret_cast<unsigned int*>(cmax + CMAX_NORM), __float_as_uint(sqrtf(n2f)));
     atomicMax(reinterpret_cast<unsigned int*>(cmax + CMAX_RES), __float_as_uint(__fsqrt_ru(r2) * 1.0001f));
     atomicMax(reinterpret_cast<unsigned int*>(cmax + CMAX_LO), __float_as_uint(__fsqrt_ru(l2) * 1.0001f));
+    atomicMax(reinterpret_cast<unsigned int*>(cmax + CMAX_F16), __float_as_uint(__fsqrt_ru(f2) * 1.0001f));
   }
 }
 
@@ -66,7 +79,8 @@
                                                        int lane) {
   uint16_t* hi = planes + static_cast<int64_t>(k) * D;
   uint16_t* lo = planes + (static_cast<int64_t>(Kpad) + k) * D;
-  for (int i = lane; i < D; i += 32) { hi[i] = 0; lo[i] = 0; }
+  uint16_t* h16 = planes + (2 * static_cast<int64_t>(Kpad) + k) * D;
+  for (int i = lane; i < D; i += 32) { hi[i] = 0; lo[i] = 0; h16[i] = 0; }
   if (lane == 0) bias[k] = INFINITY;
   if (lane < 16) bext[k * 16 + lane] = (lane == 0) ? float_to_bf16_bits(-3.0e38f) : 0;
 }
diff --git a/vector_quantize_pytorch_b200/csrc/ptx.cuh b/vector_quantize_pytorch_b200/csrc/ptx.cuh
--- a/vector_quantize_pytorch_b200/csrc/ptx.cuh
+++ b/vector_quantize_pytorch_b200/csrc/ptx.cuh
@@ -81,6 +81,8 @@
 }
 
 __device__ __forceinline__ void fence_proxy_async_shared() { asm volatile("fence.proxy.async.shared::cta;" ::: "memory"); }
+template <int ID, int N>
+__device__ __forceinline__ void named_barrier_sync() { asm volatile("bar.sync %0, %1;" ::"n"(ID), "n"(N) : "memory"); }
 __device__ __forceinline__ void wgmma_fence() { asm volatile("wgmma.fence.sync.aligned;" ::: "memory"); }
 __device__ __forceinline__ void wgmma_commit() { asm volatile("wgmma.commit_group.sync.aligned;" ::: "memory"); }
 template <int N>
@@ -92,25 +94,48 @@
   for (int i = 0; i < R; ++i) asm volatile("" : "+f"(d[i])::"memory");
 }
 
-__device__ __forceinline__ void wgmma_m64n128k16_bf16(float (&d)[64], uint64_t adesc, uint64_t bdesc) {
-  asm volatile(
-      "{\n"
-      "wgmma.mma_async.sync.aligned.m64n128k16.f32.bf16.bf16 "
-      "{%0, %1, %2, %3, %4, %5, %6, %7, %8, %9, %10, %11, %12, %13, %14, %15, "
-      "%16, %17, %18, %19, %20, %21, %22, %23, %24, %25, %26, %27, %28, %29, %30, %31, "
-      "%32, %33, %34, %35, %36, %37, %38, %39, %40, %41, %42, %43, %44, %45, %46, %47, "
-      "%48, %49, %50, %51, %52, %53, %54, %55, %56, %57, %58, %59, %60, %61, %62, %63}, "
-      "%64, %65, 1, 1, 1, 0, 0;\n"
-      "}\n"
-      : "+f"(d[0]), "+f"(d[1]), "+f"(d[2]), "+f"(d[3]), "+f"(d[4]), "+f"(d[5]), "+f"(d[6]), "+f"(d[7]),
-        "+f"(d[8]), "+f"(d[9]), "+f"(d[10]), "+f"(d[11]), "+f"(d[12]), "+f"(d[13]), "+f"(d[14]), "+f"(d[15]),
-        "+f"(d[16]), "+f"(d[17]), "+f"(d[18]), "+f"(d[19]), "+f"(d[20]), "+f"(d[21]), "+f"(d[22]), "+f"(d[23]),
-        "+f"(d[24]), "+f"(d[25]), "+f"(d[26]), "+f"(d[27]), "+f"(d[28]), "+f"(d[29]), "+f"(d[30]), "+f"(d[31]),
-        "+f"(d[32]), "+f"(d[33]), "+f"(d[34]), "+f"(d[35]), "+f"(d[36]), "+f"(d[37]), "+f"(d[38]), "+f"(d[39]),
-        "+f"(d[40]), "+f"(d[41]), "+f"(d[42]), "+f"(d[43]), "+f"(d[44]), "+f"(d[45]), "+f"(d[46]), "+f"(d[47]),
-        "+f"(d[48]), "+f"(d[49]), "+f"(d[50]), "+f"(d[51]), "+f"(d[52]), "+f"(d[53]), "+f"(d[54]), "+f"(d[55]),
-        "+f"(d[56]), "+f"(d[57]), "+f"(d[58]), "+f"(d[59]), "+f"(d[60]), "+f"(d[61]), "+f"(d[62]), "+f"(d[63])
-      : "l"(adesc), "l"(bdesc));
+#define VQB_ACC_REGS_64 \
+  "%0, %1, %2, %3, %4, %5, %6, %7, %8, %9, %10, %11, %12, %13, %14, %15, " \
+  "%16, %17, %18, %19, %20, %21, %22, %23, %24, %25, %26, %27, %28, %29, %30, %31, " \
+  "%32, %33, %34, %35, %36, %37, %38, %39, %40, %41, %42, %43, %44, %45, %46, %47, " \
+  "%48, %49, %50, %51, %52, %53, %54, %55, %56, %57, %58, %59, %60, %61, %62, %63"
+#define VQB_ACC_REGS_128 \
+  "%0, %1, %2, %3, %4, %5, %6, %7, %8, %9, %10, %11, %12, %13, %14, %15, " \
+  "%16, %17, %18, %19, %20, %21, %22, %23, %24, %25, %26, %27, %28, %29, %30, %31, " \
+  "%32, %33, %34, %35, %36, %37, %38, %39, %40, %41, %42, %43, %44, %45, %46, %47, " \
+  "%48, %49, %50, %51, %52, %53, %54, %55, %56, %57, %58, %59, %60, %61, %62, %63, " \
+  "%64, %65, %66, %67, %68, %69, %70, %71, %72, %73, %74, %75, %76, %77, %78, %79, " \
+  "%80, %81, %82, %83, %84, %85, %86, %87, %88, %89, %90, %91, %92, %93, %94, %95, " \
+  "%96, %97, %98, %99, %100, %101, %102, %103, %104, %105, %106, %107, %108, %109, %110, %111, " \
+  "%112, %113, %114, %115, %116, %117, %118, %119, %120, %121, %122, %123, %124, %125, %126, %127"
+#define VQB_ACC_RW_64(d) \
+  "+f"(d[0]), "+f"(d[1]), "+f"(d[2]), "+f"(d[3]), "+f"(d[4]), "+f"(d[5]), "+f"(d[6]), "+f"(d[7]),\
+  "+f"(d[8]), "+f"(d[9]), "+f"(d[10]), "+f"(d[11]), "+f"(d[12]), "+f"(d[13]), "+f"(d[14]), "+f"(d[15]),\
+  "+f"(d[16]), "+f"(d[17]), "+f"(d[18]), "+f"(d[19]), "+f"(d[20]), "+f"(d[21]), "+f"(d[22]), "+f"(d[23]),\
+  "+f"(d[24]), "+f"(d[25]), "+f"(d[26]), "+f"(d[27]), "+f"(d[28]), "+f"(d[29]), "+f"(d[30]), "+f"(d[31]),\
+  "+f"(d[32]), "+f"(d[33]), "+f"(d[34]), "+f"(d[35]), "+f"(d[36]), "+f"(d[37]), "+f"(d[38]), "+f"(d[39]),\
+  "+f"(d[40]), "+f"(d[41]), "+f"(d[42]), "+f"(d[43]), "+f"(d[44]), "+f"(d[45]), "+f"(d[46]), "+f"(d[47]),\
+  "+f"(d[48]), "+f"(d[49]), "+f"(d[50]), "+f"(d[51]), "+f"(d[52]), "+f"(d[53]), "+f"(d[54]), "+f"(d[55]),\
+  "+f"(d[56]), "+f"(d[57]), "+f"(d[58]), "+f"(d[59]), "+f"(d[60]), "+f"(d[61]), "+f"(d[62]), "+f"(d[63])
+#define VQB_ACC_RW_128(d) \
+  VQB_ACC_RW_64(d), \
+  "+f"(d[64]), "+f"(d[65]), "+f"(d[66]), "+f"(d[67]), "+f"(d[68]), "+f"(d[69]), "+f"(d[70]), "+f"(d[71]),\
+  "+f"(d[72]), "+f"(d[73]), "+f"(d[74]), "+f"(d[75]), "+f"(d[76]), "+f"(d[77]), "+f"(d[78]), "+f"(d[79]),\
+  "+f"(d[80]), "+f"(d[81]), "+f"(d[82]), "+f"(d[83]), "+f"(d[84]), "+f"(d[85]), "+f"(d[86]), "+f"(d[87]),\
+  "+f"(d[88]), "+f"(d[89]), "+f"(d[90]), "+f"(d[91]), "+f"(d[92]), "+f"(d[93]), "+f"(d[94]), "+f"(d[95]),\
+  "+f"(d[96]), "+f"(d[97]), "+f"(d[98]), "+f"(d[99]), "+f"(d[100]), "+f"(d[101]), "+f"(d[102]), "+f"(d[103]),\
+  "+f"(d[104]), "+f"(d[105]), "+f"(d[106]), "+f"(d[107]), "+f"(d[108]), "+f"(d[109]), "+f"(d[110]), "+f"(d[111]),\
+  "+f"(d[112]), "+f"(d[113]), "+f"(d[114]), "+f"(d[115]), "+f"(d[116]), "+f"(d[117]), "+f"(d[118]), "+f"(d[119]),\
+  "+f"(d[120]), "+f"(d[121]), "+f"(d[122]), "+f"(d[123]), "+f"(d[124]), "+f"(d[125]), "+f"(d[126]), "+f"(d[127])
+
+template <bool F16>
+__device__ __forceinline__ void wgmma_m64n128k16(float (&d)[64], uint64_t adesc, uint64_t bdesc) {
+  if constexpr (F16)
+    asm volatile("wgmma.mma_async.sync.aligned.m64n128k16.f32.f16.f16 {" VQB_ACC_REGS_64 "}, %64, %65, 1, 1, 1, 0, 0;\n"
+                 : VQB_ACC_RW_64(d) : "l"(adesc), "l"(bdesc));
+  else
+    asm volatile("wgmma.mma_async.sync.aligned.m64n128k16.f32.bf16.bf16 {" VQB_ACC_REGS_64 "}, %64, %65, 1, 1, 1, 0, 0;\n"
+                 : VQB_ACC_RW_64(d) : "l"(adesc), "l"(bdesc));
 }
 
 __device__ __forceinline__ void wgmma_m64n128k16_bf16_rs_set(float (&d)[64], uint32_t a01, uint64_t bdesc) {
@@ -136,38 +161,14 @@
       : "r"(a01), "r"(0u), "l"(bdesc), "n"(0));
 }
 
-__device__ __forceinline__ void wgmma_m64n256k16_bf16(float (&d)[128], uint64_t adesc, uint64_t bdesc) {
-  asm volatile(
-      "{\n"
-      "wgmma.mma_async.sync.aligned.m64n256k16.f32.bf16.bf16 "
-      "{%0, %1, %2, %3, %4, %5, %6, %7, %8, %9, %10, %11, %12, %13, %14, %15, "
-      "%16, %17, %18, %19, %20, %21, %22, %23, %24, %25, %26, %27, %28, %29, %30, %31, "
-      "%32, %33, %34, %35, %36, %37, %38, %39, %40, %41, %42, %43, %44, %45, %46, %47, "
-      "%48, %49, %50, %51, %52, %53, %54, %55, %56, %57, %58, %59, %60, %61, %62, %63, "
-      "%64, %65, %66, %67, %68, %69, %70, %71, %72, %73, %74, %75, %76, %77, %78, %79, "
-      "%80, %81, %82, %83, %84, %85, %86, %87, %88, %89, %90, %91, %92, %93, %94, %95, "
-      "%96, %97, %98, %99, %100, %101, %102, %103, %104, %105, %106, %107, %108, %109, %110, %111, "
-      "%112, %113, %114, %115, %116, %117, %118, %119, %120, %121, %122, %123, %124, %125, %126, %127}, "
-      "%128, %129, 1, 1, 1, 0, 0;\n"
-      "}\n"
-      :
-        "+f"(d[0]), "+f"(d[1]), "+f"(d[2]), "+f"(d[3]), "+f"(d[4]), "+f"(d[5]), "+f"(d[6]), "+f"(d[7]),
-        "+f"(d[8]), "+f"(d[9]), "+f"(d[10]), "+f"(d[11]), "+f"(d[12]), "+f"(d[13]), "+f"(d[14]), "+f"(d[15]),
-        "+f"(d[16]), "+f"(d[17]), "+f"(d[18]), "+f"(d[19]), "+f"(d[20]), "+f"(d[21]), "+f"(d[22]), "+f"(d[23]),
-        "+f"(d[24]), "+f"(d[25]), "+f"(d[26]), "+f"(d[27]), "+f"(d[28]), "+f"(d[29]), "+f"(d[30]), "+f"(d[31]),
-        "+f"(d[32]), "+f"(d[33]), "+f"(d[34]), "+f"(d[35]), "+f"(d[36]), "+f"(d[37]), "+f"(d[38]), "+f"(d[39]),
-        "+f"(d[40]), "+f"(d[41]), "+f"(d[42]), "+f"(d[43]), "+f"(d[44]), "+f"(d[45]), "+f"(d[46]), "+f"(d[47]),
-        "+f"(d[48]), "+f"(d[49]), "+f"(d[50]), "+f"(d[51]), "+f"(d[52]), "+f"(d[53]), "+f"(d[54]), "+f"(d[55]),
-        "+f"(d[56]), "+f"(d[57]), "+f"(d[58]), "+f"(d[59]), "+f"(d[60]), "+f"(d[61]), "+f"(d[62]), "+f"(d[63]),
-        "+f"(d[64]), "+f"(d[65]), "+f"(d[66]), "+f"(d[67]), "+f"(d[68]), "+f"(d[69]), "+f"(d[70]), "+f"(d[71]),
-        "+f"(d[72]), "+f"(d[73]), "+f"(d[74]), "+f"(d[75]), "+f"(d[76]), "+f"(d[77]), "+f"(d[78]), "+f"(d[79]),
-        "+f"(d[80]), "+f"(d[81]), "+f"(d[82]), "+f"(d[83]), "+f"(d[84]), "+f"(d[85]), "+f"(d[86]), "+f"(d[87]),
-        "+f"(d[88]), "+f"(d[89]), "+f"(d[90]), "+f"(d[91]), "+f"(d[92]), "+f"(d[93]), "+f"(d[94]), "+f"(d[95]),
-        "+f"(d[96]), "+f"(d[97]), "+f"(d[98]), "+f"(d[99]), "+f"(d[100]), "+f"(d[101]), "+f"(d[102]), "+f"(d[103]),
-        "+f"(d[104]), "+f"(d[105]), "+f"(d[106]), "+f"(d[107]), "+f"(d[108]), "+f"(d[109]), "+f"(d[110]), "+f"(d[111]),
-        "+f"(d[112]), "+f"(d[113]), "+f"(d[114]), "+f"(d[115]), "+f"(d[116]), "+f"(d[117]), "+f"(d[118]), "+f"(d[119]),
-        "+f"(d[120]), "+f"(d[121]), "+f"(d[122]), "+f"(d[123]), "+f"(d[124]), "+f"(d[125]), "+f"(d[126]), "+f"(d[127])
-      : "l"(adesc), "l"(bdesc));
+template <bool F16>
+__device__ __forceinline__ void wgmma_m64n256k16(float (&d)[128], uint64_t adesc, uint64_t bdesc) {
+  if constexpr (F16)
+    asm volatile("wgmma.mma_async.sync.aligned.m64n256k16.f32.f16.f16 {" VQB_ACC_REGS_128 "}, %128, %129, 1, 1, 1, 0, 0;\n"
+                 : VQB_ACC_RW_128(d) : "l"(adesc), "l"(bdesc));
+  else
+    asm volatile("wgmma.mma_async.sync.aligned.m64n256k16.f32.bf16.bf16 {" VQB_ACC_REGS_128 "}, %128, %129, 1, 1, 1, 0, 0;\n"
+                 : VQB_ACC_RW_128(d) : "l"(adesc), "l"(bdesc));
 }
 
 __device__ __forceinline__ void wgmma_m64n256k16_bf16_ss_set(float (&d)[128], uint64_t adesc, uint64_t bdesc) {
diff --git a/vector_quantize_pytorch_b200/csrc/vq_assign.cu b/vector_quantize_pytorch_b200/csrc/vq_assign.cu
--- a/vector_quantize_pytorch_b200/csrc/vq_assign.cu
+++ b/vector_quantize_pytorch_b200/csrc/vq_assign.cu
@@ -111,7 +111,7 @@
 };
 constexpr int WIDE_STATIC_SMEM = NUM_CONSUMER_WARPS * 32 * 4 + WM * 16 * 2;
 
-template <int TAIL, int WN>
+template <int TAIL, int WN, bool F16>
 __global__ void __launch_bounds__(NUM_THREADS, 1)
 vq_assign_kernel(const __grid_constant__ CUtensorMap tmA, const __grid_constant__ CUtensorMap tmB,
                  const __grid_constant__ CUtensorMap tmS, const AssignParams p) {
@@ -170,11 +170,18 @@
             for (int kb = 0; kb < p.KB; ++kb) tma_prefetch_l2_3d(&tmA, kb * BK, row0 + static_cast<int>(gridDim.x) * BM, ap);
         }
         for (int ct = 0; ct < p.num_code_steps; ++ct, ++gstep) {
+          if (F16 && ct == 0) {
+            for (int kb = 0; kb < p.KB; ++kb) {
+              { const long long c0 = PROF_CLOCK(); mbar_wait(smem_u32(&ctrl->a_empty[kb]), (t & 1) ^ 1); w_aempty += PROF_CLOCK() - c0; }
+              mbar_arrive_expect_tx(smem_u32(&ctrl->a_full[kb]), A_SUB_BYTES);
+              tma_load_3d(a_base + kb * A_SUB_BYTES, &tmA, smem_u32(&ctrl->a_full[kb]), kb * BK, row0, 0);
+            }
+          }
           for (int kb = 0; kb < p.KB; ++kb) {
             for (int ps = 0; ps < p.n_passes; ++ps) {
-              const int bplane = (ps == 1) ? 1 : 0;
+              const int bplane = F16 ? 2 : ((ps == 1) ? 1 : 0);
               const int aplane = (ps == 2) ? 1 : 0;
-              if (!stream_a && ct == 0 && (ps == 0 || ps == 2)) {
+              if (!F16 && !stream_a && ct == 0 && (ps == 0 || ps == 2)) {
                 const int sub = aplane * p.KB + kb;
                 { const long long c0 = PROF_CLOCK(); mbar_wait(smem_u32(&ctrl->a_empty[sub]), (t & 1) ^ 1); w_aempty += PROF_CLOCK() - c0; }
                 mbar_arrive_expect_tx(smem_u32(&ctrl->a_full[sub]), A_SUB_BYTES);
@@ -236,9 +243,13 @@
               for (int b = 0; b < CB; ++b)
                 if (ks[b] >= 0) v[b] = __ldg(reinterpret_cast<const uint4*>(src + static_cast<int64_t>(ks[b]) * row_bytes + off));
               if (TAIL == 1) {
+                uint4 xv[CB];
 #pragma unroll
                 for (int b = 0; b < CB; ++b)
-                  if (ex[b]) lsum += sq_diff16(*reinterpret_cast<const uint4*>(xin + (row_base + b) * row_bytes + off), v[b], bf);
+                  if (ex[b]) xv[b] = *reinterpret_cast<const uint4*>(xin + (row_base + b) * row_bytes + off);
+#pragma unroll
+                for (int b = 0; b < CB; ++b)
+                  if (ex[b]) lsum += sq_diff16(xv[b], v[b], bf);
               }
               if (TAIL == 2) {
                 uint4 x[CB];
@@ -346,21 +357,54 @@
         alo += __shfl_xor_sync(0xffffffffu, alo, 1);
         alo += __shfl_xor_sync(0xffffffffu, alo, 2);
         if (q == 0) ctrl->x2[rit0 + 8 * h] = a;
-        xlo[h] = alo;
-      }
+        if (!F16) xlo[h] = alo;
+      }
+    };
+    auto to_f16 = [&](int t, float (&xlo)[2]) {
+      for (int sub = 0; sub < p.KB; ++sub) mbar_wait(smem_u32(&ctrl->a_full[sub]), t & 1);
+      xlo[0] = xlo[1] = 0.f;
+#pragma unroll 1
+      for (int i = 0; i < 2 * p.KB; ++i) {
+#pragma unroll
+        for (int h = 0; h < 2; ++h) {
+          const uint32_t chunk = a_base + (i >> 1) * A_SUB_BYTES + (rit0 + 8 * h) * 128 + (q + 4 * (i & 1)) * 16;
+          uint32_t w[4];
+          asm volatile("ld.shared.v4.b32 {%0, %1, %2, %3}, [%4];" : "=r"(w[0]), "=r"(w[1]), "=r"(w[2]), "=r"(w[3]) : "r"(chunk) : "memory");
+          uint32_t o[4];
+#pragma unroll
+          for (int e = 0; e < 4; ++e) {
+            const float x0 = __uint_as_float(w[e] << 16), x1 = __uint_as_float(w[e] & 0xFFFF0000u);
+            asm("cvt.rn.satfinite.f16x2.f32 %0, %1, %2;" : "=r"(o[e]) : "f"(x1), "f"(x0));
+            const float d0 = x0 - __half2float(__ushort_as_half(static_cast<uint16_t>(o[e] & 0xFFFFu)));
+            const float d1 = x1 - __half2float(__ushort_as_half(static_cast<uint16_t>(o[e] >> 16)));
+            xlo[h] = fmaf(d0, d0, xlo[h]);
+            xlo[h] = fmaf(d1, d1, xlo[h]);
+          }
+          asm volatile("st.shared.v4.b32 [%0], {%1, %2, %3, %4};" ::"r"(chunk), "r"(o[0]), "r"(o[1]), "r"(o[2]), "r"(o[3]) : "memory");
+        }
+      }
+#pragma unroll
+      for (int h = 0; h < 2; ++h) {
+        xlo[h] += __shfl_xor_sync(0xffffffffu, xlo[h], 1);
+        xlo[h] += __shfl_xor_sync(0xffffffffu, xlo[h], 2);
+      }
+      fence_proxy_async_shared();
+      if (a_row_off == 0) named_barrier_sync<1, 128>();
+      else named_barrier_sync<2, 128>();
     };
     auto init_band = [&](auto (&sc)[2], float (&xlo)[2]) {
       const bool euclid = p.metric != VQB_METRIC_COSINE;
       const float cmax = __ldg(p.cmax + CMAX_NORM);
-      const float cres = __ldg(p.cmax + CMAX_RES);
-      const float caux = p.n_a == 2 ? 0x1.02p-8f * cmax + __ldg(p.cmax + CMAX_LO) : 0.f;
+      const float cres = __ldg(p.cmax + (F16 ? CMAX_F16 : CMAX_RES));
+      const float caux = F16 ? cmax + cres : (p.n_a == 2 ? 0x1.02p-8f * cmax + __ldg(p.cmax + CMAX_LO) : 0.f);
       __syncwarp();
 #pragma unroll
       for (int h = 0; h < 2; ++h) {
         const float x2 = ctrl->x2[rit0 + 8 * h];
         const float xn = sqrtf(x2);
         const float xc = xn * cmax;
-        xlo[h] = p.n_a == 2 ? sqrtf(xlo[h]) * 1.0001f : 0.f;
+        if (F16) xlo[h] = fminf(sqrtf(xlo[h]) * 1.0001f, 3.4e38f);
+        else xlo[h] = p.n_a == 2 ? sqrtf(xlo[h]) * 1.0001f : 0.f;
         sc[h].init(2.f * (xn * cres + xlo[h] * caux + p.margin_rel * xc + (euclid ? 0x1p-21f * cmax * cmax : 0.f)) +
                    0x1p-18f * (xc + (euclid ? 0.5f * cmax * cmax : 0.f)) +
                    (euclid ? 0x1p-22f * (x2 + cmax * cmax) + 1e-8f : 1e-30f));
@@ -373,7 +417,9 @@
       float xlo[2] = {0.f, 0.f};
       for (int ct = 0; ct < p.num_code_steps; ++ct) {
         const bool last_ct = ct == p.num_code_steps - 1;
+        if (WN == 128 && F16 && ct == 0) to_f16(t, xlo);
         if (WN == 256 && ct == 0) {
+          if (F16) to_f16(t, xlo);
           row_norms(tile, xlo);
           init_band(sc, xlo);
         }
@@ -388,7 +434,7 @@
         for (int i = 0; i < n_items; ++i) {
           const int aplane = (ps == 2) ? 1 : 0;
           const int sub = aplane * p.KB + kb;
-          if (ct == 0 && !stream_a) { const long long c0 = PROF_CLOCK(); mbar_wait(smem_u32(&ctrl->a_full[sub]), t & 1); w_afull += PROF_CLOCK() - c0; }
+          if (!F16 && ct == 0 && !stream_a) { const long long c0 = PROF_CLOCK(); mbar_wait(smem_u32(&ctrl->a_full[sub]), t & 1); w_afull += PROF_CLOCK() - c0; }
           if (i > 0) { const long long c0 = PROF_CLOCK(); mbar_wait(smem_u32(&ctrl->b_full[stage]), ph); w_full += PROF_CLOCK() - c0; }
           const uint32_t st_addr = b_base + stage * stage_stride;
           const uint32_t a_addr = (stream_a ? st_addr : a_base + sub * A_SUB_BYTES) + a_row_off;
@@ -398,15 +444,15 @@
           wgmma_fence();
 #pragma unroll
           for (int k = 0; k < 8; k += 2) {
-            if constexpr (WN == 128) wgmma_m64n128k16_bf16(acc, ad + k, bd + k);
-            else wgmma_m64n256k16_bf16(acc, ad + k, bd + k);
+            if constexpr (WN == 128) wgmma_m64n128k16<F16>(acc, ad + k, bd + k);
+            else wgmma_m64n256k16<F16>(acc, ad + k, bd + k);
           }
           wgmma_commit();
           if (i == n_items - 1) gap0 = PROF_CLOCK();
           wgmma_wait<1>();
           fence_regs(acc);
           if (pend_stage >= 0) release(pend_stage, pend_sub);
-          const bool last_use = last_ct && !stream_a && (aplane == 1 ? ps == 2 : ps == 1);
+          const bool last_use = last_ct && !stream_a && (aplane == 1 ? ps == 2 : ps == (F16 ? 0 : 1));
           pend_stage = stage;
           pend_sub = last_use ? sub : -1;
           if (++stage == n_ring) { stage = 0; ph ^= 1; }
@@ -546,13 +592,18 @@
   int stream_a, n_stages, n_seed, n_items, KB, smem_bytes;
 };
 
-static int assign_plan(int n_a, int D, int n_passes, AssignPlan* pl) {
+static int assign_plan(int n_a, int D, int n_passes, AssignPlan* pl, bool f16 = false) {
   if (D <= 0 || (n_a != 1 && n_a != 2)) return VQB_E_INVALID;
+  if (f16) {
+    if (n_a != 1) return VQB_E_UNSUPPORTED;
+    n_passes = 1;
+  }
   if (n_passes == 0) n_passes = n_a + 1;
-  if (n_passes != n_a + 1) return VQB_E_UNSUPPORTED;
+  if (!f16 && n_passes != n_a + 1) return VQB_E_UNSUPPORTED;
   if (D % 8 != 0) return VQB_E_UNSUPPORTED;
   const int KB = (D + BK - 1) / BK;
   const int stream_a = n_a * KB > MAX_A_SUB ? 1 : 0;
+  if (f16 && stream_a) return VQB_E_UNSUPPORTED;
   const int a_bytes = stream_a ? 0 : n_a * KB * A_SUB_BYTES;
   const int stage_bytes = B_SUB_BYTES + (stream_a ? A_SUB_BYTES : 0);
   const int fixed = SMEM_CTRL_BYTES + 1024  + a_bytes;
@@ -595,6 +646,16 @@
   return VQB_OK;
 }
 
+extern "C" int vqb_debug_assign_plan_f16(int D, int* out6) {
+  if (!out6) return VQB_E_INVALID;
+  AssignPlan pl;
+  const int rc = assign_plan(1, D, 1, &pl, true);
+  if (rc) return rc;
+  out6[0] = pl.stream_a; out6[1] = pl.n_stages; out6[2] = pl.n_seed;
+  out6[3] = pl.n_items; out6[4] = pl.KB; out6[5] = pl.smem_bytes;
+  return VQB_OK;
+}
+
 extern "C" int vqb_padded_codes(int K) {
   if (K <= 0) return 0;
   const int BN = code_tile(K);
@@ -623,15 +684,42 @@
                             flagged, flag_count, dbg_best, fused, metric, cnorm2, stream);
 }
 
+template <bool F16>
+static void launch_kernel(bool wide, int tail, int grid, int smem_bytes, cudaStream_t s, const CUtensorMap& tmA,
+                          const CUtensorMap& tmB, const CUtensorMap& tmS, const AssignParams& p) {
+  if (wide) {
+    if (tail == 1) vq_assign_kernel<1, 256, F16><<<grid, NUM_THREADS, smem_bytes, s>>>(tmA, tmB, tmS, p);
+    else if (tail == 2) vq_assign_kernel<2, 256, F16><<<grid, NUM_THREADS, smem_bytes, s>>>(tmA, tmB, tmS, p);
+    else vq_assign_kernel<0, 256, F16><<<grid, NUM_THREADS, smem_bytes, s>>>(tmA, tmB, tmS, p);
+  } else {
+    if (tail == 1) vq_assign_kernel<1, 128, F16><<<grid, NUM_THREADS, smem_bytes, s>>>(tmA, tmB, tmS, p);
+    else if (tail == 2) vq_assign_kernel<2, 128, F16><<<grid, NUM_THREADS, smem_bytes, s>>>(tmA, tmB, tmS, p);
+    else vq_assign_kernel<0, 128, F16><<<grid, NUM_THREADS, smem_bytes, s>>>(tmA, tmB, tmS, p);
+  }
+}
+
+extern "C" int vqb_debug_assign_f16(const void* x, int64_t N, int D, const void* b_planes, const void* bext, const float* cmax,
+                                    int K, float margin_rel, int32_t* idx, vqb_flag_entry* flagged, int32_t* flag_count,
+                                    float* dbg_best, int metric, void* stream) {
+  int out6[6];
+  const int rc = vqb_debug_assign_plan_f16(D, out6);
+  if (rc) return rc;
+  return vqb::assign_launch(x, 1, N, D, b_planes, bext, cmax, K, margin_rel, 0, idx, nullptr, nullptr, 0, flagged, flag_count,
+                            dbg_best, nullptr, metric, nullptr, stream, nullptr, true);
+}
+
 int vqb::assign_launch(const void* a_planes, int n_a, int64_t N, int D, const void* b_planes, const void* bext,
                        const float* cmax, int K, float margin_rel, int n_passes, int32_t* idx, int32_t* idx_prov,
                        int32_t* hist, int hist_shift, vqb_flag_entry* flagged, int32_t* flag_count, float* dbg_best,
-                       const vqb_fused_outputs* fused, int metric, const float* cnorm2, void* stream, const uint8_t* row_mask) {
+                       const vqb_fused_outputs* fused, int metric, const float* cnorm2, void* stream, const uint8_t* row_mask,
+                       bool f16) {
   if (!a_planes || !b_planes || !bext || !cmax || !idx || !flagged || !flag_count) return VQB_E_INVALID;
   if (N <= 0 || K <= 0) return VQB_E_INVALID;
   AssignPlan plan;
-  int rc = assign_plan(n_a, D, n_passes, &plan);
-  if (rc) return rc;
+  f16 = f16 && assign_plan(n_a, D, n_passes, &plan, true) == VQB_OK;
+  int rc = assign_plan(n_a, D, n_passes, &plan, f16);
+  if (rc) return rc;
+  if (f16) n_passes = 1;
   if (n_passes == 0) n_passes = n_a + 1;
   if (N > (static_cast<int64_t>(1) << 31) - BM) return VQB_E_UNSUPPORTED;
   if ((reinterpret_cast<uintptr_t>(a_planes) | reinterpret_cast<uintptr_t>(b_planes) | reinterpret_cast<uintptr_t>(bext)) & 15)
@@ -670,18 +758,20 @@
   CUtensorMap tmA, tmB, tmS;
   rc = make_map(&tmA, a_planes, D, N, n_a, BK, BM, CU_TENSOR_MAP_SWIZZLE_128B);
   if (rc) return rc;
-  rc = make_map(&tmB, b_planes, D, p.Kpad, 2, BK, WN, CU_TENSOR_MAP_SWIZZLE_128B);
+  rc = make_map(&tmB, b_planes, D, p.Kpad, f16 ? 3 : 2, BK, WN, CU_TENSOR_MAP_SWIZZLE_128B);
   if (rc) return rc;
   rc = make_map(&tmS, bext, 16, p.Kpad, 1, 16, WN, CU_TENSOR_MAP_SWIZZLE_32B);
   if (rc) return rc;
 
   static bool attr_set = false;
   if (!attr_set) {
-    void (*const kernels[6])(CUtensorMap, CUtensorMap, CUtensorMap, AssignParams) = {
-        vq_assign_kernel<0, 128>, vq_assign_kernel<1, 128>, vq_assign_kernel<2, 128>,
-        vq_assign_kernel<0, 256>, vq_assign_kernel<1, 256>, vq_assign_kernel<2, 256>};
-    for (int i = 0; i < 6; ++i) {
-      const int dyn = i < 3 ? SMEM_LIMIT : SMEM_LIMIT - WIDE_STATIC_SMEM;
+    void (*const kernels[12])(CUtensorMap, CUtensorMap, CUtensorMap, AssignParams) = {
+        vq_assign_kernel<0, 128, false>, vq_assign_kernel<1, 128, false>, vq_assign_kernel<2, 128, false>,
+        vq_assign_kernel<0, 128, true>, vq_assign_kernel<1, 128, true>, vq_assign_kernel<2, 128, true>,
+        vq_assign_kernel<0, 256, false>, vq_assign_kernel<1, 256, false>, vq_assign_kernel<2, 256, false>,
+        vq_assign_kernel<0, 256, true>, vq_assign_kernel<1, 256, true>, vq_assign_kernel<2, 256, true>};
+    for (int i = 0; i < 12; ++i) {
+      const int dyn = i < 6 ? SMEM_LIMIT : SMEM_LIMIT - WIDE_STATIC_SMEM;
       const cudaError_t e = cudaFuncSetAttribute(kernels[i], cudaFuncAttributeMaxDynamicSharedMemorySize, dyn);
       if (e != cudaSuccess) return static_cast<int>(e);
     }
@@ -689,14 +779,8 @@
   }
   const int grid = p.num_row_tiles < num_sms() ? p.num_row_tiles : num_sms();
   cudaStream_t s = static_cast<cudaStream_t>(stream);
-  if (wide) {
-    if (p.copy_mode) vq_assign_kernel<1, 256><<<grid, NUM_THREADS, smem_bytes, s>>>(tmA, tmB, tmS, p);
-    else if (p.resid_mode) vq_assign_kernel<2, 256><<<grid, NUM_THREADS, smem_bytes, s>>>(tmA, tmB, tmS, p);
-    else vq_assign_kernel<0, 256><<<grid, NUM_THREADS, smem_bytes, s>>>(tmA, tmB, tmS, p);
-  } else {
-    if (p.copy_mode) vq_assign_kernel<1, 128><<<grid, NUM_THREADS, smem_bytes, s>>>(tmA, tmB, tmS, p);
-    else if (p.resid_mode) vq_assign_kernel<2, 128><<<grid, NUM_THREADS, smem_bytes, s>>>(tmA, tmB, tmS, p);
-    else vq_assign_kernel<0, 128><<<grid, NUM_THREADS, smem_bytes, s>>>(tmA, tmB, tmS, p);
-  }
+  const int tail = p.copy_mode ? 1 : (p.resid_mode ? 2 : 0);
+  if (f16) launch_kernel<true>(wide, tail, grid, smem_bytes, s, tmA, tmB, tmS, p);
+  else launch_kernel<false>(wide, tail, grid, smem_bytes, s, tmA, tmB, tmS, p);
   return static_cast<int>(cudaGetLastError());
 }
diff --git a/vector_quantize_pytorch_b200/csrc/vq_ema.cu b/vector_quantize_pytorch_b200/csrc/vq_ema.cu
--- a/vector_quantize_pytorch_b200/csrc/vq_ema.cu
+++ b/vector_quantize_pytorch_b200/csrc/vq_ema.cu
@@ -361,7 +361,7 @@
     double t = 0.0;
     for (int i = 0; i < (blockDim.x >> 5); ++i) t += part[i];
     scratch[0] = static_cast<float>(t);
-    if (cmax) { cmax[CMAX_NORM] = 0.f; cmax[CMAX_RES] = 0.f; cmax[CMAX_LO] = 0.f; }
+    if (cmax) { cmax[CMAX_NORM] = 0.f; cmax[CMAX_RES] = 0.f; cmax[CMAX_LO] = 0.f; cmax[CMAX_F16] = 0.f; }
   }
 }
 
diff --git a/vector_quantize_pytorch_b200/csrc/vq_forward.cu b/vector_quantize_pytorch_b200/csrc/vq_forward.cu
--- a/vector_quantize_pytorch_b200/csrc/vq_forward.cu
+++ b/vector_quantize_pytorch_b200/csrc/vq_forward.cu
@@ -528,7 +528,7 @@
   if (a->ev_search_begin) cudaEventRecord(static_cast<cudaEvent_t>(a->ev_search_begin), s);
   rc = assign_launch(a_planes, n_a, a->N, a->D, a->planes, a->bext, a->cmax, a->K, a->margin_rel, 0, a->idx32, idx_prov,
                      hist, hist_shift, flagged, flag_count, nullptr, want_tail ? &f : nullptr, a->metric, a->cnorm2, stream,
-                     a->row_mask);
+                     a->row_mask, n_a == 1);
   if (rc) return rc;
   if (a->ev_search_end) cudaEventRecord(static_cast<cudaEvent_t>(a->ev_search_end), s);
   if (side) {
diff --git a/vector_quantize_pytorch_b200/csrc/vqb_common.cuh b/vector_quantize_pytorch_b200/csrc/vqb_common.cuh
--- a/vector_quantize_pytorch_b200/csrc/vqb_common.cuh
+++ b/vector_quantize_pytorch_b200/csrc/vqb_common.cuh
@@ -1,6 +1,7 @@
 #pragma once
 #include <cuda_runtime.h>
 #include <cuda_bf16.h>
+#include <cuda_fp16.h>
 #include <stdint.h>
 #include <stdio.h>
 #include <math.h>
@@ -9,7 +10,10 @@
 
 namespace vqb {
 
-enum CmaxSlot { CMAX_NORM = 0 , CMAX_RES = 1 , CMAX_LO = 2 , CMAX_SLOTS = 3 };
+enum CmaxSlot {
+  CMAX_NORM = 0 , CMAX_RES = 1 , CMAX_LO = 2 ,
+  CMAX_F16 = 3 , CMAX_SLOTS = 4
+};
 
 __host__ __device__ inline int code_tile(int K) { return K >= 256 ? 256 : ((K + 15) / 16) * 16; }
 
@@ -74,7 +78,8 @@
                   const float* cmax, int K, float margin_rel, int n_passes, int32_t* idx, int32_t* idx_prov,
                   int32_t* hist, int hist_shift, vqb_flag_entry* flagged, int32_t* flag_count, float* dbg_best,
                   const vqb_fused_outputs* fused, int metric, const float* cnorm2, void* stream,
-                  const uint8_t* row_mask = nullptr );
+                  const uint8_t* row_mask = nullptr ,
+                  bool f16 = false );
 int loss_finalize_launch(const double* loss_sum, int64_t numel, const int64_t* n_live, int D, int dtype, float weight,
                          float* loss_out, void* stream);
 int stats_add_flagged(const void* x_eff, int dtype, int64_t N, int D, const vqb_flag_entry* flagged,
diff --git a/vector_quantize_pytorch_b200/ops.py b/vector_quantize_pytorch_b200/ops.py
--- a/vector_quantize_pytorch_b200/ops.py
+++ b/vector_quantize_pytorch_b200/ops.py
@@ -62,11 +62,11 @@
     def allocate(K: int, D: int, cosine: bool, device) -> "CodebookOperands":
         Kpad = padded_codes(K)
         return CodebookOperands(
-            planes=torch.empty((2, Kpad, D), dtype=torch.float16, device=device),
+            planes=torch.empty((3, Kpad, D), dtype=torch.float16, device=device),
             bext=torch.empty((Kpad, 16), dtype=torch.bfloat16, device=device),
             bias=torch.empty((Kpad,), dtype=torch.float32, device=device),
             cnorm2=torch.empty((K,), dtype=torch.float32, device=device),
-            cmax=torch.zeros((3,), dtype=torch.float32, device=device),
+            cmax=torch.zeros((4,), dtype=torch.float32, device=device),
             scratch=torch.zeros((2,), dtype=torch.float32, device=device),
             K=K, D=D, cosine=cosine)
 
```

Measured after the change: 398.8 million, median of 6. No clear change (+0.5%).
